# Sun-Sir/BSARec

Hardware: AMD Instinct MI355X
Metric: train sequences/sec, ML-1M L=50 d=64 2-layer (higher is better)
Workload: dtype f32

## Files before the change

### bsarec_amd/_lib.py

```python
import ctypes as C
import os

HERE = os.path.dirname(os.path.abspath(__file__))
LIB_PATH = os.environ.get("BSAREC_LIB") or os.path.join(HERE, "libbsarec_hip.so")
MAX_LAYERS = 16
ABI_VERSION = 10
TOPK_MAX = 1024
NEG_MAX = 1024
NEG_MAX_DRAWS = 1 << 20
TRAIN_NEG_MAX = 8192
TRAIN_NEG_SITE = 0x4E454753

(BUF_LAYER_OUT, BUF_LOGITS, BUF_LOSS, BUF_DSP, BUF_HMIX, BUF_PROBS, BUF_DLAYER_IN, BUF_LOSS_ROWS, BUF_CTX,
 BUF_DLOGITS, BUF_TRAIN_CAND, BUF_TRAIN_CORR, BUF_TRAIN_LOGITS, BUF_TRAIN_DLOGITS) = range(14)
K_NONE, K_FFN1, K_FFN2, K_QKV, K_LOGITS, K_DU, K_DW1, K_FUSED_FWD, K_FUSED_BWD = range(9)

LAYER_FIELDS = ["sqrt_beta", "filter_ln_w", "filter_ln_b", "query_w", "query_b", "key_w", "key_b", "value_w", "value_b",
                "dense_w", "dense_b", "attn_ln_w", "attn_ln_b", "ffn1_w", "ffn1_b", "ffn2_w", "ffn2_b", "ffn_ln_w",
                "ffn_ln_b"]
LAYER_KEYS = {
    "sqrt_beta": "layer.filter_layer.sqrt_beta",
    "filter_ln_w": "layer.filter_layer.LayerNorm.weight", "filter_ln_b": "layer.filter_layer.LayerNorm.bias",
    "query_w": "layer.attention_layer.query.weight", "query_b": "layer.attention_layer.query.bias",
    "key_w": "layer.attention_layer.key.weight", "key_b": "layer.attention_layer.key.bias",
    "value_w": "layer.attention_layer.value.weight", "value_b": "layer.attention_layer.value.bias",
    "dense_w": "layer.attention_layer.dense.weight", "dense_b": "layer.attention_layer.dense.bias",
    "attn_ln_w": "layer.attention_layer.LayerNorm.weight", "attn_ln_b": "layer.attention_layer.LayerNorm.bias",
    "ffn1_w": "feed_forward.dense_1.weight", "ffn1_b": "feed_forward.dense_1.bias",
    "ffn2_w": "feed_forward.dense_2.weight", "ffn2_b": "feed_forward.dense_2.bias",
    "ffn_ln_w": "feed_forward.LayerNorm.weight", "ffn_ln_b": "feed_forward.LayerNorm.bias",
}
OPTIONAL_LAYER_KEYS = {"filter_cw": "layer.filter_layer.complex_weight"}
TOP_KEYS = {"item_emb": "item_embeddings.weight", "pos_emb": "position_embeddings.weight",
            "ln_w": "LayerNorm.weight", "ln_b": "LayerNorm.bias"}


class Config(C.Structure):
    _fields_ = [("batch", C.c_int), ("seq_len", C.c_int), ("hidden", C.c_int), ("heads", C.c_int), ("layers", C.c_int),
                ("item_size", C.c_int), ("cutoff_bins", C.c_int), ("alpha", C.c_float), ("ln_eps", C.c_float),
                ("p_hidden", C.c_float), ("p_attn", C.c_float), ("filter_kind", C.c_int),
                ("hidden_act", C.c_int), ("storage", C.c_int), ("no_fused", C.c_int), ("no_prune_top", C.c_int),
                ("dw_tiled", C.c_int), ("splits", C.c_int), ("top_slabs", C.c_int), ("separate_embed", C.c_int),
                ("separate_top", C.c_int), ("chain_kernels", C.c_int), ("x3_products", C.c_int),
                ("train_negatives", C.c_int), ("train_sampler", C.c_int), ("train_no_logq", C.c_int),
                ("train_lazy_adam", C.c_int),
                ("weight_image", C.c_int)]


TRAIN_FIELDS = ("train_negatives", "train_sampler", "train_no_logq")
TRAIN_SAMPLERS = {"uniform": 0, "popularity": 1}


OPTION_FIELDS = ("storage", "no_fused", "no_prune_top", "dw_tiled", "splits", "top_slabs", "separate_embed", "separate_top", "chain_kernels", "x3_products",
                 "weight_image")
HIDDEN_ACTS = {"gelu": 0, "relu": 1, "swish": 2, "tanh": 3, "sigmoid": 4}

_defaults = {k: 0 for k in OPTION_FIELDS}
_defaults["weight_image"] = 1


def _env_defaults():
    e = os.environ
    d = {}
    if e.get("BSAREC_DW") == "tiled":
        d["dw_tiled"] = 1
    if e.get("BSAREC_PRUNE_TOP") == "0":
        d["no_prune_top"] = 1
    if e.get("BSAREC_EMBED_IN_BLOCK") == "0":
        d["separate_embed"] = 1
    if e.get("BSAREC_TOP_TAIL") == "0":
        d["separate_top"] = 1
    if e.get("BSAREC_FUSED") == "0":
        d["no_fused"] = 1
    if e.get("BSAREC_BLOCK_KERNELS") == "chain":
        d["chain_kernels"] = 1
    if e.get("BSAREC_PRODUCTS") == "bf16x3":
        d["x3_products"] = 1
    for env, key, hi in (("BSAREC_TOP_SLABS", "top_slabs", 16), ("BSAREC_SPLITS", "splits", 1024)):
        if e.get(env, "").isdigit() and 1 <= int(e[env]) <= hi:
            d[key] = int(e[env])
    if e.get("BSAREC_STORAGE") == "bf16":
        d["storage"] = 1
    if e.get("BSAREC_WEIGHT_IMAGE") == "0":
        d["weight_image"] = 0
    return d


def set_default_options(**kw):
    old = {}
    for k, v in kw.items():
        if k not in _defaults:
            raise KeyError(k)
        old[k] = _defaults[k]
        _defaults[k] = int(v)
    return old


def default_options():
    d = dict(_defaults)
    d.update(_env_defaults())
    return d


class Layer(C.Structure):
    _fields_ = [(f, C.c_void_p) for f in LAYER_FIELDS] + [("filter_cw", C.c_void_p)]


class Tensors(C.Structure):
    _fields_ = [("item_emb", C.c_void_p), ("pos_emb", C.c_void_p), ("ln_w", C.c_void_p), ("ln_b", C.c_void_p),
                ("layer", Layer * MAX_LAYERS)]


class Adam(C.Structure):
    _fields_ = [("params", C.c_void_p), ("grads", C.c_void_p), ("exp_avg", C.c_void_p), ("exp_avg_sq", C.c_void_p),
                ("n", C.c_long), ("lr", C.c_float), ("beta1", C.c_float), ("beta2", C.c_float), ("eps", C.c_float),
                ("weight_decay", C.c_float), ("grad_scale", C.c_float), ("shadow_bf16", C.c_void_p), ("shadow_from", C.c_long),
                ("grads2", C.c_void_p), ("grads2_n", C.c_long), ("n_grad_srcs", C.c_int), ("grad_srcs", C.c_void_p * 8),
# ... 10 lines not shown
                ("num_layers", C.c_int), ("out_size", C.c_int)]


class Gru4RecConfig(C.Structure):
    _fields_ = [("gru", GruConfig), ("item_size", C.c_int), ("dropout", C.c_float)]


class Gru4RecHead(C.Structure):
    _fields_ = [("loss", C.c_int), ("candidates", C.c_int), ("bpreg", C.c_float)]


class CaserConfig(C.Structure):
    _fields_ = [("batch", C.c_int), ("seq_len", C.c_int), ("width", C.c_int), ("n_h", C.c_int), ("n_v", C.c_int)]


GRU4REC_CAND_MAX = 8192
GRU4REC_LOSSES = {"ce": 1, "top1": 2, "bpr_max": 3}
GRU4REC_CANDIDATES = {"in_batch": 1, "in_batch+sampled": 2}

HOOK = C.CFUNCTYPE(None, C.c_void_p, C.c_void_p)


EXPORTS = {
    "bsarec_abi_version": (C.c_int, []),
    "bsarec_workspace_bytes": (C.c_size_t, [C.POINTER(Config)]),
    "bsarec_plan_create": (C.c_int, [C.POINTER(C.c_void_p), C.POINTER(Config), C.POINTER(Tensors), C.POINTER(Tensors),
                                     C.POINTER(Tensors), C.c_void_p, C.c_size_t, C.c_void_p, C.c_void_p, C.c_void_p]),
    "bsarec_shadow_refresh": (C.c_int, [C.c_void_p, C.c_void_p]),
    "bsarec_wimage_refresh": (C.c_int, [C.c_void_p, C.c_void_p]),
    "bsarec_wimage_floats": (C.c_long, [C.POINTER(Config)]),
    "bsarec_wimage_offset": (C.c_long, [C.c_int] * 5),
    "bsarec_plan_set_dense_grad_hook": (C.c_int, [C.c_void_p, HOOK, C.c_void_p, C.c_void_p]),
    "bsarec_plan_set_train_sampler": (C.c_int, [C.c_void_p, C.c_void_p]),
    "bsarec_buffer_is_bf16": (C.c_int, [C.c_void_p, C.c_int, C.c_int]),
    "bsarec_plan_is_fused": (C.c_int, [C.c_void_p]),
    "bsarec_config_is_fused": (C.c_int, [C.c_void_p]),
    "bsarec_plan_destroy": (None, [C.c_void_p]),
    "bsarec_buffer_offset": (C.c_long, [C.c_void_p, C.c_int, C.c_int]),
    "bsarec_step_begin": (C.c_int, [C.c_void_p, C.c_void_p]),
    "bsarec_forward": (C.c_int, [C.c_void_p, C.c_void_p, C.c_int, C.c_void_p]),
    "bsarec_forward_last": (C.c_int, [C.c_void_p, C.c_void_p, C.c_int, C.c_void_p]),
    "bsarec_loss": (C.c_int, [C.c_void_p, C.c_void_p, C.c_void_p]),
    "bsarec_loss_bce": (C.c_int, [C.c_void_p, C.c_void_p, C.c_void_p, C.c_void_p]),
    "bsarec_loss_logsig": (C.c_int, [C.c_void_p, C.c_void_p, C.c_void_p, C.c_void_p]),
    "bsarec_logits": (C.c_int, [C.c_void_p, C.c_void_p]),
    "bsarec_backward": (C.c_int, [C.c_void_p, C.c_void_p]),
    "bsarec_backward_seq": (C.c_int, [C.c_void_p, C.c_void_p, C.c_void_p]),
    "bsarec_backward_seq_multi": (C.c_int, [C.c_void_p, C.c_void_p, C.c_void_p]),
    "bsarec_adam_step": (C.c_int, [C.POINTER(Adam), C.c_void_p, C.c_void_p]),
    "bsarec_train_step": (C.c_int, [C.c_void_p, C.c_void_p, C.c_void_p, C.POINTER(Adam), C.c_void_p]),
    "bsarec_gather_batch": (C.c_int, [C.c_void_p, C.c_void_p, C.c_void_p, C.c_long, C.c_void_p, C.c_int, C.c_int,
                                      C.c_void_p, C.c_void_p, C.c_void_p]),
    "bsarec_train_step_indexed": (C.c_int, [C.c_void_p] * 4 + [C.c_long] + [C.c_void_p] * 3 + [C.POINTER(Adam), C.c_void_p]),
    "bsarec_grad_step_indexed": (C.c_int, [C.c_void_p] * 4 + [C.c_long] + [C.c_void_p] * 3 + [C.c_float] * 3 + [C.c_void_p]),
    "bsarec_adam_apply": (C.c_int, [C.POINTER(Adam), C.c_void_p, C.c_void_p]),
    "bsarec_mask_seen": (C.c_int, [C.c_void_p, C.c_long, C.c_int, C.c_void_p, C.c_void_p, C.c_void_p, C.c_void_p]),
    "bsarec_topk_seen": (C.c_int, [C.c_void_p, C.c_long, C.c_int, C.c_int, C.c_void_p, C.c_void_p, C.c_void_p, C.c_int, C.c_void_p,
                                   C.c_void_p, C.c_void_p]),
    "bsarec_sampled_rank": (C.c_int, [C.c_void_p, C.c_long, C.c_void_p, C.c_int, C.c_int, C.c_int] + [C.c_void_p] * 5 +
                            [C.c_int, C.c_uint64, C.c_uint32] + [C.c_void_p] * 4),
    "bsarec_topk_full_workspace_bytes": (C.c_long, [C.c_int] * 5),
    "bsarec_topk_full": (C.c_int, [C.c_void_p, C.c_long, C.c_void_p, C.c_int, C.c_int, C.c_int] + [C.c_void_p] * 3 +
                         [C.c_int, C.c_int, C.c_void_p, C.c_long, C.c_void_p, C.c_void_p, C.c_void_p]),
    "bsarec_topk_full_range": (C.c_int, [C.c_void_p, C.c_long, C.c_void_p, C.c_int, C.c_int, C.c_long, C.c_int] + [C.c_void_p] * 3 +
                               [C.c_int, C.c_int, C.c_void_p, C.c_long, C.c_void_p, C.c_void_p, C.c_void_p]),
    "bsarec_answer_rank": (C.c_int, [C.c_void_p, C.c_long, C.c_void_p, C.c_int, C.c_int, C.c_int] + [C.c_void_p] * 7),
# ... 138 lines not shown
```

### bsarec_amd/csrc/bsarec_hip.hip

```cpp
#include <cmath>
#include "../../include/bsarec_hip.h"
#include "../../include/bsarec_shard.h"
#include "epilogues.h"
#include "kernels.h"
#include "fused_layer.h"
#include "dw_direct.h"
#include "fused_top.h"
#include "fused_chain.h"
#include "comm.h"
#include "catalogue_shard.h"
#include "rank.h"
#include "sampled_rank.h"
#include "full_rank.h"
#include "answer_rank.h"
#include "info_nce.h"
#include "ce_head.h"
#include "sampled_softmax.h"
#include "lazy_adam.h"
#include "gru.h"
#include "gru4rec_step.h"
#include "gru4rec_cand.h"
#include "caser.h"

#include <hip/hip_runtime.h>
// ... 45 lines not shown
    LayerBufs lb[BSAREC_MAX_LAYERS];
    float *logits, *dlogits, *loss_rows, *loss;
    float *dXa, *dXb, *dz, *dT, *dU, *dH, *dXacc, *dO, *dF, *dC, *dS, *dq, *dk, *dv, *dXtmp, *dlast_slab;
    float *slab_wL[BSAREC_MAX_LAYERS], *slab_bL[BSAREC_MAX_LAYERS], *part_lnL[BSAREC_MAX_LAYERS], *part_betaL[BSAREC_MAX_LAYERS];
    float *part_ln0, *part_pos, *trash;
    int pos_slices;
    ReduceJob* jobs; int jobs_per_layer;
    ReduceJob* jobs_pruned;
    bool prune_ok;
    bool pruned;
    int loss_kind;
    const float* ext_dy = nullptr;
    const float* ext_mid[BSAREC_MAX_LAYERS] = {};
    const int64_t *bce_pos, *bce_neg;
    float *part_kvb, *slab_dummy;
    float* part_cwL[BSAREC_MAX_LAYERS];
    float *top_dq, *top_dO, *top_dT, *top_dU, *top_ak, *top_rk, *top_av, *top_rv;
    int* blockmap; int red_blocks;
    long red_elems; const float *red_lo, *red_hi;
    int top_slabs; bool embed_in_block, direct_dw;
    bool scatter_in_block;
    ProfState prof;
    long long* stamps = nullptr;
    bsarec_hook_t dense_hook = nullptr; void* dense_hook_user = nullptr;
    float* lookup_grad = nullptr;
    unsigned long long* lookup_acc = nullptr;
    int* ssm_cand = nullptr; float *ssm_corr = nullptr, *ssm_logits = nullptr, *ssm_dlogits = nullptr;
    const int64_t* pop_cum = nullptr;
    const int64_t* ssm_answers = nullptr;
    int ssm_nslab = 0;
    LazyRows lazy = {};
    bool lazy_now = false;
    float* wimg = nullptr;
};
struct PlanScope {
    bsarec_plan* prev;
    explicit PlanScope(bsarec_plan* p) : prev(t_plan) { t_plan = p; }
    ~PlanScope() { t_plan = prev; }
};

struct ProfScope {
    hipStream_t s; bool on; hipEvent_t stop;
    ProfScope(int kclass, hipStream_t st) : s(st), on(false) {
        ProfState* ps = t_plan ? &t_plan->prof : nullptr;
        on = ps && kclass != BSAREC_K_NONE && kclass == ps->kclass;
        if (!on) return;
        if (ps->used == ps->events.size()) {
            hipEvent_t a, b;
            (void)hipEventCreate(&a); (void)hipEventCreate(&b);
            ps->events.push_back({a, b});
        }
        (void)hipEventRecord(ps->events[ps->used].first, s);
        stop = ps->events[ps->used].second;
        ++ps->used;
    }
    ~ProfScope() { if (on) (void)hipEventRecord(stop, s); }
};

template <auto Kernel, class... A>
static int launch_lds(dim3 grid, dim3 block, size_t smem, hipStream_t s, const A&... a) {
    static size_t raised = 0;
    if (smem > 48 * 1024 && smem > raised) {
        HIPCHK(hipFuncSetAttribute(reinterpret_cast<const void*>(Kernel), hipFuncAttributeMaxDynamicSharedMemorySize, (int)smem));
        raised = smem;
    }
    if (g_dry) return 0;
// ... 48 lines not shown
    explicit Carver(char* b) : base(b), off(0) {}
    template <class T> T* take(size_t n) {
        T* p = base ? reinterpret_cast<T*>(base + off) : nullptr;
        off += rup((long)(n * sizeof(T)), 256);
        return p;
    }
};

static int check_cfg(const bsarec_config_t& c) {
    if (c.batch < 1 || c.seq_len < 1 || c.seq_len > 256) return -1;
    if (c.hidden < 4 || c.hidden > 256 || c.hidden % 4) return -2;
    if (c.heads < 1 || c.hidden % c.heads || (c.hidden / c.heads) % 4) return -3;
    if (c.layers < 1 || c.layers > BSAREC_MAX_LAYERS) return -4;
    if (c.item_size < 2) return -5;
    if (c.cutoff_bins < 1 || c.cutoff_bins > c.seq_len / 2 + 1) return -6;
    if ((long)c.cutoff_bins * c.hidden > 8192) return -7;
    if (c.p_hidden < 0.f || c.p_hidden >= 1.f || c.p_attn < 0.f || c.p_attn >= 1.f) return -8;
    if (c.filter_kind != 0 && c.filter_kind != 1) return -9;
    if (c.filter_kind == 1 && c.cutoff_bins != c.seq_len / 2 + 1) return -9;
    if (c.hidden_act < 0 || c.hidden_act > 4) return -14;
    if (c.storage < 0 || c.storage > 1) return -15;
    if (c.splits < 0 || c.splits > 1024 || c.top_slabs < 0 || c.top_slabs > 16) return -16;
    if (c.train_negatives < 0 || c.train_negatives > BSAREC_TRAIN_NEG_MAX) return -17;
    if (c.train_sampler < 0 || c.train_sampler > 1 || c.train_no_logq < 0 || c.train_no_logq > 1) return -17;
    if (c.train_negatives > 0 && c.storage != 0) return -18;
    if (c.train_lazy_adam < 0 || c.train_lazy_adam > 1 || (c.train_lazy_adam && c.train_negatives == 0)) return -19;
    if (c.weight_image < 0 || c.weight_image > 1) return -20;
    return 0;
}

static bool fused_shape_ok(const bsarec_config_t& c);
static bool wimage_wanted(const bsarec_config_t& c) {
    return c.weight_image && fused_shape_ok(c) && c.storage == 0 && !c.x3_products && !c.chain_kernels && c.filter_kind == 0;
}

static bool fused_shape_ok(const bsarec_config_t& c) {
    const int dh = c.hidden / c.heads;
    if (c.no_fused || c.hidden_act != 0 || c.hidden != 64 || c.seq_len > 64 || !(dh == 16 || dh == 32 || dh == 64)) return false;
    if (c.filter_kind == 1) return c.storage == 0 && c.alpha == 1.0f && c.cutoff_bins <= 36;
    return c.cutoff_bins <= FUSED_MAX_CB;
}

#define SSM_SLAB_MAX 32
static void ssm_split(int N, int cap, int* nslab, int* chunk) {
    const int want = std::max(1, std::min(cap, N / 256));
    *chunk = (int)rup(cdiv(N, want), SSM_KS);
    *nslab = cdiv(N, *chunk);
}

static void derive(bsarec_plan& p) {
    const bsarec_config_t& c = p.cfg;
    p.fused = fused_shape_ok(c);
    p.bf = c.storage == 1 && p.fused;
    p.bf_products = c.storage == 1 && !p.fused;
    p.T = c.batch * c.seq_len;
    p.Lp = (int)rup(c.seq_len, 4);
    p.Vp = (int)rup(c.item_size, 4);
    p.dh = c.hidden / c.heads;
    p.nblk = p.fused ? c.batch : cdiv(p.T, 64);
    p.rows_pb = p.fused ? c.seq_len : 64;
    const int want_splits = c.splits > 0 ? c.splits : (p.fused ? 32 : 40);
    p.top_slabs = c.top_slabs > 0 ? c.top_slabs : 2;
    p.embed_in_block = !c.separate_embed || p.bf;
    p.direct_dw = !c.dw_tiled && (long)p.T * 4 * c.hidden * 4 < (1L << 31);
    p.scatter_in_block = p.fused && p.direct_dw && !c.separate_embed;
    long ch = rup(cdiv(p.T, want_splits), p.bf ? 2 * GEMM_BK : GEMM_BK);
// ... 35 lines not shown
    p.dXa = cv.take<float>(Td); p.dXb = cv.take<float>(Td); p.dz = cv.take<float>(Td); p.dT = cv.take<float>(Td);
    p.dU = cv.take<float>(4 * Td); p.dH = cv.take<float>(Td); p.dXacc = cv.take<float>(Td); p.dO = cv.take<float>(Td);
    p.dF = cv.take<float>(Td); p.dC = cv.take<float>(Td); p.dS = cv.take<float>(B * h * L * p.Lp);
    p.dq = cv.take<float>(Td); p.dk = cv.take<float>(Td); p.dv = cv.take<float>(Td); p.dXtmp = cv.take<float>(Td);
    p.dlast_slab = cv.take<float>((long)p.vsplit * B * d);
    for (int l = 0; l < N; ++l) {
        p.slab_wL[l] = cv.take<float>((long)p.nsplit * 12 * d * d);
        p.slab_bL[l] = cv.take<float>((long)p.nsplit * 9 * d);
        p.part_lnL[l] = cv.take<float>((long)p.nblk * 6 * d);
        p.part_betaL[l] = cv.take<float>(B * d);
    }
    p.part_ln0 = cv.take<float>((long)p.nblk * 2 * d);
    p.pos_slices = cdiv(B, 64);
    p.part_pos = cv.take<float>((long)p.pos_slices * L * d);
    p.trash = cv.take<float>(1024);
    p.lookup_acc = cv.take<unsigned long long>((long)c.item_size * d);
    p.part_kvb = cv.take<float>(2 * B * d);
    for (int l = 0; l < N; ++l) p.part_cwL[l] = c.filter_kind == 1 ? cv.take<float>(B * c.cutoff_bins * d * 2) : nullptr;
    p.top_dq = cv.take<float>(B * d); p.top_dO = cv.take<float>(B * d); p.top_dT = cv.take<float>(B * d);
    p.top_dU = cv.take<float>(4 * B * d);
    p.top_ak = cv.take<float>(B * h * d); p.top_rk = cv.take<float>(B * h * d);
    p.top_av = cv.take<float>(B * h * d); p.top_rv = cv.take<float>(B * h * d);
    p.slab_dummy = cv.take<float>((long)p.nsplit * 4 * d);
    if (c.train_negatives > 0) {
        const long Nn = c.train_negatives;
        p.ssm_cand = cv.take<int>(Nn); p.ssm_corr = cv.take<float>(Nn);
        p.ssm_logits = cv.take<float>(B * (Nn + 1)); p.ssm_dlogits = cv.take<float>(B * (Nn + 1));
    }
    if (c.train_lazy_adam) {
        p.lazy.cap = (int)std::min<long>(c.item_size, T + B + c.train_negatives);
        p.lazy.d4 = (int)(d / 4);
        p.lazy.mark = cv.take<int>(c.item_size); p.lazy.rows = cv.take<int>(p.lazy.cap); p.lazy.count = cv.take<int>(1);
    }
    *total = cv.off;
}

extern "C" int bsarec_abi_version(void) { return BSAREC_ABI_VERSION; }

extern "C" size_t bsarec_workspace_bytes(const bsarec_config_t* cfg) {
    if (!cfg || check_cfg(*cfg) != 0) return 0;
    bsarec_plan p;
    p.cfg = *cfg;
    derive(p);
    size_t total = 0;
    carve(p, nullptr, &total);
    return total;
}

struct SlabMap { long wq, wk, wv, wo, w1, w2, wtot, bq, bk, bv, bo, b1, b2, btot; };
static SlabMap slab_map(long d) {
    SlabMap m;
    m.wq = 0; m.wk = d * d; m.wv = 2 * d * d; m.wo = 3 * d * d; m.w1 = 4 * d * d; m.w2 = 8 * d * d; m.wtot = 12 * d * d;
    m.bq = 0; m.bk = d; m.bv = 2 * d; m.bo = 3 * d; m.b1 = 4 * d; m.b2 = 8 * d; m.btot = 9 * d;
    return m;
}

static float* slab_w_ptr(const bsarec_plan& p, int l, long tensor_off) { return p.slab_wL[l] + tensor_off * p.nsplit; }
static float* slab_b_ptr(const bsarec_plan& p, int l, long tensor_off) { return p.slab_bL[l] + tensor_off * p.nsplit; }

enum LnPart { LN_FF_G, LN_FF_B, LN_A_G, LN_A_B, LN_F_G, LN_F_B };
enum Ln0Part { LN_E_G, LN_E_B };
static float* ln_part(const bsarec_plan& p, int l, LnPart k) { return p.part_lnL[l] + (long)k * p.nblk * p.cfg.hidden; }
static float* ln0_part(const bsarec_plan& p, Ln0Part k) { return p.part_ln0 + (long)k * p.nblk * p.cfg.hidden; }

static const float* h_last(const bsarec_plan& p) { return p.X[p.cfg.layers] + (long)(p.cfg.seq_len - 1) * p.cfg.hidden; }
static long h_last_stride(const bsarec_plan& p) { return (long)p.cfg.seq_len * p.cfg.hidden; }
// ... 102 lines not shown
        if (!p->red_lo || j.dst < p->red_lo) p->red_lo = j.dst;
        if (!p->red_hi || j.dst + j.len > p->red_hi) p->red_hi = j.dst + j.len;
    }
    hipError_t e = hipMemcpyAsync(p->jobs, jobs.data(), jobs.size() * sizeof(ReduceJob), hipMemcpyHostToDevice,
                                  (hipStream_t)stream);
    if (e == hipSuccess) e = hipMemcpyAsync(p->blockmap, bmap.data(), bmap.size() * sizeof(int), hipMemcpyHostToDevice,
                                            (hipStream_t)stream);
    if (e == hipSuccess) e = hipMemcpyAsync(p->jobs_pruned, jobs_pr.data(), jobs_pr.size() * sizeof(ReduceJob),
                                            hipMemcpyHostToDevice, (hipStream_t)stream);
    if (e == hipSuccess) e = hipStreamSynchronize((hipStream_t)stream);
    if (e != hipSuccess) { delete p; return (int)e; }
    g_dry = true;
    int rc = 0;
    for (int last = 0; last < 2 && rc == 0; ++last) {
        rc = last ? bsarec_forward_last(p, reinterpret_cast<const int64_t*>(p->ws), 1, stream)
                  : bsarec_forward(p, reinterpret_cast<const int64_t*>(p->ws), 1, stream);
        if (rc == 0) rc = bsarec_loss(p, reinterpret_cast<const int64_t*>(p->ws), stream);
        if (rc == 0 && p->G.item_emb) rc = bsarec_backward(p, stream);
    }
    g_dry = false;
    p->pruned = false;
    p->train = false;
    if (rc != 0) { delete p; return rc; }
    *out = p;
    return 0;
}

extern "C" void bsarec_plan_destroy(bsarec_plan_t* plan) { delete plan; }

extern "C" long bsarec_buffer_offset(const bsarec_plan_t* p, int buffer, int layer) {
    if (!p) return -1;
    const int N = p->cfg.layers;
    const void* ptr = nullptr;
    if (buffer >= BSAREC_BUF_TRAIN_CAND && p->cfg.train_negatives == 0) return -1;
    switch (buffer) {
        case BSAREC_BUF_LAYER_OUT: if (layer < 0 || layer > N) return -1; ptr = p->X[layer]; break;
        case BSAREC_BUF_LOGITS: ptr = p->logits; break;
        case BSAREC_BUF_DLOGITS: ptr = p->dlogits; break;
        case BSAREC_BUF_LOSS: ptr = p->loss; break;
        case BSAREC_BUF_LOSS_ROWS: ptr = p->loss_rows; break;
        case BSAREC_BUF_DSP: if (layer < 0 || layer >= N) return -1; ptr = p->lb[layer].dsp; break;
        case BSAREC_BUF_HMIX: if (layer < 0 || layer >= N) return -1; ptr = p->lb[layer].hmix; break;
        case BSAREC_BUF_PROBS: if (layer < 0 || layer >= N) return -1; ptr = p->lb[layer].probs; break;
        case BSAREC_BUF_CTX: if (layer < 0 || layer >= N) return -1; ptr = p->lb[layer].ctx; break;
        case BSAREC_BUF_DLAYER_IN: if (layer < 0 || layer > N) return -1; ptr = (layer & 1) ? p->dXb : p->dXa; break;
        case BSAREC_BUF_TRAIN_CAND: ptr = p->ssm_cand; break;
        case BSAREC_BUF_TRAIN_CORR: ptr = p->ssm_corr; break;
        case BSAREC_BUF_TRAIN_LOGITS: ptr = p->ssm_logits; break;
        case BSAREC_BUF_TRAIN_DLOGITS: ptr = p->ssm_dlogits; break;
        default: return -1;
    }
    return (long)((const char*)ptr - p->ws);
}

extern "C" int bsarec_plan_set_dense_grad_hook(bsarec_plan_t* p, bsarec_hook_t hook, void* user, float* lookup_grad) {
    if (!p) return -10;
    if (p->cfg.train_negatives > 0 && (hook || lookup_grad)) return -22;
    p->dense_hook = hook; p->dense_hook_user = user; p->lookup_grad = lookup_grad;
    return 0;
}

extern "C" int bsarec_plan_set_train_sampler(bsarec_plan_t* p, const int64_t* pop_cum) {
    if (!p) return -10;
    if (p->cfg.train_negatives == 0 || p->cfg.train_sampler != 1) return -22;
    p->pop_cum = pop_cum;
    return 0;
}

static int sampled_refusal(const bsarec_plan& p) {
    if (p.cfg.train_negatives == 0) return 0;
    if (p.dense_hook || p.lookup_grad) return -22;
    if (p.cfg.train_sampler == 1 && !p.pop_cum && !g_dry) return -23;
    return 0;
}

static int head_nsplit(const bsarec_plan& p) { return p.loss_kind == 1 ? 1 : (p.loss_kind == 2 ? p.ssm_nslab : p.vsplit); }

extern "C" int bsarec_plan_is_fused(const bsarec_plan_t* p) { return p && p->fused ? 1 : 0; }
extern "C" int bsarec_config_is_fused(const bsarec_config_t* cfg) {
    if (!cfg) return -10;
    RET(check_cfg(*cfg));
    return fused_shape_ok(*cfg) ? 1 : 0;
}

extern "C" int bsarec_buffer_is_bf16(const bsarec_plan_t* p, int buffer, int layer) {
    if (!p || !p->bf) return 0;
    switch (buffer) {
        case BSAREC_BUF_LAYER_OUT: return layer < p->cfg.layers ? 1 : 0;
        case BSAREC_BUF_HMIX: case BSAREC_BUF_PROBS: case BSAREC_BUF_CTX: return 1;
        case BSAREC_BUF_DLAYER_IN: return 1;
        default: return 0;
    }
// ... 101 lines not shown
}
static bool dh_problem_ok(const DhP& h) {
    if (!h.A || !h.E || !h.slab) return false;
    if (h.B < 1 || h.V < 1 || h.kchunk < 8 || (h.kchunk & 7) || h.nsplit < 1 || h.lda < h.V) return false;
    if ((long)h.B * h.lda * 4 >= (1L << 31) || (long)h.V * 256 >= (1L << 31)) return false;
    return true;
}

#define DISPATCH_DH(dh, ...) \
    do { switch (dh) { case 16: { constexpr int DH = 16; __VA_ARGS__; } break; \
                       case 32: { constexpr int DH = 32; __VA_ARGS__; } break; \
                       default: { constexpr int DH = 64; __VA_ARGS__; } break; } } while (0)
#define DISPATCH_BLOCK(p, ...) \
    do { if ((p).bf) { constexpr bool BF = true, X3 = false; DISPATCH_DH((p).dh, __VA_ARGS__); } \
         else if ((p).cfg.x3_products) { constexpr bool BF = false, X3 = true; DISPATCH_DH((p).dh, __VA_ARGS__); } \
         else { constexpr bool BF = false, X3 = false; DISPATCH_DH((p).dh, __VA_ARGS__); } } while (0)

template <bool FWD, class BlockP>
static void fill_block(const bsarec_plan& p, int l, bool tr, const bsarec_layer_t& wm, BlockP& F) {
    const bsarec_config_t& c = p.cfg;
    const bsarec_layer_t& w = p.P.layer[l];
    const LayerBufs& b = p.lb[l];
    memset(&F, 0, sizeof(F));
    F.X = p.X[l];
    F.sqrt_beta = w.sqrt_beta; F.f_g = w.filter_ln_w; F.wq = wm.query_w; F.wk = wm.key_w; F.wv = wm.value_w; F.wo = wm.dense_w;
    F.a_g = w.attn_ln_w; F.w1 = wm.ffn1_w; F.w2 = wm.ffn2_w; F.ff_g = w.ffn_ln_w; F.tw = p.twiddle;
    F.xhat_f = b.xhat_f; F.rstd_f = b.rstd_f; F.q = b.q; F.k = b.k; F.v = b.v; F.probs = b.probs;
    F.xhat_a = b.xhat_a; F.rstd_a = b.rstd_a; F.xhat_ff = b.xhat_ff; F.rstd_ff = b.rstd_ff;
    F.L = c.seq_len; F.Lp = p.Lp; F.cb = c.cutoff_bins; F.heads = c.heads;
    F.alpha = c.alpha; F.oma = (float)(1.0 - (double)c.alpha);
    F.drop_f = make_drop(p, c.p_hidden, 1 + 4 * l, tr); F.drop_p = make_drop(p, c.p_attn, 2 + 4 * l, tr);
    F.drop_o = make_drop(p, c.p_hidden, 3 + 4 * l, tr); F.drop_ff = make_drop(p, c.p_hidden, 4 + 4 * l, tr);
    F.stamps = p.stamps ? p.stamps + 32 * (2 * l + (FWD ? 0 : 1)) : nullptr;
    if constexpr (FWD) {
        F.Xout = p.X[l + 1];
        F.f_b = w.filter_ln_b; F.bq = w.query_b; F.bk = w.key_b; F.bv = w.value_b; F.bo = w.dense_b; F.a_b = w.attn_ln_b;
        F.b1 = w.ffn1_b; F.b2 = w.ffn2_b; F.ff_b = w.ffn_ln_b;
        F.ids32 = p.ids32; F.ctx = b.ctx; F.hmix = b.hmix; F.u = b.u;
        F.eps = c.ln_eps;
    }
}

template <class BlockP>
static void fill_block_partials(const bsarec_plan& p, int l, BlockP& F) {
    F.pg_ff = ln_part(p, l, LN_FF_G); F.pb_ff = ln_part(p, l, LN_FF_B); F.pg_a = ln_part(p, l, LN_A_G);
    F.pb_a = ln_part(p, l, LN_A_B); F.pg_f = ln_part(p, l, LN_F_G); F.pb_f = ln_part(p, l, LN_F_B);
    F.pbeta = p.part_betaL[l];
}

static void fill_top_fwd(bsarec_plan& p, int l, bool tr, TopFwdP& F) {
    fill_block<true>(p, l, tr, p.P.layer[l], F);
    F.low = p.lb[l].dsp;
    F.wk_sh = p.S.layer[l].key_w; F.wv_sh = p.S.layer[l].value_w;
}

static int launch_fused_fwd(bsarec_plan& p, int l, bool tr, hipStream_t s, const int64_t* ids = nullptr, const GatherP* gp = nullptr,
                            bool top_tail = false ) {
    const bsarec_config_t& c = p.cfg;
    FusedFwdP F;
    fill_block<true>(p, l, tr, p.bf ? p.S.layer[l] : p.wimg ? wimage_layer(p, l, false) : p.P.layer[l], F);
    F.xout_f32 = (l == c.layers - 1);
    F.gp = p.lb[l].gp;
    F.dsp = nullptr;
    if (l == 0 && gp) {
        F.e_E = p.P.item_emb; F.e_pos = p.P.pos_emb; F.e_g = p.P.ln_w; F.e_b = p.P.ln_b; F.e_ids = ids; F.e_gp = *gp;
        F.e_drop = make_drop(p, c.p_hidden, 0, tr); F.e_V = c.item_size;
// ... 23 lines not shown
        DISPATCH_DH(p.dh, rc = top_tail ? launch_lds<fused_layer_fwd_kernel<DH, false, TopFwdP, false, false, true>>(grid, block, smem, s, F, TF)
                                        : launch_lds<fused_layer_fwd_kernel<DH, false, NoTail, false, false, true>>(grid, block, smem, s, F, NoTail()));
        return rc;
    }
    DISPATCH_BLOCK(p, rc = top_tail ? launch_lds<fused_layer_fwd_kernel<DH, BF, TopFwdP, X3>>(grid, block, smem, s, F, TF)
                                    : launch_lds<fused_layer_fwd_kernel<DH, BF, NoTail, X3>>(grid, block, smem, s, F, NoTail()));
    return rc;
}

static int launch_fused_bwd(bsarec_plan& p, int l, bool tr, const float* dY, float* dXout, hipStream_t s, bool top,
                            const TopBwdP* head = nullptr ) {
    const bsarec_config_t& c = p.cfg;
    FusedBwdP F;
    fill_block<false>(p, l, tr, p.bf ? p.S.layer[l] : p.wimg ? wimage_layer(p, l, true) : p.P.layer[l], F);
    fill_block_partials(p, l, F);
    F.dY = dY; F.dX = dXout;
    F.u = p.lb[l].gp;
    if (top) { F.dh_slabs = p.dlast_slab; F.dh_nsplit = head_nsplit(p); F.dh_stride = (long)c.batch * c.hidden; }
    if (l == 0) {
        F.e_dz = p.dz; F.e_xhat = p.xhat0; F.e_rstd = p.rstd0; F.e_g = p.P.ln_w;
        F.e_pg = ln0_part(p, LN_E_G); F.e_pb = ln0_part(p, LN_E_B); F.e_drop = make_drop(p, c.p_hidden, 0, tr);
        F.e_dx_extra = p.ext_dy ? p.ext_mid[0] : nullptr;
    }
    F.dT = p.dT; F.dU = p.dU; F.dO = p.dO; F.dq = p.dq; F.dk = p.dk; F.dv = p.dv;
    F.trash = p.trash;
    const dim3 grid(c.batch), block(512);
    const size_t smem = fused_bwd_smem_bytes();
    ProfScope prof(BSAREC_K_FUSED_BWD, s);
    if (c.filter_kind == 1) {
        F.filter_cw = p.P.layer[l].filter_cw; F.pcw = p.part_cwL[l];
        return launch_lds<fused_layer_bwd_kernel<32, false, NoTail, false, true>>(grid, block, smem, s, F, NoTail());
    }
    int rc = 0;
    if (p.wimg) {
        DISPATCH_DH(p.dh, rc = head ? launch_lds<fused_layer_bwd_kernel<DH, false, TopBwdP, false, false, true>>(grid, block, smem, s, F, *head)
                                    : launch_lds<fused_layer_bwd_kernel<DH, false, NoTail, false, false, true>>(grid, block, smem, s, F, NoTail()));
        return rc;
    }
    DISPATCH_BLOCK(p, rc = head ? launch_lds<fused_layer_bwd_kernel<DH, BF, TopBwdP, X3>>(grid, block, smem, s, F, *head)
                                : launch_lds<fused_layer_bwd_kernel<DH, BF, NoTail, X3>>(grid, block, smem, s, F, NoTail()));
    return rc;
}

static int launch_top_fwd(bsarec_plan& p, int l, bool tr, hipStream_t s) {
    TopFwdP F;
    fill_top_fwd(p, l, tr, F);
    int rc = 0;
    DISPATCH_BLOCK(p, rc = launch_lds<top_fwd_kernel<DH, BF>>(dim3(p.cfg.batch), dim3(256), top_fwd_smem_bytes(), s, F));
    return rc;
}

static void fill_top_bwd(bsarec_plan& p, int l, bool tr, float* dXout, TopBwdP& F) {
    const bsarec_config_t& c = p.cfg;
    fill_block<false>(p, l, tr, p.P.layer[l], F);
    fill_block_partials(p, l, F);
    F.dX = dXout;
    F.u = p.lb[l].u; F.low = p.lb[l].dsp;
    F.dh_slabs = p.dlast_slab; F.dh_nsplit = head_nsplit(p); F.dh_stride = (long)c.batch * c.hidden;
    F.dT = p.top_dT; F.dU = p.top_dU; F.dO = p.top_dO; F.dq = p.top_dq;
    F.ak = p.top_ak; F.rk = p.top_rk; F.av = p.top_av; F.rv = p.top_rv;
    F.pbk = p.part_kvb; F.pbv = p.part_kvb + (long)c.batch * c.hidden;
}

static int launch_top_bwd(bsarec_plan& p, int l, bool tr, float* dXout, hipStream_t s) {
    TopBwdP F;
    fill_top_bwd(p, l, tr, dXout, F);
    int rc = 0;
    DISPATCH_BLOCK(p, rc = launch_lds<top_bwd_kernel<DH, BF>>(dim3(p.cfg.batch), dim3(256), top_bwd_smem_bytes(), s, F));
    return rc;
}

extern "C" int bsarec_debug_stamps(bsarec_plan_t* p, void* dev_buf) { if (!p) return -10; p->stamps = (long long*)dev_buf; return 0; }

#ifdef BSAREC_DW_STAMPS
extern "C" int bsarec_debug_dw_stamps(long long* host_out, int n) {
    if (!host_out || n < 1 || n > DW_STAMP_MAX) return -10;
    HIPCHK(hipDeviceSynchronize());
    HIPCHK(hipMemcpyFromSymbol(host_out, HIP_SYMBOL(g_dw_stamps), (size_t)n * 8 * sizeof(long long)));
    return 0;
}
#endif

extern "C" int bsarec_step_begin(bsarec_plan_t* p, void* stream) {
    if (!p) return -10;
    LAUNCH(step_begin_kernel, dim3(1), dim3(1), 0, (hipStream_t)stream, p->state, (long long*)nullptr, 0);
    return (int)hipGetLastError();
}

static int forward_impl(bsarec_plan_t* p, const int64_t* ids, int train, void* stream, const GatherP& gp, bool last_only);

extern "C" int bsarec_forward(bsarec_plan_t* p, const int64_t* ids, int train, void* stream) {
    GatherP none;
    memset(&none, 0, sizeof(none));
    return forward_impl(p, ids, train, stream, none, false);
}

extern "C" int bsarec_forward_last(bsarec_plan_t* p, const int64_t* ids, int train, void* stream) {
    GatherP none;
    memset(&none, 0, sizeof(none));
    return forward_impl(p, ids, train, stream, none, true);
// ... 1961 lines not shown
```

### bsarec_amd/csrc/fused_layer.h

```cpp
#pragma once
#include "common.h"
#include "kernels.h"
#include "wimage.h"
#include <type_traits>

#define FS 68
#define FU 260
#define FUSED_MAX_CB 8

struct FusedFwdP {
    const float* X; float* Xout;
    const float *sqrt_beta, *f_g, *f_b, *wq, *bq, *wk, *bk, *wv, *bv, *wo, *bo, *a_g, *a_b, *w1, *b1, *w2, *b2, *ff_g, *ff_b;
    const float* tw; const int* ids32;
    float *xhat_f, *rstd_f, *q, *k, *v, *probs, *ctx, *xhat_a, *rstd_a, *hmix, *u, *xhat_ff, *rstd_ff, *dsp;
    float* gp;
    int L, Lp, cb, heads;
    float alpha, oma, eps;
    DropP drop_f, drop_p, drop_o, drop_ff;
    float* trash;
    long long* stamps;
    const float *e_E, *e_pos, *e_g, *e_b; const int64_t* e_ids; GatherP e_gp; DropP e_drop; int e_V;
    float *e_X0, *e_xhat, *e_rstd; int* e_ids32;
    int xout_f32;
    const float* filter_cw;
};


template <class T> struct GlobalPtr { static __device__ __forceinline__ T fix(T v) { return v; } };
template <class U> struct GlobalPtr<U*> {
    static __device__ __forceinline__ U* fix(U* v) {
        return (U*)(__attribute__((address_space(1))) U*)v;
    }
};
template <class T>
__device__ __forceinline__ T kernarg_field(unsigned byte_off) {
    typedef __attribute__((address_space(4))) const char* kptr_t;
    typedef __attribute__((address_space(4))) const unsigned* kwords_t;
    kptr_t base = (kptr_t)__builtin_amdgcn_kernarg_segment_ptr();
    asm volatile("" : "+s"(base));
    kwords_t w = (kwords_t)(base + byte_off);
    union { T v; unsigned u[(sizeof(T) + 3) / 4]; } x;
#pragma unroll
    for (unsigned i = 0; i < (sizeof(T) + 3) / 4; ++i) x.u[i] = w[i];
    return GlobalPtr<T>::fix(x.v);
}
#define KARG(S, f) kernarg_field<decltype(S::f)>((unsigned)offsetof(S, f))
struct KernargTouch { unsigned v[3]; };
template <unsigned BYTES>
__device__ __forceinline__ KernargTouch kernarg_touch() {
    static_assert(BYTES <= 24 * 64, "three lines per wave");
    typedef __attribute__((address_space(4))) const unsigned* kwords_t;
    kwords_t base = (kwords_t)__builtin_amdgcn_kernarg_segment_ptr();
    const unsigned wave = __builtin_amdgcn_readfirstlane(threadIdx.x >> 6);
    constexpr unsigned LAST = (BYTES - 4) / 64;
    KernargTouch t;
#pragma unroll
    for (unsigned j = 0; j < 3; ++j) t.v[j] = base[16 * min(8 * j + wave, LAST)];
// ... 202 lines not shown
#pragma unroll
        for (int s = 0; s < K / 16; ++s)
            acc = mfma_bf16(pk8(ld4(sa + 16 * s), ld4(sa + 16 * s + 4)), pk8(ld4(sb + 16 * s), ld4(sb + 16 * s + 4)), acc);
    } else if constexpr (MM == 2) {
#pragma unroll
        for (int s = 0; s < K / 16; ++s)
            acc = mfma_x3(split3(ld4(sa + 16 * s), ld4(sa + 16 * s + 4)), split3(ld4(sb + 16 * s), ld4(sb + 16 * s + 4)), acc);
    } else {
#pragma unroll
        for (int kb = 0; kb < K / 8; ++kb) {
            const f32x4 a = ld4(sa + 8 * kb), b = ld4(sb + 8 * kb);
#pragma unroll
            for (int s = 0; s < 4; ++s) acc = __builtin_amdgcn_mfma_f32_32x32x2f32(a[s], b[s], acc, 0, 0, 0);
        }
    }
}

struct LnPre { f32x4 bi, g, be, dm[2]; };
__device__ __forceinline__ LnPre ln_pre(const float* __restrict__ bias, const float* __restrict__ gamma, const float* __restrict__ beta,
                                        const DropP& drop, const DropSeed& dseed, long tok0) {
    const int lr = threadIdx.x >> 4, lc = (threadIdx.x & 15) << 2;
    LnPre P;
    P.bi = gld4(bias + lc); P.g = gld4(gamma + lc); P.be = gld4(beta + lc);
#pragma unroll
    for (int i = 0; i < 2; ++i) P.dm[i] = drop_mult4(drop, dseed, (uint64_t)((tok0 + lr + 32 * i) * 64 + lc) >> 2);
    return P;
}
template <bool MIX, bool BF>
__device__ __forceinline__ void ln_rows_64(const LnPre& P, const float* __restrict__ tileA, const float* __restrict__ tileB,
                                           const float* __restrict__ resid, float eps, const float* __restrict__ dsp,
                                           float alpha, float oma, long tok0, int L, float* __restrict__ outL,
                                           float* __restrict__ outG, float* __restrict__ xhatG, float* __restrict__ rstdG,
                                           bool out_f32 = false ,
                                           bool round_outL = false ) {
    const int lr = threadIdx.x >> 4, lc = (threadIdx.x & 15) << 2;
#pragma unroll
    for (int i = 0; i < 2; ++i) {
        const int r = lr + 32 * i;
        const bool ok = r < L;
        const long e = (tok0 + r) * 64 + lc;
        f32x4 v = {0, 0, 0, 0};
        if (ok) v = (ld4(tileA + r * FS + lc) + ld4(tileB + r * FS + lc) + P.bi) * P.dm[i] + ld4(resid + r * FS + lc);
        const float mean = group_sum<16>(v.x + v.y + v.z + v.w) * (1.0f / 64.0f);
        f32x4 dl = {0, 0, 0, 0};
        if (ok) dl = v - mean;
        const float var = group_sum<16>(dl.x * dl.x + dl.y * dl.y + dl.z * dl.z + dl.w * dl.w) * (1.0f / 64.0f);
        const float rs = 1.0f / sqrtf(var + eps);
        f32x4 y = {0, 0, 0, 0};
        if (ok) {
            const f32x4 xh = dl * rs;
            y = P.g * xh + P.be;
            if (MIX) y = alpha * ld4(dsp + r * FS + lc) + oma * y;
            ast4<BF>(xhatG, e, xh);
            if (BF && out_f32) gst4(outG + e, y); else ast4<BF>(outG, e, y);
            if (lc == 0) gst(rstdG + tok0 + r, rs);
        }
        if (BF && round_outL) {
            const unsigned a = pk_bf16(y.x, y.y), c = pk_bf16(y.z, y.w);
            y = f32x4{bf_lo(a), bf_hi(a), bf_lo(c), bf_hi(c)};
        }
        if (outL) st4(outL + r * FS + lc, y);
    }
}

struct NoTail {};
template <bool BF> struct TopFwdRegs;
template <bool BF, unsigned KOFF, bool KV> __device__ __forceinline__ void top_fwd_prefetch(TopFwdRegs<BF>& R);
template <int DH, bool BF, unsigned KOFF, bool HELPED>
__device__ __forceinline__ void top_fwd_rest(const TopFwdRegs<BF>& R, const DropSeed& dseed, float* sX, float* sK, float* sV,
                                             float* sPart, float* sTab, float* sSpec, float* sVec, const int* sIds);
template <bool BF> struct TopFwdHelpRegs;
template <bool BF, unsigned KOFF, bool IMG> __device__ __forceinline__ void top_fwd_help_prefetch(TopFwdHelpRegs<BF>& H);
template <int DH, bool BF, unsigned KOFF>
__device__ __forceinline__ void top_fwd_help(const TopFwdHelpRegs<BF>& H, const float* sX, float* sK, float* sV, float* sVec);
template <class T> struct IsTail { static constexpr bool value = true; };
template <> struct IsTail<NoTail> { static constexpr bool value = false; };
constexpr int TOP_BWD_BARRIERS = 11;
struct TopBwdRegs {
    float sl[32];
    float xh_ff, g_ff, rs_ff, xa, xf, g_a, g_f, rs_a, rs_f, bt, low_l, x_l, q_l;
    f32x4 tq[16];
    float p_pre;
};
struct TopBwdHelpRegs { f32x4 w2c[16], w1c[16], u4; };
template <bool BF, unsigned KOFF> __device__ __forceinline__ void top_bwd_prefetch(TopBwdRegs& R);
template <bool BF, unsigned KOFF> __device__ __forceinline__ void top_bwd_prefetch_tile(TopBwdRegs& R);
template <bool BF, unsigned KOFF> __device__ __forceinline__ void top_bwd_help_prefetch(TopBwdHelpRegs& H);
template <int DH, bool BF, unsigned KOFF, bool HELPED>
__device__ __forceinline__ void top_bwd_body(const TopBwdRegs& R, const DropSeed& dseed, float* sX, float* sK, float* sV, const float* sTab,
                                             float* sVec, float* sDX);
template <bool BF, unsigned KOFF> __device__ __forceinline__ void top_bwd_help_a(const TopBwdHelpRegs& H, float* sVec);
template <int DH, bool BF, unsigned KOFF> __device__ __forceinline__ void top_bwd_help_b(const float* sX, float* sVec, const float* gu, f32x4 (&uw)[16]);


template <int DH, bool BF, class TAILP, bool X3 = false, bool FM = false, bool IMG = false>
__global__ void __launch_bounds__(512) __attribute__((amdgpu_waves_per_eu(2, 2)))
fused_layer_fwd_kernel(const FusedFwdP P_unused, const TAILP T_unused) {
#define PTYPE FusedFwdP
    static_assert(!(BF && X3), "x3 products work on fp32 tensors");
    static_assert(!IMG || (!BF && !X3 && !FM), "the fragment image feeds the fp32 products of the BSARec block");
    constexpr int MM = X3 ? 2 : (BF ? 1 : 0);
    static_assert(!FM || (!BF && !X3 && !IsTail<TAILP>::value), "the FMLPRec block runs in fp32, without a top-block tail");
    constexpr int MAXCB = FM ? 36 : FUSED_MAX_CB;
    constexpr bool TAIL = IsTail<TAILP>::value;
    constexpr unsigned KOFF = (unsigned)((sizeof(FusedFwdP) + 7) & ~(size_t)7);
    const auto R0_L = KARG(FusedFwdP, L);
    const auto R0_Lp = KARG(FusedFwdP, Lp);
    const auto R0_cb = KARG(FusedFwdP, cb);
    const auto R0_heads = KARG(FusedFwdP, heads);
    extern __shared__ __attribute__((aligned(16))) float sm[];
    constexpr int TS = 64 * FS;
    float* sX = sm;
    float* sD = sm + TS;
    float* sH = sm + 2 * TS;
    float* sE = sm + 3 * TS;
    float* sR = sm + 4 * TS;
    float* sQ = sR;
    float* sK = sR + TS;
    float* sVt = sR + 2 * TS;
    float* sC = sR + 3 * TS;
    float* sU = sR;
    float* sTab = sR + 4 * TS;
    float* sSpec = sTab + FUSED_MAX_CB * 128;
    float* sRed = sSpec + FUSED_MAX_CB * 128;
    int* sIds = reinterpret_cast<int*>(sRed + 512);
    if constexpr (FM) { sTab = sR; sSpec = sR + 2 * TS; }

    const int tid = threadIdx.x, lane = tid & 63, wave = tid >> 6;
    const int l31 = lane & 31, half = lane >> 5;
    const int grp = wave >> 2, wm = (wave >> 1) & 1, wn = wave & 1;
    const int L = R0_L, Lp = R0_Lp, heads = R0_heads, cb = R0_cb;
    const int b = blockIdx.x;
    const long tok0 = (long)b * L;
    const int col = wn * 32 + l31;
    constexpr int KHM = MM ? 8 : 4;
    const int KH = KHM * half;
    const long wrow = (long)col * 64 + KH;
    const int arow = (wm * 32 + l31) * FS + KH;
    float* const trash = KARG(FusedFwdP, trash) + 4 * lane;

    STAMP(0);
    const KernargTouch ktouch = kernarg_touch<IsTail<TAILP>::value ? KOFF + (unsigned)sizeof(TAILP) : (unsigned)sizeof(FusedFwdP)>();
    const DropSeed dseed = drop_seed(KARG(FusedFwdP, drop_f));
    kernarg_touch_done(ktouch);
    const auto R1_X = KARG(FusedFwdP, X);
    const auto R1_ids32 = KARG(FusedFwdP, ids32);
    const auto R1_tw = KARG(FusedFwdP, tw);
    const auto R1_wq = KARG(FusedFwdP, wq);
    WFrag<MM, 64> wA, wB;
    float qkv_bias[3] = {0.f, 0.f, 0.f};
    if (!FM && grp == 1) {
        load_w<MM, 64, 64, IMG>(R1_wq, wrow, wA);
        qkv_bias[0] = gld(KARG(FusedFwdP, bq) + col); qkv_bias[1] = gld(KARG(FusedFwdP, bk) + col);
        qkv_bias[2] = gld(KARG(FusedFwdP, bv) + col);
    }
    const float* const eE = KARG(FusedFwdP, e_E);
    if (eE) {
        const GatherP gp = KARG(FusedFwdP, e_gp);
        const int64_t* const eids = KARG(FusedFwdP, e_ids);
        const float* const epos = KARG(FusedFwdP, e_pos);
        const int V = KARG(FusedFwdP, e_V);
        const float eeps = KARG(FusedFwdP, eps);
        const float* const e_g = KARG(FusedFwdP, e_g); const float* const e_b = KARG(FusedFwdP, e_b);
        int* const e_ids32 = KARG(FusedFwdP, e_ids32); const DropP e_drop = KARG(FusedFwdP, e_drop);
        float* const e_xhat = KARG(FusedFwdP, e_xhat); float* const e_X0 = KARG(FusedFwdP, e_X0); float* const e_rstd = KARG(FusedFwdP, e_rstd);
        long src = 0;
        if (gp.table) {
            src = *(const AS_GLOBAL long long*)gp.cursor + b;
            src = src < gp.n ? (long)*(const AS_GLOBAL int64_t*)(gp.perm + src) : 0;
            if (tid == 0) *(AS_GLOBAL int64_t*)(gp.ans_out + b) = *(const AS_GLOBAL int64_t*)(gp.ans_table + src);
        }
        const f32x4 eg = gld4(e_g + ((tid & 15) << 2)), eb = gld4(e_b + ((tid & 15) << 2));
#pragma unroll
        for (int p = 0; p < 2; ++p) {
            const int idx = tid + p * 512, r = idx >> 4, c4 = (idx & 15) << 2;
            const bool ok = r < L;
            const long e = (tok0 + r) * 64 + c4;
            f32x4 v = {0, 0, 0, 0};
            int id = 0;
            if (ok) {
                int64_t id64;
                if (gp.table) {
                    id64 = *(const AS_GLOBAL int64_t*)(gp.table + src * L + r);
                    if (c4 == 0) *(AS_GLOBAL int64_t*)(gp.ids_out + tok0 + r) = id64;
                } else id64 = *(const AS_GLOBAL int64_t*)(eids + tok0 + r);
                id = (int)id64;
                id = id < 0 ? 0 : (id >= V ? V - 1 : id);
                v = gld4(eE + (long)id * 64 + c4) + gld4(epos + (long)r * 64 + c4);
            }
            if (c4 == 0) { sIds[r] = id; if (ok) *(AS_GLOBAL int*)(e_ids32 + tok0 + r) = id; }
            const float mean = group_sum<16>(v.x + v.y + v.z + v.w) * (1.0f / 64.0f);
            f32x4 dl = {0, 0, 0, 0};
            if (ok) dl = v - mean;
            const float var = group_sum<16>(dl.x * dl.x + dl.y * dl.y + dl.z * dl.z + dl.w * dl.w) * (1.0f / 64.0f);
            const float rs = 1.0f / sqrtf(var + eeps);
            f32x4 y = {0, 0, 0, 0};
            if (ok) {
                const f32x4 xh = dl * rs;
                y = (eg * xh + eb) * drop_mult4(e_drop, dseed, (uint64_t)e >> 2);
                ast4<BF>(e_xhat, e, xh);
                ast4<BF>(e_X0, e, y);
                if (c4 == 0) gst(e_rstd + tok0 + r, rs);
            }
            st4(sX + r * FS + c4, y);
        }
    } else {
#pragma unroll
    for (int p = 0; p < 2; ++p) {
        const int idx = tid + p * 512, r = idx >> 4, c4 = (idx & 15) << 2;
        f32x4 v = ald4<BF>(R1_X, (tok0 + min(r, L - 1)) * 64 + c4);
        if (r >= L) v = f32x4{0, 0, 0, 0};
        st4(sX + r * FS + c4, v);
    }
    if (tid < 64) sIds[tid] = tid < L ? gldi(R1_ids32 + (tok0 + tid)) : 0;
    }
    build_twiddle_table(R1_tw, L, cb, sTab);
    lds_barrier();

    STAMP(1);
    const auto R2_bk = KARG(FusedFwdP, bk);
    const auto R2_bq = KARG(FusedFwdP, bq);
    const auto R2_bv = KARG(FusedFwdP, bv);
    const auto R2_drop_f = KARG(FusedFwdP, drop_f);
    const auto R2_dsp = KARG(FusedFwdP, dsp);
    const auto R2_eps = KARG(FusedFwdP, eps);
    const auto R2_f_b = KARG(FusedFwdP, f_b);
    const auto R2_f_g = KARG(FusedFwdP, f_g);
    const auto R2_k = KARG(FusedFwdP, k);
    const auto R2_q = KARG(FusedFwdP, q);
    const auto R2_rstd_f = KARG(FusedFwdP, rstd_f);
    const auto R2_sqrt_beta = KARG(FusedFwdP, sqrt_beta);
    const auto R2_v = KARG(FusedFwdP, v);
    const auto R2_wk = KARG(FusedFwdP, wk);
    const auto R2_wo = KARG(FusedFwdP, wo);
    const auto R2_wv = KARG(FusedFwdP, wv);
    const auto R2_xhat_f = KARG(FusedFwdP, xhat_f);
    {
        float* part = sH;
        const int lr = (tid & 255) >> 4, lc = (tid & 15) << 2;
        auto qkv = [&](auto whichc) {
            constexpr int which = decltype(whichc)::value;
            f32x16 acc;
#pragma unroll
            for (int r = 0; r < 16; ++r) acc[r] = 0.f;
            if (which == 0) { load_w<MM, 64, 64, IMG>(R2_wk, wrow, wB); mma_w<MM, 64>(sX + arow, wA, acc); }
            else if (which == 1) { load_w<MM, 64, 64, IMG>(R2_wv, wrow, wA); mma_w<MM, 64>(sX + arow, wB, acc); }
            else mma_w<MM, 64>(sX + arow, wA, acc);
            const float bias = qkv_bias[which];
#pragma unroll
            for (int r = 0; r < 16; ++r) {
                const int row = wm * 32 + rho(r) + 4 * half;
                const float val = acc[r] + bias;
                if (which == 0) sQ[row * FS + col] = val;
                else if (which == 1) sK[row * FS + col] = val;
                else sVt[col * FS + row] = val;
            }
        };
#pragma unroll
        for (int ch = 0; ch < MAXCB / 4; ++ch) {
            const int k0 = 4 * ch;
            if (k0 >= cb) break;
            if (grp == 0) {
                f32x4 re[4], im[4];
#pragma unroll
                for (int j = 0; j < 4; ++j) { re[j] = f32x4{0, 0, 0, 0}; im[j] = f32x4{0, 0, 0, 0}; }
#pragma unroll
                for (int r0 = 0; r0 < 64; r0 += 16) {
                    const int t = r0 + lr;
                    if (t < L) {
// ... 20 lines not shown
                        float acc = 0.f;
#pragma unroll
                        for (int g = 0; g < 16; ++g) acc += part[g * 512 + i];
                        sSpec[(k0 + j) * 128 + rc] = acc;
                    }
                }
            } else if (!FM && ch == 0) qkv(std::integral_constant<int, 1>{});
            lds_barrier();
        }
        if (!FM && grp == 1) qkv(std::integral_constant<int, 2>{});
        if constexpr (FM) {
            const float* const cwp = KARG(FusedFwdP, filter_cw);
            for (int i = tid; i < cb * 64; i += 512) {
                const int k = i >> 6, c = i & 63;
                const float xr = sSpec[k * 128 + c], xi = sSpec[k * 128 + 64 + c];
                const float wr = gld(cwp + 2 * i), wi = gld(cwp + 2 * i + 1);
                sSpec[k * 128 + c] = xr * wr - xi * wi;
                sSpec[k * 128 + 64 + c] = xr * wi + xi * wr;
            }
            lds_barrier();
        }
        {
            f32x4 b2 = gld4(R2_sqrt_beta + lc);
            b2 = b2 * b2;
            if constexpr (FM) b2 = f32x4{0, 0, 0, 0};
            float* const R2_hmix = KARG(FusedFwdP, hmix);
            const f32x4 g = gld4(R2_f_g + lc), be = gld4(R2_f_b + lc);
            const int rbeg = grp == 0 ? 0 : 48, rend = grp == 0 ? 48 : 64;
            for (int r0 = rbeg; r0 < rend; r0 += 16) {
                const int t = r0 + lr;
                const bool ok = t < L;
                const long e = (tok0 + t) * 64 + lc;
                f32x4 v = {0, 0, 0, 0};
                if (ok) {
                    const f32x4 xv = ld4(sX + t * FS + lc);
                    const f32x4 low = lowpass_tab(sSpec, t, lc, L, cb, sTab);
                    v = (low + b2 * (xv - low)) * drop_mult4(R2_drop_f, dseed, (uint64_t)e >> 2) + xv;
                }
                const float mean = group_sum<16>(v.x + v.y + v.z + v.w) * (1.0f / 64.0f);
                f32x4 dl = {0, 0, 0, 0};
                if (ok) dl = v - mean;
                const float var = group_sum<16>(dl.x * dl.x + dl.y * dl.y + dl.z * dl.z + dl.w * dl.w) * (1.0f / 64.0f);
                const float rs = 1.0f / sqrtf(var + R2_eps);
                f32x4 y = {0, 0, 0, 0};
                if (ok) {
                    const f32x4 xh = dl * rs;
                    y = g * xh + be;
                    ast4<BF>(R2_xhat_f, e, xh);
                    if (R2_dsp) gst4(R2_dsp + e, y);
                    if constexpr (FM) gst4(R2_hmix + e, y);
                    if (lc == 0) gst(R2_rstd_f + (tok0 + t), rs);
                }
                st4((FM ? sH : sD) + t * FS + lc, y);
            }
        }
    }
    WFrag<MM, 32> wO;
    if constexpr (!FM) load_w<MM, 32, 64, IMG>(R2_wo, wrow + 32 * grp, wO);
    lds_barrier();
    if constexpr (!FM) {
    {
        const int lr = tid >> 4, lc = (tid & 15) << 2;
#pragma unroll
        for (int r0 = 0; r0 < 64; r0 += 32) {
            const int r = r0 + lr;
            if (r < L) {
                const long e = (tok0 + r) * 64 + lc;
                ast4<BF>(R2_q, e, ld4(sQ + r * FS + lc));
                ast4<BF>(R2_k, e, ld4(sK + r * FS + lc));
                ast4<BF>(R2_v, e, f32x4{sVt[lc * FS + r], sVt[(lc + 1) * FS + r], sVt[(lc + 2) * FS + r], sVt[(lc + 3) * FS + r]});
            }
        }
    }

    STAMP(3);
    const auto R3_ctx = KARG(FusedFwdP, ctx);
    const auto R3_drop_p = KARG(FusedFwdP, drop_p);
    const auto R3_probs = KARG(FusedFwdP, probs);
    {
        const int nt = (L + 31) >> 5;
        const float sqrt_dh = sqrtf((float)DH);
        constexpr int NCT = (DH + 31) / 32;
        const int ncombo = heads * nt;
        const int pair = wave >> 1, kt = wave & 1;
        for (int c0 = 0; c0 < ncombo; c0 += 4) {
            const int combo = c0 + pair;
            const bool act = combo < ncombo && kt < nt;
            const int head = act ? combo / nt : 0, qt = act ? combo % nt : 0;
            const int query = 32 * qt + l31;
            f32x16 st;
#pragma unroll
            for (int r = 0; r < 16; ++r) st[r] = 0.f;
            float mx = -INFINITY;
            if (act) {
                mma_ll<MM, DH>(sK + (32 * kt + l31) * FS + head * DH + KH, sQ + query * FS + head * DH + KH, st);
#pragma unroll
                for (int r = 0; r < 16; ++r) {
                    const int key = 32 * kt + rho(r) + 4 * half;
                    float s = -INFINITY;
                    if (key < L) s = st[r] / sqrt_dh + ((key <= query && sIds[key] > 0) ? 0.0f : -10000.0f);
                    st[r] = s;
                    mx = fmaxf(mx, s);
                }
                mx = xor32_max(mx);
                sRed[(pair * 2 + kt) * 64 + lane] = mx;
            }
            lds_barrier();
            float sum = 0.f;
            if (act) {
                if (nt == 2) mx = fmaxf(mx, sRed[(pair * 2 + (kt ^ 1)) * 64 + lane]);
#pragma unroll
                for (int r = 0; r < 16; ++r) {
                    const int key = 32 * kt + rho(r) + 4 * half;
                    const float e = key < L ? __expf(st[r] - mx) : 0.f;
                    st[r] = e;
                    sum += e;
                }
                sum = xor32_sum(sum);
            }
            lds_barrier();
            if (act) sRed[(pair * 2 + kt) * 64 + lane] = sum;
            lds_barrier();
            if (act) {
                if (nt == 2) sum += sRed[(pair * 2 + (kt ^ 1)) * 64 + lane];
                const float inv = 1.0f / sum;
#pragma unroll
                for (int g = 0; g < 4; ++g) {
                    const int key0 = 32 * kt + 8 * g + 4 * half;
                    f32x4 p = {st[4 * g] * inv, st[4 * g + 1] * inv, st[4 * g + 2] * inv, st[4 * g + 3] * inv};
                    f32x4 m = {1.f, 1.f, 1.f, 1.f};
                    if (query < L && key0 < Lp) {
                        const long e = (((long)b * heads + head) * L + query) * Lp + key0;
                        ast4<BF>(R3_probs, e, p);
                        m = drop_mult4(R3_drop_p, dseed, (uint64_t)e >> 2);
                    }
                    p = p * m;
                    st[4 * g] = p.x; st[4 * g + 1] = p.y; st[4 * g + 2] = p.z; st[4 * g + 3] = p.w;
                }
                float* dstT = kt == 0 ? sC : sE;
#pragma unroll
                for (int ct = 0; ct < NCT; ++ct) {
                    f32x16 cacc;
#pragma unroll
                    for (int r = 0; r < 16; ++r) cacc[r] = 0.f;
                    const bool crow_ok = 32 * ct + l31 < DH;
                    const float* va = sVt + (head * DH + 32 * ct + (crow_ok ? l31 : 0)) * FS + 32 * kt + 4 * half;
                    if constexpr (MM != 0) {
#pragma unroll
                        for (int s2 = 0; s2 < 2; ++s2) {
                            f32x4 a0 = ld4(va + 16 * s2), a1 = ld4(va + 16 * s2 + 8);
                            if (!crow_ok) { a0 = f32x4{0, 0, 0, 0}; a1 = a0; }
                            if constexpr (MM == 1) {
                                const u32x4 pb = {pk_bf16(st[8 * s2], st[8 * s2 + 1]), pk_bf16(st[8 * s2 + 2], st[8 * s2 + 3]),
                                                  pk_bf16(st[8 * s2 + 4], st[8 * s2 + 5]), pk_bf16(st[8 * s2 + 6], st[8 * s2 + 7])};
                                cacc = mfma_bf16(pk8(a0, a1), pb, cacc);
                            } else {
                                cacc = mfma_x3(split3(a0, a1), split3(f32x4{st[8 * s2], st[8 * s2 + 1], st[8 * s2 + 2], st[8 * s2 + 3]},
                                                                      f32x4{st[8 * s2 + 4], st[8 * s2 + 5], st[8 * s2 + 6], st[8 * s2 + 7]}), cacc);
                            }
                        }
                    } else {
#pragma unroll
                    for (int g = 0; g < 4; ++g) {
                        f32x4 a = ld4(va + 8 * g);
                        if (!crow_ok) a = f32x4{0, 0, 0, 0};
#pragma unroll
                        for (int j = 0; j < 4; ++j)
                            cacc = __builtin_amdgcn_mfma_f32_32x32x2f32(a[j], st[4 * g + j], cacc, 0, 0, 0);
                    }
                    }
#pragma unroll
// ... 21 lines not shown
    lds_barrier();
    }

    STAMP(4);
    const auto R4_a_b = KARG(FusedFwdP, a_b);
    const auto R4_a_g = KARG(FusedFwdP, a_g);
    const auto R4_alpha = KARG(FusedFwdP, alpha);
    const auto R4_bo = KARG(FusedFwdP, bo);
    const auto R4_drop_o = KARG(FusedFwdP, drop_o);
    const auto R4_eps = KARG(FusedFwdP, eps);
    const auto R4_hmix = KARG(FusedFwdP, hmix);
    const auto R4_oma = KARG(FusedFwdP, oma);
    const auto R4_rstd_a = KARG(FusedFwdP, rstd_a);
    const auto R4_w1 = KARG(FusedFwdP, w1);
    const auto R4_xhat_a = KARG(FusedFwdP, xhat_a);
    float ffn_bias[2];
    LnPre lnA;
    if constexpr (!FM) lnA = ln_pre(R4_bo, R4_a_g, R4_a_b, R4_drop_o, dseed, tok0);
    {
        load_w<MM, 64, 64, IMG>(R4_w1, (long)(128 * grp + col) * 64 + KH, wA);
        ffn_bias[0] = gld(KARG(FusedFwdP, b1) + 128 * grp + col); ffn_bias[1] = gld(KARG(FusedFwdP, b1) + 128 * grp + 64 + col);
        if constexpr (!FM) {
        f32x16 acc;
#pragma unroll
        for (int r = 0; r < 16; ++r) acc[r] = 0.f;
        mma_w<MM, 32>(sC + arow + 32 * grp, wO, acc);
        float* part = grp == 0 ? sQ : sK;
#pragma unroll
        for (int r = 0; r < 16; ++r) part[(wm * 32 + rho(r) + 4 * half) * FS + col] = acc[r];
        }
    }
    if constexpr (!FM) {
    lds_barrier();
    ln_rows_64<true, BF>(lnA, sQ, sK, sX, R4_eps, sD, R4_alpha, R4_oma, tok0, L, sH, R4_hmix, R4_xhat_a, R4_rstd_a);
    lds_barrier();
    }

    STAMP(5);
    const auto R5_b1 = KARG(FusedFwdP, b1);
    const auto R5_u = KARG(FusedFwdP, u);
    const auto R5_w1 = KARG(FusedFwdP, w1);
    const auto R5_w2 = KARG(FusedFwdP, w2);
    {
        const float* sa = sH + arow;
#pragma unroll
        for (int i = 0; i < 2; ++i) {
            const int c256 = (2 * grp + i) * 64 + col;
            WFrag<MM, 64>& wcur = i ? wB : wA;
            WFrag<MM, 64>& wnxt = i ? wA : wB;
            if (i == 0) load_w<MM, 64, 64, IMG>(R5_w1, (long)(c256 + 64) * 64 + KH, wnxt);
            else load_w<MM, 64, 256, IMG>(R5_w2, (long)col * 256 + 128 * grp + KH, wnxt);
            f32x16 acc;
#pragma unroll
            for (int r = 0; r < 16; ++r) acc[r] = 0.f;
            mma_w<MM, 64>(sa, wcur, acc);
            const float bias = ffn_bias[i];
#pragma unroll
            for (int r = 0; r < 16; ++r) {
                const int row = wm * 32 + rho(r) + 4 * half;
                sU[row * FU + c256] = acc[r] + bias;
            }
        }
    }
    lds_barrier();

    STAMP(6);
    const auto R6_w2 = KARG(FusedFwdP, w2);
// ... 7 lines not shown
    {
        for (int idx = tid; idx < 64 * 64; idx += 512) {
            const int r = idx >> 6, c4 = (idx & 63) << 2;
            const f32x4 v = ld4(sU + r * FU + c4);
            float g0, g1, g2, g3, p0, p1, p2, p3;
            gelu_both(v.x, g0, p0); gelu_both(v.y, g1, p1); gelu_both(v.z, g2, p2); gelu_both(v.w, g3, p3);
            const f32x4 g = {g0, g1, g2, g3}, gp = {p0, p1, p2, p3};
            if (r < L) { ast4<BF>(R6_u, (tok0 + r) * 256 + c4, g); ast4<BF>(R6_gp, (tok0 + r) * 256 + c4, gp); }
            st4(sU + r * FU + c4, g);
        }
        lds_barrier();
        lnF = ln_pre(R7_b2, R7_ff_g, R7_ff_b, R7_drop_ff, dseed, tok0);
        f32x16 acc;
#pragma unroll
        for (int r = 0; r < 16; ++r) acc[r] = 0.f;
        const float* sa = sU + (wm * 32 + l31) * FU + 128 * grp + KH;
        load_w<MM, 64, 256, IMG>(R6_w2, (long)col * 256 + 128 * grp + 64 + KH, wB);
        mma_w<MM, 64>(sa, wA, acc);
        mma_w<MM, 64>(sa + 64, wB, acc);
        float* part = grp == 0 ? sX : sE;
#pragma unroll
        for (int r = 0; r < 16; ++r) part[(wm * 32 + rho(r) + 4 * half) * FS + col] = acc[r];
    }
    lds_barrier();
    STAMP(7);
    TopFwdRegs<BF> TR;
    TopFwdHelpRegs<BF> TH;
    if constexpr (TAIL) { if (wave < 4) top_fwd_prefetch<BF, KOFF, false>(TR); else top_fwd_help_prefetch<BF, KOFF, IMG>(TH); }
    const auto R7_Xout = KARG(FusedFwdP, Xout);
    const auto R7_eps = KARG(FusedFwdP, eps);
    const auto R7_rstd_ff = KARG(FusedFwdP, rstd_ff);
    const auto R7_xhat_ff = KARG(FusedFwdP, xhat_ff);
    ln_rows_64<false, BF>(lnF, sX, sE, sH, R7_eps, nullptr, 0.f, 1.f, tok0, L,
                          TAIL ? sD : nullptr, R7_Xout, R7_xhat_ff, R7_rstd_ff, KARG(FusedFwdP, xout_f32) != 0, TAIL);
    STAMP(8);
    if constexpr (TAIL) {
        lds_barrier();
        if (wave < 4) top_fwd_rest<DH, BF, KOFF, true>(TR, dseed, sD, sR, sR + TS, sR + 2 * TS, sTab, sSpec, sX, sIds);
        else top_fwd_help<DH, BF, KOFF>(TH, sD, sR, sR + TS, sX);
    }
}
#undef PTYPE

static inline size_t fused_fwd_smem_bytes() {
    return (size_t)(8 * 64 * FS + 2 * FUSED_MAX_CB * 128 + 512 + 64) * 4;
}

struct FusedBwdP {
    const float* dY; float* dX; const float* X;
    const float *sqrt_beta, *f_g, *wq, *wk, *wv, *wo, *a_g, *w1, *w2, *ff_g;
    const float* tw;
    const float *xhat_f, *rstd_f, *q, *k, *v, *probs, *xhat_a, *rstd_a, *u, *xhat_ff, *rstd_ff;
    const float* dh_slabs; int dh_nsplit; long dh_stride;
    float *dT, *dU, *dO, *dq, *dk, *dv;
    float *pg_ff, *pb_ff, *pg_a, *pb_a, *pg_f, *pb_f, *pbeta;
    int L, Lp, cb, heads;
    float alpha, oma;
    DropP drop_f, drop_p, drop_o, drop_ff;
    float* trash;
    long long* stamps;
    float* e_dz; const float *e_xhat, *e_rstd, *e_g; float *e_pg, *e_pb; DropP e_drop;
    const float* filter_cw; float* pcw;
    const float* e_dx_extra;
};


__device__ __forceinline__ void seq_partial_64(const f32x4& v, float* __restrict__ red, float* __restrict__ dst, float scale_by = 1.f,
                                               const float* __restrict__ mul = nullptr) {
    const int lr = threadIdx.x >> 4, lc = (threadIdx.x & 15) << 2;
    const int ng = blockDim.x >> 4;
    lds_barrier();
    st4(red + lr * 64 + lc, v);
    lds_barrier();
    if (threadIdx.x < 64) {
        float s = 0.f;
        for (int g = 0; g < ng; ++g) s += red[g * 64 + threadIdx.x];
        if (mul) s *= gld(mul + threadIdx.x);
        gst(dst + threadIdx.x, s * scale_by);
    }
}


template <int N>
__device__ __forceinline__ void seq_partials_64(const f32x4 (&v)[N], float* const (&red)[N], float* const (&dst)[N],
                                                float scale0 = 1.f, const float* __restrict__ mul0 = nullptr) {
    const int lr = threadIdx.x >> 4, lc = (threadIdx.x & 15) << 2;
    const int ng = blockDim.x >> 4;
    lds_barrier();
#pragma unroll
    for (int i = 0; i < N; ++i) st4(red[i] + lr * 64 + lc, v[i]);
    lds_barrier();
    const int i = threadIdx.x >> 6, c = threadIdx.x & 63;
    if (i < N) {
        const float* r = red[0];
        float* d = dst[0];
#pragma unroll
        for (int k = 1; k < N; ++k) if (i == k) { r = red[k]; d = dst[k]; }
        float s0 = 0.f, s1 = 0.f, s2 = 0.f, s3 = 0.f;
        for (int g = 0; g < ng; g += 4) {
            s0 += r[g * 64 + c]; s1 += r[(g + 1) * 64 + c]; s2 += r[(g + 2) * 64 + c]; s3 += r[(g + 3) * 64 + c];
        }
        float sum = (s0 + s1) + (s2 + s3);
        if (i == 0) { if (mul0) sum *= gld(mul0 + c); sum *= scale0; }
        gst(d + c, sum);
    }
}

template <int DH, bool BF, class HEADP, bool X3 = false, bool FM = false, bool IMG = false>
__global__ void __launch_bounds__(512) __attribute__((amdgpu_waves_per_eu(2, 2)))
fused_layer_bwd_kernel(const FusedBwdP P_unused, const HEADP H_unused) {
#define PTYPE FusedBwdP
    static_assert(!(BF && X3), "x3 products work on fp32 tensors");
    static_assert(!IMG || (!BF && !X3 && !FM), "the fragment image feeds the fp32 products of the BSARec block");
    constexpr int MM = X3 ? 2 : (BF ? 1 : 0);
    static_assert(!FM || (!BF && !X3 && !IsTail<HEADP>::value), "the FMLPRec block runs in fp32, without a top-block head");
    constexpr bool HEAD = IsTail<HEADP>::value;
    constexpr unsigned KOFF = (unsigned)((sizeof(FusedBwdP) + 7) & ~(size_t)7);
    const auto R0_L = KARG(FusedBwdP, L);
    const auto R0_Lp = KARG(FusedBwdP, Lp);
    const auto R0_cb = KARG(FusedBwdP, cb);
    const auto R0_heads = KARG(FusedBwdP, heads);
    extern __shared__ __attribute__((aligned(16))) float sm[];
    constexpr int TS = 64 * FS;
    float* sAcc = sm;
    float* sT = sm + TS;
    float* sQ = sm + 2 * TS;
    float* sK = sm + 3 * TS;
    float* sV = sm + 4 * TS;
    float* sS = sm + 5 * TS;
    float* sdU = sQ;
    float* sG = sm + 6 * TS;
    float* sdF = sm + 7 * TS;
    float* sPm = sm + 8 * TS;
    float* sTab = sm + 9 * TS;
    float* sRed = sTab + FUSED_MAX_CB * 128;
    const int tid = threadIdx.x, lane = tid & 63, wave = tid >> 6;
    const int l31 = lane & 31, half = lane >> 5;
    const int grp = wave >> 2, wm = (wave >> 1) & 1, wn = wave & 1;
    const int lr = tid >> 4, lc = (tid & 15) << 2;
    const int L = R0_L, Lp = R0_Lp, heads = R0_heads, cb = R0_cb;
    const int b = blockIdx.x;
    const long tok0 = (long)b * L;
    const int col = wn * 32 + l31;
    constexpr int KHM = MM ? 8 : 4;
    const int KH = KHM * half;
    const int arow = (wm * 32 + l31) * FS + KH;
    float* const trash = KARG(FusedBwdP, trash) + 4 * lane;

    STAMP(0);
    const KernargTouch ktouch = kernarg_touch<KOFF + (unsigned)sizeof(HEADP)>();
    TopBwdRegs HR;
    TopBwdHelpRegs HH;
    if constexpr (HEAD) {
        if (wave == 0) top_bwd_prefetch<BF, KOFF>(HR);
        else if (wave < 4) {
            if (wave == 3) build_twiddle_table(KARG(FusedBwdP, tw), L, cb, sTab, 192, 64);
            top_bwd_prefetch_tile<BF, KOFF>(HR);
        } else top_bwd_help_prefetch<BF, KOFF>(HH);
    }
    const DropSeed dseed = drop_seed(KARG(FusedBwdP, drop_f));
    kernarg_touch_done(ktouch);
    const auto R1_dT = KARG(FusedBwdP, dT);
    const auto R1_dY = KARG(FusedBwdP, dY);
    const auto R1_dh_nsplit = KARG(FusedBwdP, dh_nsplit);
    const auto R1_dh_slabs = KARG(FusedBwdP, dh_slabs);
    const auto R1_dh_stride = KARG(FusedBwdP, dh_stride);
    const auto R1_drop_ff = KARG(FusedBwdP, drop_ff);
    const auto R1_ff_g = KARG(FusedBwdP, ff_g);
    const auto R1_pb_ff = KARG(FusedBwdP, pb_ff);
    const auto R1_pg_ff = KARG(FusedBwdP, pg_ff);
    const auto R1_rstd_ff = KARG(FusedBwdP, rstd_ff);
    const auto R1_tw = KARG(FusedBwdP, tw);
    const auto R1_w2 = KARG(FusedBwdP, w2);
    const auto R1_xhat_ff = KARG(FusedBwdP, xhat_ff);
    if constexpr (!FM && !HEAD) build_twiddle_table(R1_tw, L, cb, sTab);
    if constexpr (HEAD) {
        if (wave < 4) {
            top_bwd_body<DH, BF, KOFF, true>(HR, dseed, sG, sdF, sPm, sTab, sAcc, sT);
        } else {
            top_bwd_help_a<BF, KOFF>(HH, sAcc);
            f32x4 uw[16];
            top_bwd_help_b<DH, BF, KOFF>(sG, sAcc, KARG(FusedBwdP, u), uw);
#pragma unroll
            for (int i = 0; i < 16; ++i) {
                const int idx = (tid - 256) + i * 256, r = idx >> 6, c4 = (idx & 63) << 2;
                st4(sdU + r * FU + c4, r < L ? uw[i] : f32x4{0, 0, 0, 0});
            }
        }
    }
    WFrag<MM, 64> wA, wB;
    WFrag<MM, 32> wk4;
    f32x4 e_bt, e_x[2];
    load_wT<MM, 64, 256, 64, IMG>(R1_w2, (long)KH * 256 + 128 * grp + col, wA);
    const f32x4 g = gld4(R1_ff_g + lc);
    f32x4 dy[2], xh[2];
    float rs[2];
#pragma unroll
    for (int i = 0; i < 2; ++i) {
        const int r = 32 * i + lr;
        const long e = (tok0 + r) * 64 + lc;
        dy[i] = f32x4{0, 0, 0, 0}; xh[i] = dy[i]; rs[i] = 0.f;
        if (R1_dh_slabs) {
            if (r < L) {
                if (r == L - 1)
                    for (int sp = 0; sp < R1_dh_nsplit; ++sp) dy[i] += gld4(R1_dh_slabs + sp * R1_dh_stride + (long)b * 64 + lc);
                xh[i] = ald4<BF>(R1_xhat_ff, e); rs[i] = gld(R1_rstd_ff + tok0 + r);
            }
        } else {
            const bool ok = r < L;
            const long ec = (tok0 + min(r, L - 1)) * 64 + lc;
            f32x4 d4 = {0, 0, 0, 0};
            if constexpr (!HEAD) d4 = ald4<BF>(R1_dY, ec);
            const f32x4 x4 = ald4<BF>(R1_xhat_ff, ec);
            const float r1 = gld(R1_rstd_ff + tok0 + min(r, L - 1));
            if constexpr (HEAD) d4 = ld4(sT + r * FS + lc);
            dy[i] = ok ? d4 : f32x4{0, 0, 0, 0}; xh[i] = ok ? x4 : f32x4{0, 0, 0, 0}; rs[i] = ok ? r1 : 0.f;
        }
    }
    f32x4 uv[8];
    if constexpr (!HEAD)
    {
        const float* gu = KARG(FusedBwdP, u);
#pragma unroll
        for (int i = 0; i < 8; ++i) {
            const int idx = tid + i * 512, r = idx >> 6, c4 = (idx & 63) << 2;
            uv[i] = ald4<BF>(gu, (tok0 + min(r, L - 1)) * 256 + c4);
        }
    }

    {
        f32x4 sg = {0, 0, 0, 0}, sb = sg;
#pragma unroll
        for (int i = 0; i < 2; ++i) {
            const int r = 32 * i + lr;
            const bool ok = r < L;
            const long e = (tok0 + r) * 64 + lc;
            const f32x4 gg = dy[i] * g;
            const float m1 = group_sum<16>(gg.x + gg.y + gg.z + gg.w) * (1.0f / 64.0f);
            const float m2 = group_sum<16>(gg.x * xh[i].x + gg.y * xh[i].y + gg.z * xh[i].z + gg.w * xh[i].w) * (1.0f / 64.0f);
            const f32x4 dz = rs[i] * (gg - m1 - xh[i] * m2);
            sg += dy[i] * xh[i]; sb += dy[i];
            f32x4 dt = {0, 0, 0, 0};
            if (ok) { dt = dz * drop_mult4(R1_drop_ff, dseed, (uint64_t)e >> 2); ast4<BF>(R1_dT, e, dt); }
            st4(sAcc + r * FS + lc, dz);
            st4(sT + r * FS + lc, dt);
        }
        {
            const f32x4 pv[2] = {sg, sb};
            float* const pr[2] = {sPm, sPm + 2048};
            float* const pd[2] = {R1_pg_ff + (long)b * 64, R1_pb_ff + (long)b * 64};
            seq_partials_64<2>(pv, pr, pd);
        }
    }
    if constexpr (!HEAD) {
#pragma unroll
    for (int i = 0; i < 8; ++i) {
        const int idx = tid + i * 512, r = idx >> 6, c4 = (idx & 63) << 2;
        st4(sdU + r * FU + c4, r < L ? uv[i] : f32x4{0, 0, 0, 0});
    }
    }
    lds_barrier();

    STAMP(1);
    const auto R2_dU = KARG(FusedBwdP, dU);
    const auto R2_u = KARG(FusedBwdP, u);
    const auto R2_w1 = KARG(FusedBwdP, w1);
    const auto R2_w2 = KARG(FusedBwdP, w2);
    if constexpr (MM == 0) {
        const float* sa = sT + arow;
        const int c0 = (2 * grp) * 64 + col, c1 = c0 + 64;
        load_wT<MM, 64, 256, 64, IMG>(R2_w2, (long)KH * 256 + c1, wB);
        f32x16 acc0, acc1;
#pragma unroll
        for (int r = 0; r < 16; ++r) { acc0[r] = 0.f; acc1[r] = 0.f; }
        mma_w<MM, 64>(sa, wA, acc0);
        load_wT<MM, 64, 64, 256, IMG>(R2_w1, (long)(128 * grp + KH) * 64 + col, wA);
// ... 13 lines not shown
            float* pu = sdU + row * FU + c1;
            *pu = row < L ? acc1[r] * *pu : 0.f;
        }
    } else {
        const float* sa = sT + arow;
#pragma unroll
        for (int i = 0; i < 2; ++i) {
            const int blk = 2 * grp + i, c256 = blk * 64 + col;
            WFrag<MM, 64>& wcur = i ? wB : wA;
            WFrag<MM, 64>& wnxt = i ? wA : wB;
            if (i == 0) load_wT<MM, 64, 256, 64, IMG>(R2_w2, (long)KH * 256 + c256 + 64, wnxt);
            else load_wT<MM, 64, 64, 256, IMG>(R2_w1, (long)(128 * grp + KH) * 64 + col, wnxt);
            f32x16 acc;
#pragma unroll
            for (int r = 0; r < 16; ++r) acc[r] = 0.f;
            mma_w<MM, 64>(sa, wcur, acc);
#pragma unroll
            for (int r = 0; r < 16; ++r) {
                const int row = wm * 32 + rho(r) + 4 * half;
                float* pu = sdU + row * FU + c256;
                *pu = row < L ? acc[r] * *pu : 0.f;
            }
        }
    }
    lds_barrier();
    for (int idx = tid; idx < 64 * 64; idx += 512) {
        const int r = idx >> 6, c4 = (idx & 63) << 2;
        if (r < L) ast4<BF>(R2_dU, (tok0 + r) * 256 + c4, ld4(sdU + r * FU + c4));
    }

    STAMP(2);
    const auto R3_w1 = KARG(FusedBwdP, w1);
    const auto R3_wo = KARG(FusedBwdP, wo);
    WFrag<MM, 32> wO;
    f32x4 pq[2], pk[2], pv[2], xa[2], xf[2];
    float ra[2], rf[2];
    {
        f32x16 acc;
#pragma unroll
        for (int r = 0; r < 16; ++r) acc[r] = 0.f;
        const float* sa = sdU + (wm * 32 + l31) * FU + 128 * grp + KH;
        load_wT<MM, 64, 64, 256, IMG>(R3_w1, (long)(128 * grp + 64 + KH) * 64 + col, wB);
        if constexpr (!FM) load_wT<MM, 32, 64, 64, IMG>(R3_wo, (long)(32 * grp + KH) * 64 + col, wO);
#pragma unroll
        for (int i = 0; i < 2; ++i) {
            const int r = 32 * i + lr;
            const long ec = (tok0 + min(r, L - 1)) * 64 + lc;
            if constexpr (!FM) {
            pq[i] = ald4<BF>(KARG(FusedBwdP, q), ec); pk[i] = ald4<BF>(KARG(FusedBwdP, k), ec); pv[i] = ald4<BF>(KARG(FusedBwdP, v), ec);
            xa[i] = ald4<BF>(KARG(FusedBwdP, xhat_a), ec); ra[i] = gld(KARG(FusedBwdP, rstd_a) + tok0 + min(r, L - 1));
            }
            xf[i] = ald4<BF>(KARG(FusedBwdP, xhat_f), ec);
            rf[i] = gld(KARG(FusedBwdP, rstd_f) + tok0 + min(r, L - 1));
        }
        mma_w<MM, 64>(sa, wA, acc);
        mma_w<MM, 64>(sa + 64, wB, acc);
        float* part = grp == 0 ? sG : sdF;
#pragma unroll
        for (int r = 0; r < 16; ++r) part[(wm * 32 + rho(r) + 4 * half) * FS + col] = acc[r];
    }
    lds_barrier();

    STAMP(3);
    if constexpr (FM) {
        float* const sXin = sT;  float* const sdFm = sPm;  float* const tab = sV;  float* const spec = sG;
        const DropP drop_f = KARG(FusedBwdP, drop_f);
        const f32x4 gf = gld4(KARG(FusedBwdP, f_g) + lc);
        const float* const Xg = KARG(FusedBwdP, X);
        f32x4 sgf = {0, 0, 0, 0}, sbf = sgf;
        const f32x4 z4 = {0, 0, 0, 0};
        f32x4 dzf2[2], dF2[2], x2[2];
#pragma unroll
        for (int i = 0; i < 2; ++i) {
            const int r = 32 * i + lr;
            const bool ok = r < L;
            const long e = (tok0 + r) * 64 + lc;
            if (!ok) { xf[i] = z4; rf[i] = 0.f; }
            f32x4 dh = z4;
            if (ok) dh = ld4(sG + r * FS + lc) + ld4(sdF + r * FS + lc) + ld4(sAcc + r * FS + lc);
            const f32x4 g2 = dh * gf;
            const float n1 = group_sum<16>(g2.x + g2.y + g2.z + g2.w) * (1.0f / 64.0f);
            const float n2 = group_sum<16>(g2.x * xf[i].x + g2.y * xf[i].y + g2.z * xf[i].z + g2.w * xf[i].w) * (1.0f / 64.0f);
            dzf2[i] = rf[i] * (g2 - n1 - xf[i] * n2);
            sgf += dh * xf[i]; sbf += dh;
            dF2[i] = z4; x2[i] = z4;
            if (ok) {
// ... 134 lines not shown
    const auto R4_rstd_a = KARG(FusedBwdP, rstd_a);
    const auto R4_rstd_f = KARG(FusedBwdP, rstd_f);
    const auto R4_v = KARG(FusedBwdP, v);
    const auto R4_xhat_a = KARG(FusedBwdP, xhat_a);
    const auto R4_xhat_f = KARG(FusedBwdP, xhat_f);
    {
        const f32x4 ga = gld4(R4_a_g + lc), gf = gld4(R4_f_g + lc);
        f32x4 sga = {0, 0, 0, 0}, sba = sga, sgf = sga, sbf = sga;
#pragma unroll
        for (int i = 0; i < 2; ++i) {
            const int r = 32 * i + lr;
            const f32x4 z4 = {0, 0, 0, 0};
            f32x4 q4 = pq[i], k4 = pk[i], v4 = pv[i];
            if (r >= L) { q4 = z4; k4 = z4; v4 = z4; xa[i] = z4; xf[i] = z4; ra[i] = 0.f; rf[i] = 0.f; }
            st4(sQ + r * FS + lc, q4); st4(sK + r * FS + lc, k4); st4(sV + r * FS + lc, v4);
        }
#pragma unroll
        for (int i = 0; i < 2; ++i) {
            const int r = 32 * i + lr;
            const bool ok = r < L;
            const long e = (tok0 + r) * 64 + lc;
            f32x4 dh = {0, 0, 0, 0};
            if (ok) dh = ld4(sG + r * FS + lc) + ld4(sdF + r * FS + lc) + ld4(sAcc + r * FS + lc);
            const f32x4 dya = dh * R4_oma, dyf = dh * R4_alpha;
            const f32x4 g1 = dya * ga, g2 = dyf * gf;
            const float m1 = group_sum<16>(g1.x + g1.y + g1.z + g1.w) * (1.0f / 64.0f);
            const float m2 = group_sum<16>(g1.x * xa[i].x + g1.y * xa[i].y + g1.z * xa[i].z + g1.w * xa[i].w) * (1.0f / 64.0f);
            const float n1 = group_sum<16>(g2.x + g2.y + g2.z + g2.w) * (1.0f / 64.0f);
            const float n2 = group_sum<16>(g2.x * xf[i].x + g2.y * xf[i].y + g2.z * xf[i].z + g2.w * xf[i].w) * (1.0f / 64.0f);
            const f32x4 dza = ra[i] * (g1 - m1 - xa[i] * m2), dzf = rf[i] * (g2 - n1 - xf[i] * n2);
            sga += dya * xa[i]; sba += dya; sgf += dyf * xf[i]; sbf += dyf;
            f32x4 dO = {0, 0, 0, 0}, dF = dO;
            if (ok) {
                dO = dza * drop_mult4(R4_drop_o, dseed, (uint64_t)e >> 2);
                dF = dzf * drop_mult4(R4_drop_f, dseed, (uint64_t)e >> 2);
                ast4<BF>(R4_dO, e, dO);
            }
            st4(sAcc + r * FS + lc, dza + dzf);
            st4(sT + r * FS + lc, dO);
            st4(sdF + r * FS + lc, dF);
        }
        {
            const f32x4 pv[4] = {sga, sba, sgf, sbf};
            float* const pr[4] = {sPm, sPm + 2048, sG, sG + 2048};
            float* const pd[4] = {R4_pg_a + (long)b * 64, R4_pb_a + (long)b * 64, R4_pg_f + (long)b * 64, R4_pb_f + (long)b * 64};
            seq_partials_64<4>(pv, pr, pd);
        }
    }
    lds_barrier();

    STAMP(4);
    {
        f32x16 acc;
#pragma unroll
        for (int r = 0; r < 16; ++r) acc[r] = 0.f;
        mma_w<MM, 32>(sT + arow + 32 * grp, wO, acc);
        float* part = grp == 0 ? sG : sPm;
#pragma unroll
        for (int r = 0; r < 16; ++r) part[(wm * 32 + rho(r) + 4 * half) * FS + col] = acc[r];
    }
    lds_barrier();
#pragma unroll
    for (int i = 0; i < 2; ++i) {
        const int r = 32 * i + lr;
        st4(sG + r * FS + lc, ld4(sG + r * FS + lc) + ld4(sPm + r * FS + lc));
    }
    lds_barrier();

    STAMP(5);
    const auto R6_dk = KARG(FusedBwdP, dk);
    const auto R6_dq = KARG(FusedBwdP, dq);
    const auto R6_drop_p = KARG(FusedBwdP, drop_p);
    const auto R6_dv = KARG(FusedBwdP, dv);
    const auto R6_probs = KARG(FusedBwdP, probs);
    {
        const int nt = (L + 31) >> 5;
        const float inv_sqrt_dh = 1.0f / sqrtf((float)DH);
        constexpr int NCT = (DH + 31) / 32;
        constexpr int NRES = (6 * NCT + 7) / 8;
        for (int head = 0; head < heads; ++head) {
            const int hc = head * DH;
            const int qt = (wave >> 1) & 1, kt = wave & 1;
            const int query = 32 * qt + l31;
            const bool c1 = wave < 4;
            f32x4 pp[4], mm[4];
            f32x16 da;
            float delta = 0.f;
            if (c1) {
#pragma unroll
                for (int g = 0; g < 4; ++g) {
                    const int key0 = 32 * kt + 8 * g + 4 * half;
                    pp[g] = f32x4{0, 0, 0, 0}; mm[g] = pp[g];
                    if (query < L && key0 < Lp) {
                        const long e = (((long)b * heads + head) * L + query) * Lp + key0;
                        pp[g] = ald4<BF>(R6_probs, e);
                        mm[g] = drop_mult4(R6_drop_p, dseed, (uint64_t)e >> 2);
                    }
                }
#pragma unroll
                for (int r = 0; r < 16; ++r) da[r] = 0.f;
                if (kt < nt && qt < nt)
                    mma_ll<MM, DH>(sV + (32 * kt + l31) * FS + hc + KH, sG + query * FS + hc + KH, da);
#pragma unroll
                for (int g = 0; g < 4; ++g)
#pragma unroll
                    for (int j = 0; j < 4; ++j) {
                        const float dA = da[4 * g + j] * mm[g][j];
                        delta += dA * pp[g][j];
                        da[4 * g + j] = dA;
                        sPm[(32 * kt + 8 * g + 4 * half + j) * FS + query] = pp[g][j] * mm[g][j];
                    }
                delta = xor32_sum(delta);
                sRed[(qt * 2 + kt) * 64 + lane] = delta;
            }
            lds_barrier();
            if (c1) {
                delta += sRed[(qt * 2 + (kt ^ 1)) * 64 + lane];
#pragma unroll
                for (int g = 0; g < 4; ++g)
#pragma unroll
                    for (int j = 0; j < 4; ++j)
                        sS[(32 * kt + 8 * g + 4 * half + j) * FS + query] = pp[g][j] * (da[4 * g + j] - delta) * inv_sqrt_dh;
            }
            lds_barrier();
            f32x16 res[NRES];
#pragma unroll
            for (int ti = 0; ti < NRES; ++ti) {
                const int t = wave + 8 * ti;
                f32x16 acc;
#pragma unroll
                for (int r = 0; r < 16; ++r) acc[r] = 0.f;
                if (t < 6 * NCT) {
                    const int kind = t / (2 * NCT), rt = (t / NCT) & 1, ct = t % NCT;
                    const int c = 32 * ct + l31;
                    const bool cok = c < DH;
                    const int cc = hc + (cok ? c : 0);
                    if (rt < nt) {
                        const float* bsrc = kind == 0 ? sK : kind == 1 ? sQ : sG;
                        const float* asrc = kind == 2 ? sPm : sS;
                        if constexpr (MM != 0) {
#pragma unroll 2
                            for (int s2 = 0; s2 < 2 * nt; ++s2) {
                                f32x4 a0, a1;
// ... 71 lines not shown
                ast4<BF>(R6_dq, e, ld4(sQ + r * FS + lc));
                ast4<BF>(R6_dk, e, ld4(sK + r * FS + lc));
                ast4<BF>(R6_dv, e, ld4(sV + r * FS + lc));
            }
        }
    }

    STAMP(6);
    {
        f32x16 acc;
#pragma unroll
        for (int r = 0; r < 16; ++r) acc[r] = 0.f;
        mma_w<MM, 64>((grp == 0 ? sQ : sV) + arow, wA, acc);
        mma_w<MM, 32>(sK + arow + 32 * grp, wk4, acc);
        float* part = grp == 0 ? sG : sPm;
#pragma unroll
        for (int r = 0; r < 16; ++r) part[(wm * 32 + rho(r) + 4 * half) * FS + col] = acc[r];
    }
    lds_barrier();

    STAMP(7);
    const auto R8_dX = KARG(FusedBwdP, dX);
    const auto R8_pbeta = KARG(FusedBwdP, pbeta);
    const auto R8_sqrt_beta = KARG(FusedBwdP, sqrt_beta);
    {
        float* sXin = sT;
        float* spec = sAcc;
        float* part = (grp == 0 ? sQ : sV);
        const f32x4 bt = e_bt;
        const f32x4 b2 = bt * bt, omb2 = 1.0f - b2;
        float* const e_dz = KARG(FusedBwdP, e_dz);
        const float* const e_dx_extra = KARG(FusedBwdP, e_dx_extra);
        f32x4 g0 = {0, 0, 0, 0}, e_xh[2], e_ex[2], e_dm[2];
        float e_rs[2];
#pragma unroll
        for (int i = 0; i < 2; ++i) { e_xh[i] = f32x4{0, 0, 0, 0}; e_ex[i] = e_xh[i]; e_dm[i] = e_xh[i]; e_rs[i] = 0.f; }
        if (e_dz || e_dx_extra) {
            const float* const e_xhat = KARG(FusedBwdP, e_xhat);
            const float* const e_rstd = KARG(FusedBwdP, e_rstd);
            const DropP e_drop = KARG(FusedBwdP, e_drop);
            if (e_dz) g0 = gld4(KARG(FusedBwdP, e_g) + lc);
#pragma unroll
            for (int i = 0; i < 2; ++i) {
                const int t = 32 * i + lr;
                const long e = (tok0 + min(t, L - 1)) * 64 + lc;
                if (e_dx_extra) e_ex[i] = gld4(e_dx_extra + e);
                if (e_dz) { e_xh[i] = ald4<BF>(e_xhat, e); e_rs[i] = gld(e_rstd + tok0 + min(t, L - 1)); e_dm[i] = drop_mult4(e_drop, dseed, (uint64_t)e >> 2); }
            }
        }
#pragma unroll
        for (int i = 0; i < 2; ++i) {
            const int r = 32 * i + lr;
            f32x4 x = e_x[i];
            if (r >= L) x = f32x4{0, 0, 0, 0};
            st4(sG + r * FS + lc, ld4(sG + r * FS + lc) + ld4(sPm + r * FS + lc) + ld4(sAcc + r * FS + lc));
            st4(sXin + r * FS + lc, x);
        }
        lds_barrier();
        const int lr16 = (tid & 255) >> 4;
        const float* srcT = grp == 0 ? sXin : sdF;
        float* specg = spec + grp * cb * 128;
#pragma unroll
        for (int ch = 0; ch < FUSED_MAX_CB / 4; ++ch) {
            const int k0 = 4 * ch;
            if (k0 >= cb) break;
            f32x4 re[4], im[4];
#pragma unroll
            for (int j = 0; j < 4; ++j) { re[j] = f32x4{0, 0, 0, 0}; im[j] = f32x4{0, 0, 0, 0}; }
#pragma unroll
            for (int r0 = 0; r0 < 64; r0 += 16) {
                const int t = r0 + lr16;
                if (t < L) {
                    f32x4 x = ld4(srcT + t * FS + lc);
                    if (grp == 1) x = x * omb2;
#pragma unroll
                    for (int j = 0; j < 4; ++j)
                        if (k0 + j < cb) {
                            const float c = sTab[2 * ((k0 + j) * 64 + t)], sn = sTab[2 * ((k0 + j) * 64 + t) + 1];
                            re[j] += x * c; im[j] -= x * sn;
                        }
// ... 1 lines not shown
            }
#pragma unroll
            for (int j = 0; j < 4; ++j) {
                st4(part + ((lr16 * 4 + j) * 2 + 0) * 64 + lc, re[j]);
                st4(part + ((lr16 * 4 + j) * 2 + 1) * 64 + lc, im[j]);
            }
            lds_barrier();
            for (int i = tid & 255; i < 512; i += 256) {
                const int j = i >> 7, rc = i & 127;
                if (k0 + j < cb) {
                    float acc = 0.f;
#pragma unroll
                    for (int g = 0; g < 16; ++g) acc += part[g * 512 + i];
                    specg[(k0 + j) * 128 + rc] = acc;
                }
            }
            lds_barrier();
        }
        f32x4 sb = {0, 0, 0, 0}, sg0 = sb, sb0 = sb;
#pragma unroll
        for (int i = 0; i < 2; ++i) {
            const int t = 32 * i + lr;
            const bool ok = t < L;
            const long e = (tok0 + t) * 64 + lc;
            f32x4 dx = {0, 0, 0, 0}, xh = dx;
            float rs = 0.f;
            if (ok) {
                const f32x4 xv = ld4(sXin + t * FS + lc), df = ld4(sdF + t * FS + lc);
                const f32x4 lowx = lowpass_tab(spec, t, lc, L, cb, sTab);
                const f32x4 lowg = lowpass_tab(spec + cb * 128, t, lc, L, cb, sTab);
                dx = ld4(sG + t * FS + lc) + b2 * df + lowg;
                if (e_dx_extra) dx += e_ex[i];
                sb += df * (xv - lowx);
                if (e_dz) { xh = e_xh[i]; rs = e_rs[i]; dx = dx * e_dm[i]; }
                else ast4<BF>(R8_dX, e, dx);
            }
            if (e_dz) {
                const f32x4 gg = dx * g0;
                const float m1 = group_sum<16>(gg.x + gg.y + gg.z + gg.w) * (1.0f / 64.0f);
                const float m2 = group_sum<16>(gg.x * xh.x + gg.y * xh.y + gg.z * xh.z + gg.w * xh.w) * (1.0f / 64.0f);
                if (ok) gst4(e_dz + e, rs * (gg - m1 - xh * m2));
                sg0 += dx * xh; sb0 += dx;
            }
        }
        if (e_dz) {
            const f32x4 pv[3] = {sb, sg0, sb0};
            float* const pr[3] = {sQ, sQ + 2048, sQ + 4096};
            float* const pd[3] = {R8_pbeta + (long)b * 64, KARG(FusedBwdP, e_pg) + (long)b * 64, KARG(FusedBwdP, e_pb) + (long)b * 64};
            seq_partials_64<3>(pv, pr, pd, 2.0f, R8_sqrt_beta);
        } else {
            const f32x4 pv[1] = {sb};
            float* const pr[1] = {sQ};
            float* const pd[1] = {R8_pbeta + (long)b * 64};
            seq_partials_64<1>(pv, pr, pd, 2.0f, R8_sqrt_beta);
        }
    }
    STAMP(8);
}
#undef PTYPE

static inline size_t fused_bwd_smem_bytes() { return (size_t)(9 * 64 * FS + FUSED_MAX_CB * 128 + 512) * 4; }
```

### bsarec_amd/csrc/fused_top.h

```cpp
#pragma once
#include "fused_layer.h"

struct TopFwdP {
    const float* X; float* Xout;
    const float *sqrt_beta, *f_g, *f_b, *wq, *bq, *wk, *bk, *wv, *bv, *wo, *bo, *a_g, *a_b, *w1, *b1, *w2, *b2, *ff_g, *ff_b;
    const float* tw; const int* ids32;
    float *xhat_f, *rstd_f, *q, *k, *v, *probs, *ctx, *xhat_a, *rstd_a, *hmix, *u, *xhat_ff, *rstd_ff;
    float* low;
    int L, Lp, cb, heads;
    float alpha, oma, eps;
    DropP drop_f, drop_p, drop_o, drop_ff;
    long long* stamps;
    const float *wk_sh, *wv_sh;
};

__device__ __forceinline__ float drop_mult1(const DropP& d, const DropSeed& sd, uint64_t e) {
    if (d.thresh == 0) return d.scale;
    const uint64_t grp = e >> 2;
    const uint4 w = philox4x32_10((uint32_t)grp, (uint32_t)(grp >> 32), d.site, sd.step, sd.k0, sd.k1);
    const int j = (int)(e & 3);
    const uint32_t r = j == 0 ? w.x : j == 1 ? w.y : j == 2 ? w.z : w.w;
    return r >= d.thresh ? d.scale : 0.f;
}

template <int K, int KS>
__device__ __forceinline__ void gemv_rows_load(const float* __restrict__ W, int ldw, int n, int slice, f32x4 (&wv)[K / KS / 4]) {
    const float* w = W + (long)n * ldw + slice * (K / KS);
#pragma unroll
    for (int i = 0; i < K / KS / 4; ++i) wv[i] = gld4(w + 4 * i);
}
template <int K, int KS>
__device__ __forceinline__ float gemv_rows_dot(const f32x4 (&wv)[K / KS / 4], const float* __restrict__ sx, int slice) {
    const float* x = sx + slice * (K / KS);
    float acc = 0.f;
#pragma unroll
    for (int i = 0; i < K / KS / 4; ++i) {
        const f32x4 xv = ld4(x + 4 * i);
        acc += wv[i].x * xv.x + wv[i].y * xv.y + wv[i].z * xv.z + wv[i].w * xv.w;
    }
    if (KS >= 2) acc += dpp_mov<0xB1>(acc);
    if (KS >= 4) acc += dpp_mov<0x4E>(acc);
    if (KS >= 8) acc += dpp_mov<0x141>(acc);
    if (KS >= 16) acc += dpp_mov<0x140>(acc);
    return acc;
}

template <int KC>
__device__ __forceinline__ void gemv_cols_load(const float* __restrict__ W, int ldw, int k0, int i, float (&wv)[KC]) {
    const float* w = W + (long)k0 * ldw + i;
#pragma unroll
    for (int k = 0; k < KC; ++k) wv[k] = gld(w + (long)k * ldw);
}
template <int KC>
__device__ __forceinline__ float gemv_cols_dot(const float (&wv)[KC], const float* __restrict__ sx, int k0) {
    float acc = 0.f;
// ... 49 lines not shown
    const int KH = (BF ? 8 : 4) * half;
    const long wrow = (long)col * 64 + KH;
    if constexpr (KV) {
        load_w<BF, 64>(BF ? TP(wk_sh) : TP(wk), wrow, R.wA);
        load_w<BF, 64>(BF ? TP(wv_sh) : TP(wv), wrow, R.wB);
        R.bias_k = gld(TP(bk) + col); R.bias_v = gld(TP(bv) + col);
    }
    const int on = tid >> 2, osl = tid & 3;
    gemv_rows_load<64, 4>(TP(wq), 64, on, osl, R.wq4);
    gemv_rows_load<64, 4>(TP(wo), 64, on, osl, R.wo4);
    R.bq_n = gld(TP(bq) + on); R.bo_n = gld(TP(bo) + on); R.b1_n = gld(TP(b1) + tid); R.b2_n = gld(TP(b2) + on);
}

template <int DH, bool BF, unsigned KOFF, bool HELPED>
__device__ __forceinline__ void top_fwd_rest(const TopFwdRegs<BF>& R, const DropSeed& dseed, float* sX, float* sK, float* sV,
                                             float* sPart, float* sTab, float* sSpec, float* sVec, const int* sIds) {
    float* sQ = sVec; float* sPd = sVec + 64; float* sCtx = sVec + 320; float* sHm = sVec + 384; float* sG = sVec + 448;
    float* sDsp = sVec + 704;
    float* sMul = sVec + 768;
    float* sMp = sVec + 960;
    const int tid = threadIdx.x, lane = tid & 63, wave = tid >> 6;
    const int l31 = lane & 31, half = lane >> 5;
    const int L = TP(L), Lp = TP(Lp), heads = TP(heads), cb = TP(cb);
    const int b = blockIdx.x, tl = L - 1;
    const long tok0 = (long)b * L, el = (tok0 + tl) * 64;
    const int wm = wave >> 1, wn = wave & 1, col = wn * 32 + l31;
    const int KH = (BF ? 8 : 4) * half;
    const int on = tid >> 2, osl = tid & 3;
    TSTAMP(1);
    float* const Pq = TP(q); float* const Pk = TP(k); float* const Pv = TP(v);
    float* const k_low = TP(low); const DropP d_f = TP(drop_f); const float k_eps = TP(eps);
    float* const k_xhat_f = TP(xhat_f); float* const k_rstd_f = TP(rstd_f);
    const float* const pW1 = TP(w1); const float* const pW2 = TP(w2);

    if constexpr (!HELPED) {
        const int arow = (wm * 32 + l31) * FS + KH;
        f32x16 acc;
#pragma unroll
        for (int r = 0; r < 16; ++r) acc[r] = 0.f;
        mma_w<BF, 64>(sX + arow, R.wA, acc);
#pragma unroll
        for (int r = 0; r < 16; ++r) sK[(wm * 32 + rho(r) + 4 * half) * FS + col] = acc[r] + R.bias_k;
#pragma unroll
        for (int r = 0; r < 16; ++r) acc[r] = 0.f;
        mma_w<BF, 64>(sX + arow, R.wB, acc);
#pragma unroll
        for (int r = 0; r < 16; ++r) sV[(wm * 32 + rho(r) + 4 * half) * FS + col] = acc[r] + R.bias_v;
    }
#ifdef BSAREC_FINE_STAMPS
    TSTAMP(9);
#endif
    if constexpr (!HELPED) {
        auto xsrc = [&](int, int t, int lc) { return ld4(sX + t * FS + lc); };
        dft_spectrum_tab<1>(xsrc, L, cb, sTab, sSpec, sPart);
    } else {
        if (wave == 1) sMul[lane] = drop_mult1(d_f, dseed, (uint64_t)(el + lane));
        const int t = 16 * wave + (lane & 15);
        float pl = 0.f;
        if (t < L)
            for (int k = 0; k < cb; ++k) {
                const float w = (k == 0 || 2 * k == L) ? 1.0f : 2.0f;
                pl += w * (sTab[2 * (k * 64 + t)] * sTab[2 * (k * 64 + tl)] + sTab[2 * (k * 64 + t) + 1] * sTab[2 * (k * 64 + tl) + 1]);
            }
        pl *= 1.0f / (float)L;
        float a2[2] = {0.f, 0.f};
#pragma unroll
        for (int j = 0; j < 16; ++j)
            a2[j & 1] += __builtin_bit_cast(float, __builtin_amdgcn_readlane(__builtin_bit_cast(int, pl), j)) * sX[(16 * wave + j) * FS + lane];
        sPart[wave * 64 + lane] = a2[0] + a2[1];
    }
#ifdef BSAREC_FINE_STAMPS
    TSTAMP(10);
#endif

    {
        const float qv = gemv_rows_dot<64, 4>(R.wq4, sX + tl * FS, osl) + R.bq_n;
        if (osl == 0) { sQ[on] = qv; ast<BF>(Pq, el + on, qv); }
        if constexpr (!HELPED) {
            const int lr = tid >> 4, lc = (tid & 15) << 2;
            for (int r = lr; r < L; r += 16) {
                ast4<BF>(Pk, (tok0 + r) * 64 + lc, ld4(sK + r * FS + lc));
                ast4<BF>(Pv, (tok0 + r) * 64 + lc, ld4(sV + r * FS + lc));
            }
        }
    }
    if constexpr (HELPED) lds_barrier();
#ifdef BSAREC_FINE_STAMPS
    TSTAMP(11);
#endif
    if (wave == 0) {
        const int c = lane, c4 = c & ~3;
        float low;
        if constexpr (HELPED) low = (sPart[c] + sPart[64 + c]) + (sPart[128 + c] + sPart[192 + c]);
        else {
            const f32x4 low4 = lowpass_tab(sSpec, tl, c4, L, cb, sTab);
            low = (c & 3) == 0 ? low4.x : (c & 3) == 1 ? low4.y : (c & 3) == 2 ? low4.z : low4.w;
        }
        const float xv = sX[tl * FS + c];
        gst(k_low + el + c, low);
        const float bt = R.c_beta;
        const float f = low + bt * bt * (xv - low);
        const float v = f * (HELPED ? sMul[c] : drop_mult1(d_f, dseed, (uint64_t)(el + c))) + xv;
        float xh, rs;
        ln_row(v, k_eps, xh, rs);
        ast<BF>(k_xhat_f, el + c, xh);
        if (c == 0) gst(k_rstd_f + tok0 + tl, rs);
        sDsp[c] = R.c_fg * xh + R.c_fb;
    }
    if constexpr (HELPED) {
        if (wave >= 2) {
            const DropP dd = wave == 2 ? TP(drop_o) : TP(drop_ff);
            sMul[(wave - 1) * 64 + lane] = drop_mult1(dd, dseed, (uint64_t)(el + lane));
            const DropP dp = TP(drop_p);
            for (int h = wave - 2; h < heads; h += 2) {
                const long pe = (((long)b * heads + h) * L + tl) * Lp;
                sMp[h * 64 + lane] = drop_mult1(dp, dseed, (uint64_t)(pe + lane));
            }
        }
    }
    float* const k_probs = TP(probs); const DropP d_p = TP(drop_p); float* const k_ctx = TP(ctx);
    lds_barrier();
    TSTAMP(2);
    f32x4 w1r[HELPED ? 1 : 16], w2r[HELPED ? 1 : 16];
    if constexpr (!HELPED) gemv_rows_load<64, 1>(pW1, 64, tid, 0, w1r);

    if (wave < heads) {
        const int head = wave, key = lane;
        float s = -INFINITY;
        if (key < L) {
            float acc = 0.f;
            const float* kr = sK + key * FS + head * DH;
            const float* qr = sQ + head * DH;
#pragma unroll
            for (int c = 0; c < DH; c += 4) {
                const f32x4 kv = ld4(kr + c), qv = ld4(qr + c);
                acc += kv.x * qv.x + kv.y * qv.y + kv.z * qv.z + kv.w * qv.w;
            }
            s = acc / sqrtf((float)DH) + (sIds[key] > 0 ? 0.0f : -10000.0f);
        }
        const float mx = group_max<64>(s);
        const float e = key < L ? __expf(s - mx) : 0.f;
        const float p = e / group_sum<64>(e);
        const long pe = (((long)b * heads + head) * L + tl) * Lp;
        if (key < Lp) ast<BF>(k_probs, pe + key, p);
        sPd[head * 64 + key] = key < L ? p * (HELPED ? sMp[head * 64 + key] : drop_mult1(d_p, dseed, (uint64_t)(pe + key))) : 0.f;
    }
    const DropP d_o = TP(drop_o); float* const k_xhat_a = TP(xhat_a); float* const k_rstd_a = TP(rstd_a);
    const float k_alpha = TP(alpha), k_oma = TP(oma); float* const k_hmix = TP(hmix); float* const k_u = TP(u);
    lds_barrier();
    TSTAMP(3);
    if (tid < 64) {
        const int c = tid, head = c / DH;
        float acc = 0.f;
        float a4[4] = {0.f, 0.f, 0.f, 0.f};
#pragma unroll 16
        for (int j = 0; j < 64; ++j) a4[j & 3] += sPd[head * 64 + j] * sV[j * FS + c];
        acc = (a4[0] + a4[1]) + (a4[2] + a4[3]);
        sCtx[c] = acc;
        ast<BF>(k_ctx, el + c, acc);
    }
    lds_barrier();
    TSTAMP(4);

    {
        const float o = gemv_rows_dot<64, 4>(R.wo4, sCtx, osl) + R.bo_n;
        if (osl == 0) sG[on] = o;
    }
    lds_barrier();
    TSTAMP(5);
    if constexpr (!HELPED) { if (wave != 0) gemv_rows_load<256, 4>(pW2, 256, on, osl, w2r); }
    if (wave == 0) {
        const int c = lane;
        const float v = sG[c] * (HELPED ? sMul[64 + c] : drop_mult1(d_o, dseed, (uint64_t)(el + c))) + sX[tl * FS + c];
        float xh, rs;
        ln_row(v, k_eps, xh, rs);
        ast<BF>(k_xhat_a, el + c, xh);
        if (c == 0) gst(k_rstd_a + tok0 + tl, rs);
        const float a = R.c_ag * xh + R.c_ab;
        const float hm = k_alpha * sDsp[c] + k_oma * a;
        sHm[c] = hm;
        ast<BF>(k_hmix, el + c, hm);
        if constexpr (!HELPED) gemv_rows_load<256, 4>(pW2, 256, on, osl, w2r);
    }
    const DropP d_ff = TP(drop_ff); float* const k_xhat_ff = TP(xhat_ff); float* const k_rstd_ff = TP(rstd_ff); float* const k_Xout = TP(Xout);
    lds_barrier();
    TSTAMP(6);

    if constexpr (!HELPED) {
        const float u = gemv_rows_dot<64, 1>(w1r, sHm, 0) + R.b1_n;
        ast<BF>(k_u, (tok0 + tl) * 256 + tid, u);
        sG[tid] = gelu_f(u);
    }
    lds_barrier();
    TSTAMP(7);
    if constexpr (!HELPED) {
        const float y = gemv_rows_dot<256, 4>(w2r, sG, osl) + R.b2_n;
        if (osl == 0) sQ[on] = y;
    }
    lds_barrier();
    TSTAMP(8);
    if (wave == 0) {
        const int c = lane;
        const float v = sQ[c] * (HELPED ? sMul[128 + c] : drop_mult1(d_ff, dseed, (uint64_t)(el + c))) + sHm[c];
        float xh, rs;
        ln_row(v, k_eps, xh, rs);
        ast<BF>(k_xhat_ff, el + c, xh);
        if (c == 0) gst(k_rstd_ff + tok0 + tl, rs);
        gst(k_Xout + el + c, R.c_ffg * xh + R.c_ffb);
    }
    TSTAMP(15);
}

template <bool BF>
struct TopFwdHelpRegs {
    WFrag<BF, 64> wA, wB;
    float bias_k, bias_v;
};
template <bool BF, unsigned KOFF, bool IMG>
__device__ __forceinline__ void top_fwd_help_prefetch(TopFwdHelpRegs<BF>& H) {
    const int lane = threadIdx.x & 63, hw = ((int)threadIdx.x >> 6) - 4;
    const int l31 = lane & 31, half = lane >> 5;
    const int wn = hw & 1, col = wn * 32 + l31;
    const int KH = (BF ? 8 : 4) * half;
    load_w<BF, 64, 64, IMG>(BF || IMG ? TP(wv_sh) : TP(wv), (long)col * 64 + KH, H.wB);
    load_w<BF, 64, 64, IMG>(BF || IMG ? TP(wk_sh) : TP(wk), (long)col * 64 + KH, H.wA);
    H.bias_v = gld(TP(bv) + col); H.bias_k = gld(TP(bk) + col);
}
template <int DH, bool BF, unsigned KOFF>
__device__ __forceinline__ void top_fwd_help(const TopFwdHelpRegs<BF>& H, const float* sX, float* sK, float* sV, float* sVec) {
    float* sQ = sVec; const float* sHm = sVec + 384; float* sG = sVec + 448;
    const int t = (int)threadIdx.x - 256, lane = t & 63, hw = t >> 6;
    const int l31 = lane & 31, half = lane >> 5;
    const int L = TP(L);
    const int b = blockIdx.x, tl = L - 1;
    const long tok0 = (long)b * L;
    const int wm = hw >> 1, wn = hw & 1, col = wn * 32 + l31;
// ... 99 lines not shown
    {
        const float* const X = TP(X);
#pragma unroll
        for (int p = 0; p < 4; ++p) {
            const int idx = tid + p * 256, r = idx >> 4, c4 = (idx & 15) << 2;
            f32x4 v = ald4<BF>(X, (tok0 + min(r, L - 1)) * 64 + c4);
            if (r >= L) v = f32x4{0, 0, 0, 0};
            st4(sX + r * FS + c4, v);
        }
    }
    if (tid < 64) sIds[tid] = tid < L ? gldi(TP(ids32) + (tok0 + tid)) : 0;
    build_twiddle_table(TP(tw), L, cb, sTab);
    lds_barrier();
    top_fwd_rest<DH, BF, KOFF, false>(R, dseed, sX, sK, sV, sPart, sTab, sSpec, sVec, sIds);
}

static inline size_t top_fwd_smem_bytes() { return (size_t)(3 * 64 * FS + 8192 + 2 * FUSED_MAX_CB * 128 + 768 + 64) * 4; }


struct TopBwdP {
    float* dX; const float* X;
    const float *sqrt_beta, *f_g, *wq, *wk, *wv, *wo, *a_g, *w1, *w2, *ff_g;
    const float* tw;
    const float *xhat_f, *rstd_f, *q, *k, *v, *probs, *xhat_a, *rstd_a, *u, *xhat_ff, *rstd_ff, *low;
    const float* dh_slabs; int dh_nsplit; long dh_stride;
    float *dT, *dU, *dO, *dq;
    float *ak, *rk, *av, *rv;
    float *pbk, *pbv;
    float *pg_ff, *pb_ff, *pg_a, *pb_a, *pg_f, *pb_f, *pbeta;
    int L, Lp, cb, heads;
    float alpha, oma;
    DropP drop_f, drop_p, drop_o, drop_ff;
    long long* stamps;
};

__device__ __forceinline__ float ln_row_bwd(float dy, float gamma, float xhat, float rstd) {
    const float g = dy * gamma;
    const float m1 = group_sum<64>(g) * (1.0f / 64.0f);
    const float m2 = group_sum<64>(g * xhat) * (1.0f / 64.0f);
    return rstd * (g - m1 - xhat * m2);
}

#define TB(f) kernarg_field<decltype(TopBwdP::f)>(KOFF + (unsigned)offsetof(TopBwdP, f))
#define BSTAMP(i) do { long long* st_ = TB(stamps); if (st_ && blockIdx.x == 0 && threadIdx.x == 0) st_[i] = clock64(); } while (0)
static_assert(TOP_BWD_BARRIERS == 11, "barriers of top_bwd_body (fused_layer.h holds the constant)");

template <bool BF, unsigned KOFF>
__device__ __forceinline__ void top_bwd_prefetch(TopBwdRegs& R) {
    const int c = threadIdx.x & 63;
    const int L = TB(L), b = blockIdx.x, tl = L - 1;
    const long tok0 = (long)b * L, el = (tok0 + tl) * 64;
    const int ns = TB(dh_nsplit);
    const float* const slabs = TB(dh_slabs);
    const long stride = TB(dh_stride);
    const float* const k_xhat_ff = TB(xhat_ff); const float* const k_ff_g = TB(ff_g); const float* const k_rstd_ff = TB(rstd_ff);
    const float* const k_xhat_a = TB(xhat_a); const float* const k_xhat_f = TB(xhat_f); const float* const k_a_g = TB(a_g);
    const float* const k_f_g = TB(f_g); const float* const k_rstd_a = TB(rstd_a); const float* const k_rstd_f = TB(rstd_f);
    const float* const k_beta = TB(sqrt_beta); const float* const k_low = TB(low); const float* const k_q = TB(q);
    const float* const pX = TB(X);
    const long slab_bytes = (long)min(ns, 32) * stride * 4;
    const __amdgpu_buffer_rsrc_t rs = __builtin_amdgcn_make_buffer_rsrc((void*)slabs, 0, (int)min(slab_bytes, 0x7fffffffL), 0x00020000);
    const int voff = (b * 64 + c) * 4, sstep = (int)(stride * 4);
#pragma unroll
    for (int sp = 0; sp < 32; ++sp) R.sl[sp] = __builtin_bit_cast(float, __builtin_amdgcn_raw_buffer_load_b32(rs, voff, sp * sstep, 0));
    R.xh_ff = ald<BF>(k_xhat_ff, el + c); R.g_ff = gld(k_ff_g + c); R.rs_ff = gld(k_rstd_ff + tok0 + tl);
    R.xa = ald<BF>(k_xhat_a, el + c); R.xf = ald<BF>(k_xhat_f, el + c); R.g_a = gld(k_a_g + c); R.g_f = gld(k_f_g + c);
    R.rs_a = gld(k_rstd_a + tok0 + tl); R.rs_f = gld(k_rstd_f + tok0 + tl);
    R.bt = gld(k_beta + c); R.low_l = gld(k_low + el + c); R.x_l = ald<BF>(pX, el + c);
    R.q_l = ald<BF>(k_q, el + c);
    const int heads = TB(heads), Lp = TB(Lp);
    R.p_pre = c < L ? ald<BF>(TB(probs), (((long)b * heads + 0) * L + tl) * Lp + c) : 0.f;
}
template <bool BF, unsigned KOFF>
__device__ __forceinline__ void top_bwd_prefetch_tile(TopBwdRegs& R) {
    const int lane = threadIdx.x & 63, wave = threadIdx.x >> 6;
    const int L = TB(L), Lp = TB(Lp), heads = TB(heads), b = blockIdx.x, tl = L - 1;
    const long tok0 = (long)b * L;
    const float* const src = wave == 1 ? TB(X) : wave == 2 ? TB(k) : TB(v);
    R.p_pre = (wave < heads && lane < L) ? ald<BF>(TB(probs), (((long)b * heads + wave) * L + tl) * Lp + lane) : 0.f;
#pragma unroll
    for (int p = 0; p < 16; ++p) {
        const int idx = lane + p * 64, r = idx >> 4, c4 = (idx & 15) << 2;
        R.tq[p] = ald4<BF>(src, (tok0 + min(r, L - 1)) * 64 + c4);
    }
}

template <int DH, bool BF, unsigned KOFF>
__device__ __forceinline__ void top_bwd_head_vectors(int head, int i, int b, int heads, const float (&wkc)[DH], const float (&wvc)[DH],
                                                     const float* sX, float* sVec) {
    const float* sDC = sVec + 832; const float* sQ = sVec + 896; const float* sDs = sVec + 1024; const float* sPd = sVec + 1280;
    float* sQK = sVec + 1536; float* sCV = sVec + 1792;
    const int o = head * 64 + i;
    float* const k_rk = TB(rk); float* const k_rv = TB(rv); float* const k_ak = TB(ak); float* const k_av = TB(av);
    float rk = 0.f, rv = 0.f;
    float rk2 = 0.f, rv2 = 0.f;
#pragma unroll 16
    for (int j = 0; j < 64; j += 2) {
        const float x0 = sX[j * FS + i], x1 = sX[(j + 1) * FS + i];
        rk += sDs[head * 64 + j] * x0; rv += sPd[head * 64 + j] * x0;
        rk2 += sDs[head * 64 + j + 1] * x1; rv2 += sPd[head * 64 + j + 1] * x1;
    }
    rk += rk2; rv += rv2;
    const long e = ((long)b * heads + head) * 64 + i;
    const bool mine = i / DH == head;
    ast<BF>(k_rk, e, rk); ast<BF>(k_rv, e, rv);
    ast<BF>(k_ak, e, mine ? sQ[i] : 0.f); ast<BF>(k_av, e, mine ? sDC[i] : 0.f);
    sQK[o] = gemv_cols_dot<DH>(wkc, sQ, head * DH);
    sCV[o] = gemv_cols_dot<DH>(wvc, sDC, head * DH);
}

template <bool BF, unsigned KOFF>
__device__ __forceinline__ void top_bwd_help_prefetch(TopBwdHelpRegs& H) {
// ... 25 lines not shown
}
template <int DH, bool BF, unsigned KOFF>
__device__ __forceinline__ void top_bwd_help_b(const float* sX, float* sVec, const float* gu, f32x4 (&uw)[16]) {
    const int t = (int)threadIdx.x - 256, lane = t & 63, hw = t >> 6;
    const int heads = TB(heads), L = TB(L), b = blockIdx.x;
    const long tok0 = (long)b * L;
    const bool hv = hw < heads;
    float wkc[DH], wvc[DH];
    const float* const pWk = TB(wk); const float* const pWv = TB(wv);
    auto u_quarter = [&](int q) {
#pragma unroll
        for (int i = 4 * q; i < 4 * q + 4; ++i) {
            const int idx = t + i * 256, r = idx >> 6, c4 = (idx & 63) << 2;
            uw[i] = ald4<BF>(gu, (tok0 + min(r, L - 1)) * 256 + c4);
        }
    };
    gemv_cols_load<DH>(pWk, 64, (hv ? hw : 0) * DH, lane, wkc);
    gemv_cols_load<DH>(pWv, 64, (hv ? hw : 0) * DH, lane, wvc);
    lds_barrier();
    u_quarter(0);
    lds_barrier();
    u_quarter(1);
    lds_barrier();
    lds_barrier();
    if (hv) top_bwd_head_vectors<DH, BF, KOFF>(hw, lane, b, heads, wkc, wvc, sX, sVec);
    lds_barrier();
    u_quarter(2);
    lds_barrier();
    u_quarter(3);
    lds_barrier();
    lds_barrier();
}

template <int DH, bool BF, unsigned KOFF, bool HELPED>
__device__ __forceinline__ void top_bwd_body(const TopBwdRegs& R, const DropSeed& dseed, float* sX, float* sK, float* sV, const float* sTab,
                                             float* sVec, float* sDX) {
    float* sDT = sVec;
    float* sDU = sVec + 64;
    float* sRed = sVec + 320;
    float* sDH = sVec + 576;
    float* sDO = sVec + 640;
    float* sDF = sVec + 704;
    float* sLast = sVec + 768;
    float* sDC = sVec + 832;
    float* sQ = sVec + 896;
    float* sDQ = sVec + 960;
    float* sDs = sVec + 1024;
    float* sPd = sVec + 1280;
    float* sQK = sVec + 1536;
    float* sCV = sVec + 1792;
    float* sPl = sVec + 2048;
    float* sSum = sVec + 2112;

    const int tid = threadIdx.x, lane = tid & 63, wave = tid >> 6;
    BSTAMP(0);
    const int L = TB(L), Lp = TB(Lp), heads = TB(heads), cb = TB(cb);
    const int b = blockIdx.x, tl = L - 1;
    const long tok0 = (long)b * L, el = (tok0 + tl) * 64;

    const int c = lane;
    float dy = 0.f, dz_ff = 0.f;
    float xa = 0.f, xf = 0.f, g_a = 0.f, g_f = 0.f, rs_a = 0.f, rs_f = 0.f, bt = 0.f, low_l = 0.f, x_l = 0.f;
    float u_mine = 0.f;
    float w2c[HELPED ? 1 : 64], w1c[HELPED ? 1 : 64];
    f32x4 tx[4], tk[4], tv[4];
    const float* const pX = TB(X); const float* const pK = TB(k); const float* const pV = TB(v);
    const float* const pW1 = TB(w1); const float* const pW2 = TB(w2); const float* const pU = TB(u);
    const float* const pWo = TB(wo); const float* const pWq = TB(wq); const float* const pWk = TB(wk); const float* const pWv = TB(wv);
    auto weight_loads = [&]() {
        if constexpr (!HELPED) {
            u_mine = ald<BF>(pU, (tok0 + tl) * 256 + tid);
            gemv_cols_load<64>(pW2, 256, 0, tid, w2c);
            gemv_cols_load<64>(pW1, 64, 64 * wave, lane, w1c);
        }
    };
    auto tile_loads = [&]() {
#pragma unroll
        for (int p = 0; p < 4; ++p) {
            const int idx = tid + p * 256, r = idx >> 4, c4 = (idx & 15) << 2;
            const long et = (tok0 + min(r, L - 1)) * 64 + c4;
            tx[p] = ald4<BF>(pX, et); tk[p] = ald4<BF>(pK, et); tv[p] = ald4<BF>(pV, et);
            if (r >= L) { tx[p] = f32x4{0, 0, 0, 0}; tk[p] = tx[p]; tv[p] = tx[p]; }
        }
    };
    if (wave != 0) {
        if constexpr (!HELPED) { weight_loads(); tile_loads(); }
        if (wave == 1) { const DropP d_o = TB(drop_o); sDH[c] = drop_mult1(d_o, dseed, (uint64_t)(el + c)); }
        if (wave == 2) { const DropP d_f = TB(drop_f); sDQ[c] = drop_mult1(d_f, dseed, (uint64_t)(el + c)); }
    }
    if (wave == 0) {
        const int ns = TB(dh_nsplit);
        const DropP d_ff = TB(drop_ff);
        float* const k_pg_ff = TB(pg_ff); float* const k_pb_ff = TB(pb_ff); float* const k_dT = TB(dT);
        xa = R.xa; xf = R.xf; g_a = R.g_a; g_f = R.g_f; rs_a = R.rs_a; rs_f = R.rs_f; bt = R.bt; low_l = R.low_l; x_l = R.x_l;
        const float m_ff = drop_mult1(d_ff, dseed, (uint64_t)(el + c));
        asm volatile("" :: "v"(m_ff));
        __builtin_amdgcn_sched_barrier(0);
        float part[4] = {0.f, 0.f, 0.f, 0.f};
#pragma unroll
        for (int sp = 0; sp < 32; ++sp) part[sp & 3] += R.sl[sp];
        if (ns > 32) {
            const float* const slabs = TB(dh_slabs);
            const long stride = TB(dh_stride);
            for (int sp = 32; sp < ns; ++sp) part[0] += gld(slabs + (long)sp * stride + (long)b * 64 + c);
        }
        dy = (part[0] + part[1]) + (part[2] + part[3]);
        dz_ff = ln_row_bwd(dy, R.g_ff, R.xh_ff, R.rs_ff);
        const float dt = dz_ff * m_ff;
        sDT[c] = dt;
        sQ[c] = R.q_l;
        gst(k_pg_ff + (long)b * 64 + c, dy * R.xh_ff);
        gst(k_pb_ff + (long)b * 64 + c, dy);
        ast<BF>(k_dT, (long)b * 64 + c, dt);
        if constexpr (!HELPED) { __builtin_amdgcn_sched_barrier(0); weight_loads(); tile_loads(); }
    }
    const float k_oma = TB(oma), k_alpha = TB(alpha);
    float* const k_pg_a = TB(pg_a); float* const k_pb_a = TB(pb_a); float* const k_pg_f = TB(pg_f); float* const k_pb_f = TB(pb_f);
    float* const k_dO = TB(dO); float* const k_pbeta = TB(pbeta); float* const k_dU = TB(dU);
    lds_barrier();
    BSTAMP(1);
    if constexpr (HELPED) {
        if (wave != 0) {
            float* const dst = wave == 1 ? sX : wave == 2 ? sK : sV;
#pragma unroll
            for (int p = 0; p < 16; ++p) {
                const int idx = lane + p * 64, r = idx >> 4, c4 = (idx & 15) << 2;
                st4(dst + r * FS + c4, r < L ? R.tq[p] : f32x4{0, 0, 0, 0});
            }
// ... 45 lines not shown
        float pl = 0.f;
        if (c < L)
            for (int k = 0; k < cb; ++k) {
                const float w = (k == 0 || 2 * k == L) ? 1.0f : 2.0f;
                pl += w * (sTab[2 * (k * 64 + c)] * sTab[2 * (k * 64 + tl)] + sTab[2 * (k * 64 + c) + 1] * sTab[2 * (k * 64 + tl) + 1]);
            }
        sPl[c] = pl / (float)L;
#ifdef BSAREC_FINE_STAMPS
        BSTAMP(12);
#endif
    }
    lds_barrier();
    BSTAMP(4);
    sRed[wave * 64 + lane] = gemv_cols_dot<16>(woc, sDO, 16 * wave);
    lds_barrier();
    BSTAMP(5);
    if (tid < 64) sDC[tid] = (sRed[tid] + sRed[64 + tid]) + (sRed[128 + tid] + sRed[192 + tid]);
    lds_barrier();
    BSTAMP(6);

    if (wave < heads) {
        const int head = wave, key = lane;
        float dpd = 0.f, p = 0.f, mp = 0.f;
        if (key < L) {
            const float* vr = sV + key * FS + head * DH;
            const float* dc = sDC + head * DH;
#pragma unroll
            for (int c = 0; c < DH; c += 4) {
                const f32x4 vv = ld4(vr + c), dv = ld4(dc + c);
                dpd += vv.x * dv.x + vv.y * dv.y + vv.z * dv.z + vv.w * dv.w;
            }
            const long pe = (((long)b * heads + head) * L + tl) * Lp + key;
            p = HELPED ? R.p_pre : ald<BF>(k_probs, pe);
            mp = drop_mult1(d_p, dseed, (uint64_t)pe);
        }
        const float dp = dpd * mp;
        const float delta = group_sum<64>(p * dp);
        const float ds = p * (dp - delta) / sqrtf((float)DH);
        const float pd = p * mp;
        sDs[head * 64 + key] = ds;
        sPd[head * 64 + key] = pd;
        const float s1 = group_sum<64>(ds), s2 = group_sum<64>(pd);
        if (key == 0) { sSum[head] = s1; sSum[4 + head] = s2; }
    }
    lds_barrier();
    BSTAMP(7);
    if (tid < 64) {
        const int c = tid, head = c / DH;
        float acc = 0.f;
        float a4[4] = {0.f, 0.f, 0.f, 0.f};
#pragma unroll 16
        for (int j = 0; j < 64; ++j) a4[j & 3] += sDs[head * 64 + j] * sK[j * FS + c];
        acc = (a4[0] + a4[1]) + (a4[2] + a4[3]);
        sDQ[c] = acc;
        ast<BF>(k_dq, (long)b * 64 + c, acc);
        gst(k_pbk + (long)b * 64 + c, sQ[c] * sSum[head]);
        gst(k_pbv + (long)b * 64 + c, sDC[c] * sSum[4 + head]);
    }
    if constexpr (!HELPED) {
        if (hv) top_bwd_head_vectors<DH, BF, KOFF>(wave, lane, b, heads, wkc, wvc, sX, sVec);
    }
    lds_barrier();
    BSTAMP(8);
    sRed[wave * 64 + lane] = gemv_cols_dot<16>(wqc, sDQ, 16 * wave);
    lds_barrier();
    BSTAMP(9);
    if (tid < 64) sLast[tid] += (sRed[tid] + sRed[64 + tid]) + (sRed[128 + tid] + sRed[192 + tid]);
    lds_barrier();
    BSTAMP(10);
    {
        const int lr = tid >> 4, lc = (tid & 15) << 2;
        const f32x4 df = ld4(sDF + lc);
        float* const pdX = sDX ? nullptr : TB(dX);
        for (int j = lr; j < L; j += 16) {
            f32x4 dx = df * sPl[j];
            for (int h = 0; h < heads; ++h)
                dx += ld4(sQK + h * 64 + lc) * sDs[h * 64 + j] + ld4(sCV + h * 64 + lc) * sPd[h * 64 + j];
            if (j == tl) dx += ld4(sLast + lc);
            if (sDX) {
                if constexpr (BF) {
                    const unsigned a = pk_bf16(dx.x, dx.y), c2 = pk_bf16(dx.z, dx.w);
                    dx = f32x4{bf_lo(a), bf_hi(a), bf_lo(c2), bf_hi(c2)};
                }
                st4(sDX + j * FS + lc, dx);
            } else ast4<BF>(pdX, (tok0 + j) * 64 + lc, dx);
        }
    }
    lds_barrier();
    BSTAMP(15);
}

template <int DH, bool BF>
__global__ void __launch_bounds__(256)
top_bwd_kernel(const TopBwdP P_unused) {
    constexpr unsigned KOFF = 0;
    constexpr int TS = 64 * FS;
    extern __shared__ __attribute__((aligned(16))) float sm[];
    float* sX = sm;
    float* sK = sm + TS;
    float* sV = sm + 2 * TS;
    float* sTab = sm + 3 * TS;
    float* sVec = sTab + FUSED_MAX_CB * 128;
    BSTAMP(0);
    TopBwdRegs R;
    if (threadIdx.x < 64) top_bwd_prefetch<BF, KOFF>(R);
    const DropSeed dseed = drop_seed(TB(drop_f));
    build_twiddle_table(TB(tw), TB(L), TB(cb), sTab);
    lds_barrier();
    top_bwd_body<DH, BF, KOFF, false>(R, dseed, sX, sK, sV, sTab, sVec, nullptr);
}


static inline size_t top_bwd_smem_bytes() { return (size_t)(3 * 64 * FS + FUSED_MAX_CB * 128 + 2176) * 4; }
```

### bsarec_amd/model.py

```python
from __future__ import annotations

import ctypes as C
import math
from collections import OrderedDict
from typing import Dict, List, Optional, Tuple

import numpy as np
import torch
import torch.nn as nn

from . import _lib as L


def param_shapes(args) -> "OrderedDict[str, Tuple[int, ...]]":
    d, Lq, V = args.hidden_size, args.max_seq_length, args.item_size
    s: "OrderedDict[str, Tuple[int, ...]]" = OrderedDict()
    s["item_embeddings.weight"] = (V, d)
    s["position_embeddings.weight"] = (Lq, d)
    s["LayerNorm.weight"] = (d,)
    s["LayerNorm.bias"] = (d,)
    for l in range(args.num_hidden_layers):
        p = f"item_encoder.blocks.{l}."
        s[p + "layer.filter_layer.sqrt_beta"] = (1, 1, d)
        s[p + "layer.filter_layer.LayerNorm.weight"] = (d,)
# ... 9 lines not shown
        s[p + "feed_forward.dense_2.bias"] = (d,)
        s[p + "feed_forward.LayerNorm.weight"] = (d,)
        s[p + "feed_forward.LayerNorm.bias"] = (d,)
    if getattr(args, "filter_kind", 0) == 1:
        for l in range(args.num_hidden_layers):
            s[f"item_encoder.blocks.{l}.layer.filter_layer.complex_weight"] = (1, Lq // 2 + 1, d, 2)
    return s


class _Bag(nn.Module):
    """Attribute container so that parameter paths match the reference's module tree."""


def _twiddle(Lq: int) -> torch.Tensor:
    j = np.arange(Lq, dtype=np.float64)
    tw = np.stack([np.cos(2.0 * np.pi * j / Lq), np.sin(2.0 * np.pi * j / Lq)], axis=1)
    return torch.from_numpy(tw.astype(np.float32).reshape(-1).copy())


class _Plan:

    def __init__(self, model: "BSARecModel", batch: int, garena=None, own_state: bool = False):
        lib = L.load()
        a = model.args
        self.cfg = L.Config(batch, a.max_seq_length, a.hidden_size, a.num_attention_heads, a.num_hidden_layers,
                            a.item_size, model.cutoff_bins, float(a.alpha), 1e-12, float(a.hidden_dropout_prob),
                            float(a.attention_probs_dropout_prob), int(getattr(a, "filter_kind", 0)))
        self.cfg.hidden_act = L.HIDDEN_ACTS[getattr(a, "hidden_act", "gelu")]
        opts = L.default_options()
        opts.update(model.options)
        for k in L.OPTION_FIELDS:
            setattr(self.cfg, k, int(opts.get(k, 0)))
        self.options = {k: int(getattr(self.cfg, k)) for k in L.OPTION_FIELDS}
        for k in L.TRAIN_FIELDS:
            setattr(self.cfg, k, model.train_head[k])
        self.cfg.train_lazy_adam = int(model.lazy_adam)
        nbytes = lib.bsarec_workspace_bytes(C.byref(self.cfg))
        if nbytes == 0:
            raise ValueError("configuration not supported by libbsarec_hip (see include/bsarec_hip.h limits: "
                             "L <= 256, hidden <= 256 and % 4 == 0, head size % 4 == 0, cutoff_bins*hidden <= 8192)")
        dev = model._arena.device
        self.ws = torch.empty(nbytes + 256, dtype=torch.uint8, device=dev)
        off = (-self.ws.data_ptr()) % 256
        self.ws = self.ws[off:off + nbytes]
        self.ws.zero_()
        self.batch = batch
        self.handle = C.c_void_p()
        self.bf16 = bool(self.cfg.storage) and lib.bsarec_config_is_fused(C.byref(self.cfg)) == 1
        self.garena = model._garena if garena is None else garena
        pt, gt = model._tensor_struct(model._arena), model._tensor_struct(self.garena)
        st = model._tensor_struct(model._shadow_arena()) if self.bf16 else None
        self.wimage = lib.bsarec_wimage_floats(C.byref(self.cfg)) > 0
        if self.wimage:
            st = L.Tensors()
            st.layer[0].query_w = model._wimage_arena(lib.bsarec_wimage_floats(C.byref(self.cfg))).data_ptr()
        stream = torch.cuda.current_stream(dev).cuda_stream
        self.state = torch.zeros_like(model._state) if own_state else model._state
        L.check(lib.bsarec_plan_create(C.byref(self.handle), C.byref(self.cfg), C.byref(pt), C.byref(gt),
                                       C.byref(st) if st is not None else None,
                                       self.ws.data_ptr(), nbytes, self.state.data_ptr(),
                                       model._twiddle.data_ptr(), stream), "bsarec_plan_create")
        self.lib = lib
        if self.cfg.train_negatives > 0 and self.cfg.train_sampler == 1 and model._train_cum is not None:
            model._install_train_sampler(self)

    def view(self, buf: int, layer: int, shape) -> torch.Tensor:
        off = self.lib.bsarec_buffer_offset(self.handle, buf, layer)
        if off < 0:
            raise IndexError("no such buffer")
        if self.lib.bsarec_buffer_is_bf16(self.handle, buf, layer):
            n = int(np.prod(shape)) * 2
            return self.ws[off:off + n].view(torch.bfloat16).view(*shape)
        n = int(np.prod(shape)) * 4
        return self.ws[off:off + n].view(torch.float32).view(*shape)

    def __del__(self):
        try:
            if self.handle:
                self.lib.bsarec_plan_destroy(self.handle)
        except Exception:
            pass


class _SlotToken:

    def __init__(self, model, key):
        self.model, self.key = model, key

    def release(self):
        if self.key is not None:
            self.model._slots_busy.discard(self.key)
            self.key = None

    def __del__(self):
        self.release()
# ... 836 lines not shown
```

### include/bsarec_hip.h

```cpp
#ifndef BSAREC_HIP_H
#define BSAREC_HIP_H

#include <stddef.h>
#include <stdint.h>

#ifdef __cplusplus
extern "C" {
#endif

#define BSAREC_MAX_LAYERS 16
#define BSAREC_ABI_VERSION 10

typedef struct {
    int batch;
    int seq_len;
    int hidden;
    int heads;
    int layers;
    int item_size;
    int cutoff_bins;
    float alpha;
    float ln_eps;
    float p_hidden;
    float p_attn;
// ... 15 lines not shown
    int train_lazy_adam;
    int weight_image;
} bsarec_config_t;

typedef struct {
    float *sqrt_beta, *filter_ln_w, *filter_ln_b;
    float *query_w, *query_b, *key_w, *key_b, *value_w, *value_b, *dense_w, *dense_b;
    float *attn_ln_w, *attn_ln_b;
    float *ffn1_w, *ffn1_b, *ffn2_w, *ffn2_b, *ffn_ln_w, *ffn_ln_b;
    float *filter_cw;
} bsarec_layer_t;

typedef struct {
    float *item_emb;
    float *pos_emb;
    float *ln_w, *ln_b;
    bsarec_layer_t layer[BSAREC_MAX_LAYERS];
} bsarec_tensors_t;

enum {
    BSAREC_BUF_LAYER_OUT = 0,
    BSAREC_BUF_LOGITS = 1,
    BSAREC_BUF_LOSS = 2,
    BSAREC_BUF_DSP = 3,
    BSAREC_BUF_HMIX = 4,
    BSAREC_BUF_PROBS = 5,
    BSAREC_BUF_DLAYER_IN = 6,
    BSAREC_BUF_LOSS_ROWS = 7,
    BSAREC_BUF_CTX = 8,
    BSAREC_BUF_DLOGITS = 9,
    BSAREC_BUF_TRAIN_CAND = 10,
    BSAREC_BUF_TRAIN_CORR = 11,
    BSAREC_BUF_TRAIN_LOGITS = 12,
    BSAREC_BUF_TRAIN_DLOGITS = 13
};

typedef struct bsarec_plan bsarec_plan_t;

int bsarec_abi_version(void);

size_t bsarec_workspace_bytes(const bsarec_config_t *cfg);

#define BSAREC_STATE_BYTES 64

int bsarec_plan_create(bsarec_plan_t **out, const bsarec_config_t *cfg, const bsarec_tensors_t *params,
                       const bsarec_tensors_t *grads, const bsarec_tensors_t *shadow, void *workspace,
                       size_t workspace_bytes, void *state, const float *twiddle, void *stream);
int bsarec_shadow_refresh(bsarec_plan_t *plan, void *stream);
int bsarec_wimage_refresh(bsarec_plan_t *plan, void *stream);
long bsarec_wimage_floats(const bsarec_config_t *cfg);
long bsarec_wimage_offset(int which, int transposed, int d, int n, int k);
int bsarec_buffer_is_bf16(const bsarec_plan_t *plan, int buffer, int layer);

int bsarec_plan_is_fused(const bsarec_plan_t *plan);
int bsarec_config_is_fused(const bsarec_config_t *cfg);
void bsarec_plan_destroy(bsarec_plan_t *plan);

typedef void (*bsarec_hook_t)(void *user, void *stream);
int bsarec_plan_set_dense_grad_hook(bsarec_plan_t *plan, bsarec_hook_t hook, void *user, float *lookup_grad);

#define BSAREC_TRAIN_NEG_MAX 8192
#define BSAREC_TRAIN_NEG_SITE 0x4E454753u

int bsarec_plan_set_train_sampler(bsarec_plan_t *plan, const int64_t *pop_cum);

long bsarec_buffer_offset(const bsarec_plan_t *plan, int buffer, int layer);

int bsarec_step_begin(bsarec_plan_t *plan, void *stream);

int bsarec_forward(bsarec_plan_t *plan, const int64_t *ids, int train, void *stream);

int bsarec_loss(bsarec_plan_t *plan, const int64_t *answers, void *stream);

int bsarec_forward_last(bsarec_plan_t *plan, const int64_t *ids, int train, void *stream);

int bsarec_loss_bce(bsarec_plan_t *plan, const int64_t *pos_ids, const int64_t *neg_ids, void *stream);
int bsarec_loss_logsig(bsarec_plan_t *plan, const int64_t *pos_ids, const int64_t *neg_ids, void *stream);

int bsarec_logits(bsarec_plan_t *plan, void *stream);

int bsarec_backward(bsarec_plan_t *plan, void *stream);

int bsarec_backward_seq(bsarec_plan_t *plan, const float *d_out, void *stream);

int bsarec_backward_seq_multi(bsarec_plan_t *plan, const float *const *d_outs, void *stream);

typedef struct {
    float *params;
    const float *grads;
    float *exp_avg, *exp_avg_sq;
    long n;
    float lr, beta1, beta2, eps, weight_decay;
    float grad_scale;
    void *shadow_bf16;
    long shadow_from;
    float *grads2;
    long grads2_n;
// ... 152 lines not shown
```

Baseline: 1.727 million.

## Save dropout keep-masks as bits in forward and reuse them in backward

The forward fused layer and embedding kernels now pack each dropout keep/drop decision into a bitmask buffer in the workspace, one bitmask per layer. The backward kernels load these bits instead of regenerating the masks from the hash-based RNG. This trades RNG arithmetic in backward for a small amount of extra global memory traffic and workspace space. It is on by default and can be turned off with BSAREC_DROP_BITS=0.

```diff
diff --git a/bsarec_amd/_lib.py b/bsarec_amd/_lib.py
--- a/bsarec_amd/_lib.py
+++ b/bsarec_amd/_lib.py
@@ -12,7 +12,7 @@
 TRAIN_NEG_SITE = 0x4E454753
 
 (BUF_LAYER_OUT, BUF_LOGITS, BUF_LOSS, BUF_DSP, BUF_HMIX, BUF_PROBS, BUF_DLAYER_IN, BUF_LOSS_ROWS, BUF_CTX,
- BUF_DLOGITS, BUF_TRAIN_CAND, BUF_TRAIN_CORR, BUF_TRAIN_LOGITS, BUF_TRAIN_DLOGITS) = range(14)
+ BUF_DLOGITS, BUF_TRAIN_CAND, BUF_TRAIN_CORR, BUF_TRAIN_LOGITS, BUF_TRAIN_DLOGITS, BUF_DROP_BITS) = range(15)
 K_NONE, K_FFN1, K_FFN2, K_QKV, K_LOGITS, K_DU, K_DW1, K_FUSED_FWD, K_FUSED_BWD = range(9)
 
 LAYER_FIELDS = ["sqrt_beta", "filter_ln_w", "filter_ln_b", "query_w", "query_b", "key_w", "key_b", "value_w", "value_b",
@@ -53,10 +53,12 @@
 
 OPTION_FIELDS = ("storage", "no_fused", "no_prune_top", "dw_tiled", "splits", "top_slabs", "separate_embed", "separate_top", "chain_kernels", "x3_products",
                  "weight_image")
+PLAN_SETTERS = ("drop_bits",)
 HIDDEN_ACTS = {"gelu": 0, "relu": 1, "swish": 2, "tanh": 3, "sigmoid": 4}
 
-_defaults = {k: 0 for k in OPTION_FIELDS}
+_defaults = {k: 0 for k in OPTION_FIELDS + PLAN_SETTERS}
 _defaults["weight_image"] = 1
+_defaults["drop_bits"] = 1
 
 
 def _env_defaults():
@@ -83,6 +85,8 @@
         d["storage"] = 1
     if e.get("BSAREC_WEIGHT_IMAGE") == "0":
         d["weight_image"] = 0
+    if e.get("BSAREC_DROP_BITS") == "0":
+        d["drop_bits"] = 0
     return d
 
 
@@ -159,6 +163,10 @@
     "bsarec_wimage_offset": (C.c_long, [C.c_int] * 5),
     "bsarec_plan_set_dense_grad_hook": (C.c_int, [C.c_void_p, HOOK, C.c_void_p, C.c_void_p]),
     "bsarec_plan_set_train_sampler": (C.c_int, [C.c_void_p, C.c_void_p]),
+    "bsarec_plan_set_drop_bits": (C.c_int, [C.c_void_p, C.c_int]),
+    "bsarec_drop_bits_bytes": (C.c_long, [C.POINTER(Config)]),
+    "bsarec_drop_bits_hidden_bit": (C.c_long, [C.c_int, C.c_long, C.c_long, C.c_int]),
+    "bsarec_drop_bits_attn_bit": (C.c_long, [C.c_long, C.c_int, C.c_long, C.c_int, C.c_int, C.c_int]),
     "bsarec_buffer_is_bf16": (C.c_int, [C.c_void_p, C.c_int, C.c_int]),
     "bsarec_plan_is_fused": (C.c_int, [C.c_void_p]),
     "bsarec_config_is_fused": (C.c_int, [C.c_void_p]),
diff --git a/bsarec_amd/csrc/bsarec_hip.hip b/bsarec_amd/csrc/bsarec_hip.hip
--- a/bsarec_amd/csrc/bsarec_hip.hip
+++ b/bsarec_amd/csrc/bsarec_hip.hip
@@ -101,6 +101,8 @@
     LazyRows lazy = {};
     bool lazy_now = false;
     float* wimg = nullptr;
+    unsigned char* dbitsL[BSAREC_MAX_LAYERS] = {};
+    bool drop_bits = true;
 };
 struct PlanScope {
     bsarec_plan* prev;
@@ -215,6 +217,10 @@
 static bool fused_shape_ok(const bsarec_config_t& c);
 static bool wimage_wanted(const bsarec_config_t& c) {
     return c.weight_image && fused_shape_ok(c) && c.storage == 0 && !c.x3_products && !c.chain_kernels && c.filter_kind == 0;
+}
+
+static bool drop_bits_wanted(const bsarec_config_t& c) {
+    return fused_shape_ok(c) && c.filter_kind == 0 && (c.storage == 1 || (!c.x3_products && !c.chain_kernels && !c.separate_embed));
 }
 
 static bool fused_shape_ok(const bsarec_config_t& c) {
@@ -316,6 +322,8 @@
         p.lazy.d4 = (int)(d / 4);
         p.lazy.mark = cv.take<int>(c.item_size); p.lazy.rows = cv.take<int>(p.lazy.cap); p.lazy.count = cv.take<int>(1);
     }
+    if (drop_bits_wanted(c))
+        for (int l = 0; l < N; ++l) p.dbitsL[l] = cv.take<unsigned char>((size_t)drop_bits_layer_bytes(B, L, c.heads));
     *total = cv.off;
 }
 
@@ -484,7 +492,7 @@
     if (!p) return -1;
     const int N = p->cfg.layers;
     const void* ptr = nullptr;
-    if (buffer >= BSAREC_BUF_TRAIN_CAND && p->cfg.train_negatives == 0) return -1;
+    if (buffer >= BSAREC_BUF_TRAIN_CAND && buffer <= BSAREC_BUF_TRAIN_DLOGITS && p->cfg.train_negatives == 0) return -1;
     switch (buffer) {
         case BSAREC_BUF_LAYER_OUT: if (layer < 0 || layer > N) return -1; ptr = p->X[layer]; break;
         case BSAREC_BUF_LOGITS: ptr = p->logits; break;
@@ -500,6 +508,7 @@
         case BSAREC_BUF_TRAIN_CORR: ptr = p->ssm_corr; break;
         case BSAREC_BUF_TRAIN_LOGITS: ptr = p->ssm_logits; break;
         case BSAREC_BUF_TRAIN_DLOGITS: ptr = p->ssm_dlogits; break;
+        case BSAREC_BUF_DROP_BITS: if (layer < 0 || layer >= N || !p->dbitsL[layer]) return -1; ptr = p->dbitsL[layer]; break;
         default: return -1;
     }
     return (long)((const char*)ptr - p->ws);
@@ -510,6 +519,24 @@
     if (p->cfg.train_negatives > 0 && (hook || lookup_grad)) return -22;
     p->dense_hook = hook; p->dense_hook_user = user; p->lookup_grad = lookup_grad;
     return 0;
+}
+
+extern "C" int bsarec_plan_set_drop_bits(bsarec_plan_t* p, int on) {
+    if (!p || on < 0 || on > 1) return -10;
+    p->drop_bits = on != 0;
+    return 0;
+}
+extern "C" long bsarec_drop_bits_bytes(const bsarec_config_t* cfg) {
+    if (!cfg || check_cfg(*cfg) != 0) return -1;
+    return drop_bits_wanted(*cfg) ? drop_bits_layer_bytes(cfg->batch, cfg->seq_len, cfg->heads) : 0;
+}
+extern "C" long bsarec_drop_bits_hidden_bit(int slot, long tokens, long token, int column) {
+    if (slot < 0 || slot >= DB_SLOTS || tokens < 1 || token < 0 || token >= tokens || column < 0 || column >= 64) return -1;
+    return drop_bits_hidden_bit(slot, tokens, token, column);
+}
+extern "C" long bsarec_drop_bits_attn_bit(long tokens, int heads, long b, int head, int query, int key) {
+    if (tokens < 1 || heads < 1 || b < 0 || head < 0 || head >= heads || query < 0 || query >= 64 || key < 0 || key >= 64) return -1;
+    return drop_bits_attn_bit(tokens, heads, b, head, query, key);
 }
 
 extern "C" int bsarec_plan_set_train_sampler(bsarec_plan_t* p, const int64_t* pop_cum) {
@@ -677,6 +704,7 @@
     F.drop_f = make_drop(p, c.p_hidden, 1 + 4 * l, tr); F.drop_p = make_drop(p, c.p_attn, 2 + 4 * l, tr);
     F.drop_o = make_drop(p, c.p_hidden, 3 + 4 * l, tr); F.drop_ff = make_drop(p, c.p_hidden, 4 + 4 * l, tr);
     F.stamps = p.stamps ? p.stamps + 32 * (2 * l + (FWD ? 0 : 1)) : nullptr;
+    F.dbits = p.drop_bits ? p.dbitsL[l] : nullptr;
     if constexpr (FWD) {
         F.Xout = p.X[l + 1];
         F.f_b = w.filter_ln_b; F.bq = w.query_b; F.bk = w.key_b; F.bv = w.value_b; F.bo = w.dense_b; F.a_b = w.attn_ln_b;
@@ -766,6 +794,18 @@
         return launch_lds<fused_layer_bwd_kernel<32, false, NoTail, false, true>>(grid, block, smem, s, F, NoTail());
     }
     int rc = 0;
+    if (F.dbits) {
+        if (p.wimg)
+            DISPATCH_DH(p.dh, rc = head ? launch_lds<fused_layer_bwd_kernel<DH, false, TopBwdP, false, false, true, true>>(grid, block, smem, s, F, *head)
+                                        : launch_lds<fused_layer_bwd_kernel<DH, false, NoTail, false, false, true, true>>(grid, block, smem, s, F, NoTail()));
+        else if (p.bf)
+            DISPATCH_DH(p.dh, rc = head ? launch_lds<fused_layer_bwd_kernel<DH, true, TopBwdP, false, false, false, true>>(grid, block, smem, s, F, *head)
+                                        : launch_lds<fused_layer_bwd_kernel<DH, true, NoTail, false, false, false, true>>(grid, block, smem, s, F, NoTail()));
+        else
+            DISPATCH_DH(p.dh, rc = head ? launch_lds<fused_layer_bwd_kernel<DH, false, TopBwdP, false, false, false, true>>(grid, block, smem, s, F, *head)
+                                        : launch_lds<fused_layer_bwd_kernel<DH, false, NoTail, false, false, false, true>>(grid, block, smem, s, F, NoTail()));
+        return rc;
+    }
     if (p.wimg) {
         DISPATCH_DH(p.dh, rc = head ? launch_lds<fused_layer_bwd_kernel<DH, false, TopBwdP, false, false, true>>(grid, block, smem, s, F, *head)
                                     : launch_lds<fused_layer_bwd_kernel<DH, false, NoTail, false, false, true>>(grid, block, smem, s, F, NoTail()));
@@ -800,6 +840,11 @@
     TopBwdP F;
     fill_top_bwd(p, l, tr, dXout, F);
     int rc = 0;
+    if (F.dbits) {
+        if (p.bf) DISPATCH_DH(p.dh, rc = launch_lds<top_bwd_kernel<DH, true, true>>(dim3(p.cfg.batch), dim3(256), top_bwd_smem_bytes(), s, F));
+        else DISPATCH_DH(p.dh, rc = launch_lds<top_bwd_kernel<DH, false, true>>(dim3(p.cfg.batch), dim3(256), top_bwd_smem_bytes(), s, F));
+        return rc;
+    }
     DISPATCH_BLOCK(p, rc = launch_lds<top_bwd_kernel<DH, BF>>(dim3(p.cfg.batch), dim3(256), top_bwd_smem_bytes(), s, F));
     return rc;
 }
diff --git a/bsarec_amd/csrc/drop_bits.h b/bsarec_amd/csrc/drop_bits.h
--- /dev/null
+++ b/bsarec_amd/csrc/drop_bits.h
@@ -0,0 +1,52 @@
+#pragma once
+#include "common.h"
+
+enum { DB_EMBED = 0, DB_F = 1, DB_O = 2, DB_FF = 3, DB_SLOTS = 4 };
+
+__host__ __device__ inline long drop_bits_hidden_byte(int slot, long T, long token, int c4) {
+    return ((long)slot * T + token) * 16 + (c4 >> 2);
+}
+__host__ __device__ inline long drop_bits_attn_base(long T) { return (long)DB_SLOTS * T * 16; }
+__host__ __device__ inline long drop_bits_attn_word(int heads, long b, int head, int kt, int half, int query) {
+    return (((b * heads + head) * 2 + kt) * 2 + half) * 64 + query;
+}
+__host__ __device__ inline long drop_bits_layer_bytes(long B, long L, int heads) {
+    return drop_bits_attn_base(B * L) + B * heads * 256 * 2;
+}
+__host__ __device__ inline long drop_bits_hidden_bit(int slot, long T, long token, int c) {
+    return drop_bits_hidden_byte(slot, T, token, c & ~3) * 8 + (c & 3);
+}
+__host__ __device__ inline long drop_bits_attn_bit(long T, int heads, long b, int head, int query, int key) {
+    return (drop_bits_attn_base(T) + 2 * drop_bits_attn_word(heads, b, head, key >> 5, (key >> 2) & 1, query)) * 8 +
+           4 * ((key >> 3) & 3) + (key & 3);
+}
+
+#define DB_GLOBAL __attribute__((address_space(1)))
+__device__ __forceinline__ unsigned drop_keep4(const f32x4& m) {
+    float t = __builtin_amdgcn_fmed3f(m.w, 0.0f, 1.0f);
+    t = fmaf(t, 2.0f, __builtin_amdgcn_fmed3f(m.z, 0.0f, 1.0f));
+    t = fmaf(t, 2.0f, __builtin_amdgcn_fmed3f(m.y, 0.0f, 1.0f));
+    t = fmaf(t, 2.0f, __builtin_amdgcn_fmed3f(m.x, 0.0f, 1.0f));
+    return (unsigned)t;
+}
+__device__ __forceinline__ f32x4 drop_expand4(unsigned keep, float scale) {
+    return f32x4{(keep & 1u) ? scale : 0.f, (keep & 2u) ? scale : 0.f, (keep & 4u) ? scale : 0.f, (keep & 8u) ? scale : 0.f};
+}
+__device__ __forceinline__ unsigned drop_bits_ld8(const unsigned char* base, unsigned off) { return *((const DB_GLOBAL unsigned char*)base + off); }
+__device__ __forceinline__ unsigned drop_bits_ld16(const unsigned char* base, unsigned off) { return *(const DB_GLOBAL unsigned short*)((const DB_GLOBAL unsigned char*)base + off); }
+__device__ __forceinline__ void drop_bits_st8(unsigned char* base, unsigned off, unsigned v) { *((DB_GLOBAL unsigned char*)base + off) = (unsigned char)v; }
+__device__ __forceinline__ void drop_bits_st16(unsigned char* base, unsigned off, unsigned v) { *(DB_GLOBAL unsigned short*)((DB_GLOBAL unsigned char*)base + off) = (unsigned short)v; }
+__device__ __forceinline__ unsigned drop_bits_row_off(int row, int c4) { return (unsigned)(row * 16 + (c4 >> 2)); }
+__device__ __forceinline__ unsigned drop_bits_word_off(int kt, int half, int query) { return (unsigned)(2 * ((kt * 2 + half) * 64 + query)); }
+__device__ __forceinline__ bool drop_bits_live(const DropP& d, const unsigned char* bits) { return bits != nullptr && d.thresh != 0; }
+
+template <bool DB>
+__device__ __forceinline__ unsigned drop_bits_request(const DropP& d, const unsigned char* base, unsigned off) {
+    if constexpr (DB) return d.thresh != 0 ? drop_bits_ld8(base, off) : 0u;
+    else return 0u;
+}
+template <bool DB>
+__device__ __forceinline__ f32x4 drop_mult4_saved(const DropP& d, const DropSeed& sd, uint64_t grp, unsigned keep) {
+    if constexpr (!DB) return drop_mult4(d, sd, grp);
+    else return d.thresh == 0 ? f32x4{d.scale, d.scale, d.scale, d.scale} : drop_expand4(keep, d.scale);
+}
diff --git a/bsarec_amd/csrc/fused_layer.h b/bsarec_amd/csrc/fused_layer.h
--- a/bsarec_amd/csrc/fused_layer.h
+++ b/bsarec_amd/csrc/fused_layer.h
@@ -2,6 +2,7 @@
 #include "common.h"
 #include "kernels.h"
 #include "wimage.h"
+#include "drop_bits.h"
 #include <type_traits>
 
 #define FS 68
@@ -23,6 +24,7 @@
     float *e_X0, *e_xhat, *e_rstd; int* e_ids32;
     int xout_f32;
     const float* filter_cw;
+    unsigned char* dbits;
 };
 
 
@@ -291,7 +293,9 @@
                                            float alpha, float oma, long tok0, int L, float* __restrict__ outL,
                                            float* __restrict__ outG, float* __restrict__ xhatG, float* __restrict__ rstdG,
                                            bool out_f32 = false ,
-                                           bool round_outL = false ) {
+                                           bool round_outL = false ,
+                                           unsigned char* bits = nullptr ,
+                                           int slot = 0) {
     const int lr = threadIdx.x >> 4, lc = (threadIdx.x & 15) << 2;
 #pragma unroll
     for (int i = 0; i < 2; ++i) {
@@ -313,6 +317,7 @@
             ast4<BF>(xhatG, e, xh);
             if (BF && out_f32) gst4(outG + e, y); else ast4<BF>(outG, e, y);
             if (lc == 0) gst(rstdG + tok0 + r, rs);
+            if (bits) drop_bits_st8(bits + drop_bits_hidden_byte(slot, (long)gridDim.x * L, tok0, 0), drop_bits_row_off(r, lc), drop_keep4(P.dm[i]));
         }
         if (BF && round_outL) {
             const unsigned a = pk_bf16(y.x, y.y), c = pk_bf16(y.z, y.w);
@@ -340,12 +345,13 @@
     float xh_ff, g_ff, rs_ff, xa, xf, g_a, g_f, rs_a, rs_f, bt, low_l, x_l, q_l;
     f32x4 tq[16];
     float p_pre;
+    unsigned kb, kw;
 };
 struct TopBwdHelpRegs { f32x4 w2c[16], w1c[16], u4; };
-template <bool BF, unsigned KOFF> __device__ __forceinline__ void top_bwd_prefetch(TopBwdRegs& R);
-template <bool BF, unsigned KOFF> __device__ __forceinline__ void top_bwd_prefetch_tile(TopBwdRegs& R);
+template <bool BF, unsigned KOFF, bool DB> __device__ __forceinline__ void top_bwd_prefetch(TopBwdRegs& R);
+template <bool BF, unsigned KOFF, bool DB> __device__ __forceinline__ void top_bwd_prefetch_tile(TopBwdRegs& R);
 template <bool BF, unsigned KOFF> __device__ __forceinline__ void top_bwd_help_prefetch(TopBwdHelpRegs& H);
-template <int DH, bool BF, unsigned KOFF, bool HELPED>
+template <int DH, bool BF, unsigned KOFF, bool HELPED, bool DB>
 __device__ __forceinline__ void top_bwd_body(const TopBwdRegs& R, const DropSeed& dseed, float* sX, float* sK, float* sV, const float* sTab,
                                              float* sVec, float* sDX);
 template <bool BF, unsigned KOFF> __device__ __forceinline__ void top_bwd_help_a(const TopBwdHelpRegs& H, float* sVec);
@@ -362,6 +368,7 @@
     static_assert(!FM || (!BF && !X3 && !IsTail<TAILP>::value), "the FMLPRec block runs in fp32, without a top-block tail");
     constexpr int MAXCB = FM ? 36 : FUSED_MAX_CB;
     constexpr bool TAIL = IsTail<TAILP>::value;
+    constexpr bool DBITS = !X3 && !FM;
     constexpr unsigned KOFF = (unsigned)((sizeof(FusedFwdP) + 7) & ~(size_t)7);
     const auto R0_L = KARG(FusedFwdP, L);
     const auto R0_Lp = KARG(FusedFwdP, Lp);
@@ -391,6 +398,7 @@
     const int L = R0_L, Lp = R0_Lp, heads = R0_heads, cb = R0_cb;
     const int b = blockIdx.x;
     const long tok0 = (long)b * L;
+    const long Ttok = (long)gridDim.x * L;
     const int col = wn * 32 + l31;
     constexpr int KHM = MM ? 8 : 4;
     const int KH = KHM * half;
@@ -423,6 +431,7 @@
         const float* const e_g = KARG(FusedFwdP, e_g); const float* const e_b = KARG(FusedFwdP, e_b);
         int* const e_ids32 = KARG(FusedFwdP, e_ids32); const DropP e_drop = KARG(FusedFwdP, e_drop);
         float* const e_xhat = KARG(FusedFwdP, e_xhat); float* const e_X0 = KARG(FusedFwdP, e_X0); float* const e_rstd = KARG(FusedFwdP, e_rstd);
+        unsigned char* const e_bits = DBITS ? KARG(FusedFwdP, dbits) : nullptr;
         long src = 0;
         if (gp.table) {
             src = *(const AS_GLOBAL long long*)gp.cursor + b;
@@ -456,10 +465,12 @@
             f32x4 y = {0, 0, 0, 0};
             if (ok) {
                 const f32x4 xh = dl * rs;
-                y = (eg * xh + eb) * drop_mult4(e_drop, dseed, (uint64_t)e >> 2);
+                const f32x4 em = drop_mult4(e_drop, dseed, (uint64_t)e >> 2);
+                y = (eg * xh + eb) * em;
                 ast4<BF>(e_xhat, e, xh);
                 ast4<BF>(e_X0, e, y);
                 if (c4 == 0) gst(e_rstd + tok0 + r, rs);
+                if (drop_bits_live(e_drop, e_bits)) drop_bits_st8(e_bits + drop_bits_hidden_byte(DB_EMBED, Ttok, tok0, 0), drop_bits_row_off(r, c4), drop_keep4(em));
             }
             st4(sX + r * FS + c4, y);
         }
@@ -494,6 +505,7 @@
     const auto R2_wo = KARG(FusedFwdP, wo);
     const auto R2_wv = KARG(FusedFwdP, wv);
     const auto R2_xhat_f = KARG(FusedFwdP, xhat_f);
+    unsigned char* const R2_dbits = DBITS ? KARG(FusedFwdP, dbits) : nullptr;
     {
         float* part = sH;
         const int lr = (tid & 255) >> 4, lc = (tid & 15) << 2;
@@ -580,10 +592,13 @@
                 const bool ok = t < L;
                 const long e = (tok0 + t) * 64 + lc;
                 f32x4 v = {0, 0, 0, 0};
+                unsigned keep_f = 0;
                 if (ok) {
                     const f32x4 xv = ld4(sX + t * FS + lc);
                     const f32x4 low = lowpass_tab(sSpec, t, lc, L, cb, sTab);
-                    v = (low + b2 * (xv - low)) * drop_mult4(R2_drop_f, dseed, (uint64_t)e >> 2) + xv;
+                    const f32x4 fm = drop_mult4(R2_drop_f, dseed, (uint64_t)e >> 2);
+                    keep_f = drop_keep4(fm);
+                    v = (low + b2 * (xv - low)) * fm + xv;
                 }
                 const float mean = group_sum<16>(v.x + v.y + v.z + v.w) * (1.0f / 64.0f);
                 f32x4 dl = {0, 0, 0, 0};
@@ -598,6 +613,7 @@
                     if (R2_dsp) gst4(R2_dsp + e, y);
                     if constexpr (FM) gst4(R2_hmix + e, y);
                     if (lc == 0) gst(R2_rstd_f + (tok0 + t), rs);
+                    if (drop_bits_live(R2_drop_f, R2_dbits)) drop_bits_st8(R2_dbits + drop_bits_hidden_byte(DB_F, Ttok, tok0, 0), drop_bits_row_off(t, lc), keep_f);
                 }
                 st4((FM ? sH : sD) + t * FS + lc, y);
             }
@@ -625,6 +641,7 @@
     const auto R3_ctx = KARG(FusedFwdP, ctx);
     const auto R3_drop_p = KARG(FusedFwdP, drop_p);
     const auto R3_probs = KARG(FusedFwdP, probs);
+    unsigned char* const R3_dbits = DBITS ? KARG(FusedFwdP, dbits) : nullptr;
     {
         const int nt = (L + 31) >> 5;
         const float sqrt_dh = sqrtf((float)DH);
@@ -672,6 +689,7 @@
             if (act) {
                 if (nt == 2) sum += sRed[(pair * 2 + (kt ^ 1)) * 64 + lane];
                 const float inv = 1.0f / sum;
+                unsigned keep_p = 0;
 #pragma unroll
                 for (int g = 0; g < 4; ++g) {
                     const int key0 = 32 * kt + 8 * g + 4 * half;
@@ -681,10 +699,13 @@
                         const long e = (((long)b * heads + head) * L + query) * Lp + key0;
                         ast4<BF>(R3_probs, e, p);
                         m = drop_mult4(R3_drop_p, dseed, (uint64_t)e >> 2);
+                        keep_p |= drop_keep4(m) << (4 * g);
                     }
                     p = p * m;
                     st[4 * g] = p.x; st[4 * g + 1] = p.y; st[4 * g + 2] = p.z; st[4 * g + 3] = p.w;
                 }
+                if (drop_bits_live(R3_drop_p, R3_dbits) && query < L)
+                    drop_bits_st16(R3_dbits + drop_bits_attn_base(Ttok) + 2 * drop_bits_attn_word(heads, b, head, 0, 0, 0), drop_bits_word_off(kt, half, query), keep_p);
                 float* dstT = kt == 0 ? sC : sE;
 #pragma unroll
                 for (int ct = 0; ct < NCT; ++ct) {
@@ -772,7 +793,8 @@
     }
     if constexpr (!FM) {
     lds_barrier();
-    ln_rows_64<true, BF>(lnA, sQ, sK, sX, R4_eps, sD, R4_alpha, R4_oma, tok0, L, sH, R4_hmix, R4_xhat_a, R4_rstd_a);
+    ln_rows_64<true, BF>(lnA, sQ, sK, sX, R4_eps, sD, R4_alpha, R4_oma, tok0, L, sH, R4_hmix, R4_xhat_a, R4_rstd_a, false, false,
+                         DBITS && R4_drop_o.thresh != 0 ? KARG(FusedFwdP, dbits) : nullptr, DB_O);
     lds_barrier();
     }
 
@@ -846,7 +868,8 @@
     const auto R7_rstd_ff = KARG(FusedFwdP, rstd_ff);
     const auto R7_xhat_ff = KARG(FusedFwdP, xhat_ff);
     ln_rows_64<false, BF>(lnF, sX, sE, sH, R7_eps, nullptr, 0.f, 1.f, tok0, L,
-                          TAIL ? sD : nullptr, R7_Xout, R7_xhat_ff, R7_rstd_ff, KARG(FusedFwdP, xout_f32) != 0, TAIL);
+                          TAIL ? sD : nullptr, R7_Xout, R7_xhat_ff, R7_rstd_ff, KARG(FusedFwdP, xout_f32) != 0, TAIL,
+                          DBITS && R7_drop_ff.thresh != 0 ? KARG(FusedFwdP, dbits) : nullptr, DB_FF);
     STAMP(8);
     if constexpr (TAIL) {
         lds_barrier();
@@ -876,6 +899,7 @@
     float* e_dz; const float *e_xhat, *e_rstd, *e_g; float *e_pg, *e_pb; DropP e_drop;
     const float* filter_cw; float* pcw;
     const float* e_dx_extra;
+    const unsigned char* dbits;
 };
 
 
@@ -904,23 +928,22 @@
 #pragma unroll
     for (int i = 0; i < N; ++i) st4(red[i] + lr * 64 + lc, v[i]);
     lds_barrier();
-    const int i = threadIdx.x >> 6, c = threadIdx.x & 63;
-    if (i < N) {
-        const float* r = red[0];
-        float* d = dst[0];
-#pragma unroll
-        for (int k = 1; k < N; ++k) if (i == k) { r = red[k]; d = dst[k]; }
-        float s0 = 0.f, s1 = 0.f, s2 = 0.f, s3 = 0.f;
-        for (int g = 0; g < ng; g += 4) {
-            s0 += r[g * 64 + c]; s1 += r[(g + 1) * 64 + c]; s2 += r[(g + 2) * 64 + c]; s3 += r[(g + 3) * 64 + c];
-        }
-        float sum = (s0 + s1) + (s2 + s3);
-        if (i == 0) { if (mul0) sum *= gld(mul0 + c); sum *= scale0; }
-        gst(d + c, sum);
-    }
-}
-
-template <int DH, bool BF, class HEADP, bool X3 = false, bool FM = false, bool IMG = false>
+    const int i = __builtin_amdgcn_readfirstlane(threadIdx.x >> 6), c = threadIdx.x & 63;
+#pragma unroll
+    for (int k = 0; k < N; ++k)
+        if (i == k) {
+            const float* r = red[k];
+            float s0 = 0.f, s1 = 0.f, s2 = 0.f, s3 = 0.f;
+            for (int g = 0; g < ng; g += 4) {
+                s0 += r[g * 64 + c]; s1 += r[(g + 1) * 64 + c]; s2 += r[(g + 2) * 64 + c]; s3 += r[(g + 3) * 64 + c];
+            }
+            float sum = (s0 + s1) + (s2 + s3);
+            if (k == 0) { if (mul0) sum *= gld(mul0 + c); sum *= scale0; }
+            gst(dst[k] + c, sum);
+        }
+}
+
+template <int DH, bool BF, class HEADP, bool X3 = false, bool FM = false, bool IMG = false, bool DB = false>
 __global__ void __launch_bounds__(512) __attribute__((amdgpu_waves_per_eu(2, 2)))
 fused_layer_bwd_kernel(const FusedBwdP P_unused, const HEADP H_unused) {
 #define PTYPE FusedBwdP
@@ -929,6 +952,8 @@
     constexpr int MM = X3 ? 2 : (BF ? 1 : 0);
     static_assert(!FM || (!BF && !X3 && !IsTail<HEADP>::value), "the FMLPRec block runs in fp32, without a top-block head");
     constexpr bool HEAD = IsTail<HEADP>::value;
+    static_assert(!DB || (!X3 && !FM), "keep bits are left by the BSARec block's forward in fp32 / bf16 storage");
+    constexpr bool DBITS = DB;
     constexpr unsigned KOFF = (unsigned)((sizeof(FusedBwdP) + 7) & ~(size_t)7);
     const auto R0_L = KARG(FusedBwdP, L);
     const auto R0_Lp = KARG(FusedBwdP, Lp);
@@ -955,6 +980,7 @@
     const int L = R0_L, Lp = R0_Lp, heads = R0_heads, cb = R0_cb;
     const int b = blockIdx.x;
     const long tok0 = (long)b * L;
+    const long Ttok = (long)gridDim.x * L;
     const int col = wn * 32 + l31;
     constexpr int KHM = MM ? 8 : 4;
     const int KH = KHM * half;
@@ -966,10 +992,10 @@
     TopBwdRegs HR;
     TopBwdHelpRegs HH;
     if constexpr (HEAD) {
-        if (wave == 0) top_bwd_prefetch<BF, KOFF>(HR);
+        if (wave == 0) top_bwd_prefetch<BF, KOFF, DB>(HR);
         else if (wave < 4) {
             if (wave == 3) build_twiddle_table(KARG(FusedBwdP, tw), L, cb, sTab, 192, 64);
-            top_bwd_prefetch_tile<BF, KOFF>(HR);
+            top_bwd_prefetch_tile<BF, KOFF, DB>(HR);
         } else top_bwd_help_prefetch<BF, KOFF>(HH);
     }
     const DropSeed dseed = drop_seed(KARG(FusedBwdP, drop_f));
@@ -987,10 +1013,11 @@
     const auto R1_tw = KARG(FusedBwdP, tw);
     const auto R1_w2 = KARG(FusedBwdP, w2);
     const auto R1_xhat_ff = KARG(FusedBwdP, xhat_ff);
+    const unsigned char* const R1_dbits = DBITS ? KARG(FusedBwdP, dbits) : nullptr;
     if constexpr (!FM && !HEAD) build_twiddle_table(R1_tw, L, cb, sTab);
     if constexpr (HEAD) {
         if (wave < 4) {
-            top_bwd_body<DH, BF, KOFF, true>(HR, dseed, sG, sdF, sPm, sTab, sAcc, sT);
+            top_bwd_body<DH, BF, KOFF, true, DB>(HR, dseed, sG, sdF, sPm, sTab, sAcc, sT);
         } else {
             top_bwd_help_a<BF, KOFF>(HH, sAcc);
             f32x4 uw[16];
@@ -1009,11 +1036,13 @@
     const f32x4 g = gld4(R1_ff_g + lc);
     f32x4 dy[2], xh[2];
     float rs[2];
+    unsigned kb_ff[2];
 #pragma unroll
     for (int i = 0; i < 2; ++i) {
         const int r = 32 * i + lr;
         const long e = (tok0 + r) * 64 + lc;
         dy[i] = f32x4{0, 0, 0, 0}; xh[i] = dy[i]; rs[i] = 0.f;
+        kb_ff[i] = drop_bits_request<DBITS>(R1_drop_ff, R1_dbits + drop_bits_hidden_byte(DB_FF, Ttok, tok0, 0), drop_bits_row_off(min(r, L - 1), lc));
         if (R1_dh_slabs) {
             if (r < L) {
                 if (r == L - 1)
@@ -1055,7 +1084,7 @@
             const f32x4 dz = rs[i] * (gg - m1 - xh[i] * m2);
             sg += dy[i] * xh[i]; sb += dy[i];
             f32x4 dt = {0, 0, 0, 0};
-            if (ok) { dt = dz * drop_mult4(R1_drop_ff, dseed, (uint64_t)e >> 2); ast4<BF>(R1_dT, e, dt); }
+            if (ok) { dt = dz * drop_mult4_saved<DBITS>(R1_drop_ff, dseed, (uint64_t)e >> 2, kb_ff[i]); ast4<BF>(R1_dT, e, dt); }
             st4(sAcc + r * FS + lc, dz);
             st4(sT + r * FS + lc, dt);
         }
@@ -1135,9 +1164,12 @@
     STAMP(2);
     const auto R3_w1 = KARG(FusedBwdP, w1);
     const auto R3_wo = KARG(FusedBwdP, wo);
+    const unsigned char* const R3_dbits = DBITS ? KARG(FusedBwdP, dbits) : nullptr;
+    const DropP R3_drop_o = KARG(FusedBwdP, drop_o), R3_drop_f = KARG(FusedBwdP, drop_f);
     WFrag<MM, 32> wO;
     f32x4 pq[2], pk[2], pv[2], xa[2], xf[2];
     float ra[2], rf[2];
+    unsigned kb_o[2] = {0u, 0u}, kb_f[2] = {0u, 0u};
     {
         f32x16 acc;
 #pragma unroll
@@ -1155,6 +1187,8 @@
             }
             xf[i] = ald4<BF>(KARG(FusedBwdP, xhat_f), ec);
             rf[i] = gld(KARG(FusedBwdP, rstd_f) + tok0 + min(r, L - 1));
+            kb_o[i] = drop_bits_request<DBITS>(R3_drop_o, R3_dbits + drop_bits_hidden_byte(DB_O, Ttok, tok0, 0), drop_bits_row_off(min(r, L - 1), lc));
+            kb_f[i] = drop_bits_request<DBITS>(R3_drop_f, R3_dbits + drop_bits_hidden_byte(DB_F, Ttok, tok0, 0), drop_bits_row_off(min(r, L - 1), lc));
         }
         mma_w<MM, 64>(sa, wA, acc);
         mma_w<MM, 64>(sa + 64, wB, acc);
@@ -1355,8 +1389,8 @@
             sga += dya * xa[i]; sba += dya; sgf += dyf * xf[i]; sbf += dyf;
             f32x4 dO = {0, 0, 0, 0}, dF = dO;
             if (ok) {
-                dO = dza * drop_mult4(R4_drop_o, dseed, (uint64_t)e >> 2);
-                dF = dzf * drop_mult4(R4_drop_f, dseed, (uint64_t)e >> 2);
+                dO = dza * drop_mult4_saved<DBITS>(R4_drop_o, dseed, (uint64_t)e >> 2, kb_o[i]);
+                dF = dzf * drop_mult4_saved<DBITS>(R4_drop_f, dseed, (uint64_t)e >> 2, kb_f[i]);
                 ast4<BF>(R4_dO, e, dO);
             }
             st4(sAcc + r * FS + lc, dza + dzf);
@@ -1396,6 +1430,7 @@
     const auto R6_drop_p = KARG(FusedBwdP, drop_p);
     const auto R6_dv = KARG(FusedBwdP, dv);
     const auto R6_probs = KARG(FusedBwdP, probs);
+    const unsigned char* const R6_dbits = DBITS ? KARG(FusedBwdP, dbits) : nullptr;
     {
         const int nt = (L + 31) >> 5;
         const float inv_sqrt_dh = 1.0f / sqrtf((float)DH);
@@ -1406,18 +1441,28 @@
             const int qt = (wave >> 1) & 1, kt = wave & 1;
             const int query = 32 * qt + l31;
             const bool c1 = wave < 4;
-            f32x4 pp[4], mm[4];
+            f32x4 pp[4];
             f32x16 da;
             float delta = 0.f;
             if (c1) {
+                constexpr bool SAVED = DBITS;
+                f32x4 mm[SAVED ? 1 : 4];
+                unsigned kw = 0;
+                if constexpr (SAVED) {
+                    if (R6_drop_p.thresh != 0 && query < L)
+                        kw = drop_bits_ld16(R6_dbits + drop_bits_attn_base(Ttok) + 2 * drop_bits_attn_word(heads, b, head, 0, 0, 0),
+                                            drop_bits_word_off(kt, half, query));
+                }
 #pragma unroll
                 for (int g = 0; g < 4; ++g) {
                     const int key0 = 32 * kt + 8 * g + 4 * half;
-                    pp[g] = f32x4{0, 0, 0, 0}; mm[g] = pp[g];
+                    pp[g] = f32x4{0, 0, 0, 0};
+                    if constexpr (!SAVED) mm[g] = pp[g];
                     if (query < L && key0 < Lp) {
                         const long e = (((long)b * heads + head) * L + query) * Lp + key0;
                         pp[g] = ald4<BF>(R6_probs, e);
-                        mm[g] = drop_mult4(R6_drop_p, dseed, (uint64_t)e >> 2);
+                        if constexpr (!SAVED) mm[g] = drop_mult4(R6_drop_p, dseed, (uint64_t)e >> 2);
+                        else if (R6_drop_p.thresh == 0) kw |= 0xFu << (4 * g);
                     }
                 }
 #pragma unroll
@@ -1428,10 +1473,13 @@
                 for (int g = 0; g < 4; ++g)
 #pragma unroll
                     for (int j = 0; j < 4; ++j) {
-                        const float dA = da[4 * g + j] * mm[g][j];
+                        float m;
+                        if constexpr (SAVED) m = (kw >> (4 * g + j)) & 1u ? R6_drop_p.scale : 0.f;
+                        else m = mm[g][j];
+                        const float dA = da[4 * g + j] * m;
                         delta += dA * pp[g][j];
                         da[4 * g + j] = dA;
-                        sPm[(32 * kt + 8 * g + 4 * half + j) * FS + query] = pp[g][j] * mm[g][j];
+                        sPm[(32 * kt + 8 * g + 4 * half + j) * FS + query] = pp[g][j] * m;
                     }
                 delta = xor32_sum(delta);
                 sRed[(qt * 2 + kt) * 64 + lane] = delta;
@@ -1569,20 +1617,29 @@
         float* const e_dz = KARG(FusedBwdP, e_dz);
         const float* const e_dx_extra = KARG(FusedBwdP, e_dx_extra);
         f32x4 g0 = {0, 0, 0, 0}, e_xh[2], e_ex[2], e_dm[2];
-        float e_rs[2];
+        float e_rs[2], e_scale = 1.f;
+        unsigned kb_e[2] = {0u, 0u};
+        bool e_nodrop = true;
 #pragma unroll
         for (int i = 0; i < 2; ++i) { e_xh[i] = f32x4{0, 0, 0, 0}; e_ex[i] = e_xh[i]; e_dm[i] = e_xh[i]; e_rs[i] = 0.f; }
         if (e_dz || e_dx_extra) {
             const float* const e_xhat = KARG(FusedBwdP, e_xhat);
             const float* const e_rstd = KARG(FusedBwdP, e_rstd);
             const DropP e_drop = KARG(FusedBwdP, e_drop);
+            const unsigned char* const e_bits = DBITS ? KARG(FusedBwdP, dbits) : nullptr;
+            e_nodrop = e_drop.thresh == 0; e_scale = e_drop.scale;
             if (e_dz) g0 = gld4(KARG(FusedBwdP, e_g) + lc);
 #pragma unroll
             for (int i = 0; i < 2; ++i) {
                 const int t = 32 * i + lr;
                 const long e = (tok0 + min(t, L - 1)) * 64 + lc;
                 if (e_dx_extra) e_ex[i] = gld4(e_dx_extra + e);
-                if (e_dz) { e_xh[i] = ald4<BF>(e_xhat, e); e_rs[i] = gld(e_rstd + tok0 + min(t, L - 1)); e_dm[i] = drop_mult4(e_drop, dseed, (uint64_t)e >> 2); }
+                if (e_dz) {
+                    e_xh[i] = ald4<BF>(e_xhat, e); e_rs[i] = gld(e_rstd + tok0 + min(t, L - 1));
+                    if constexpr (DBITS)
+                        kb_e[i] = drop_bits_request<DBITS>(e_drop, e_bits + drop_bits_hidden_byte(DB_EMBED, Ttok, tok0, 0), drop_bits_row_off(min(t, L - 1), lc));
+                    else e_dm[i] = drop_mult4(e_drop, dseed, (uint64_t)e >> 2);
+                }
             }
         }
 #pragma unroll
@@ -1650,7 +1707,11 @@
                 dx = ld4(sG + t * FS + lc) + b2 * df + lowg;
                 if (e_dx_extra) dx += e_ex[i];
                 sb += df * (xv - lowx);
-                if (e_dz) { xh = e_xh[i]; rs = e_rs[i]; dx = dx * e_dm[i]; }
+                if (e_dz) {
+                    xh = e_xh[i]; rs = e_rs[i];
+                    if constexpr (DBITS) dx = dx * drop_expand4(e_nodrop ? 0xFu : kb_e[i], e_scale);
+                    else dx = dx * e_dm[i];
+                }
                 else ast4<BF>(R8_dX, e, dx);
             }
             if (e_dz) {
diff --git a/bsarec_amd/csrc/fused_top.h b/bsarec_amd/csrc/fused_top.h
--- a/bsarec_amd/csrc/fused_top.h
+++ b/bsarec_amd/csrc/fused_top.h
@@ -12,6 +12,7 @@
     DropP drop_f, drop_p, drop_o, drop_ff;
     long long* stamps;
     const float *wk_sh, *wv_sh;
+    unsigned char* dbits;
 };
 
 __device__ __forceinline__ float drop_mult1(const DropP& d, const DropSeed& sd, uint64_t e) {
@@ -21,6 +22,37 @@
     const int j = (int)(e & 3);
     const uint32_t r = j == 0 ? w.x : j == 1 ? w.y : j == 2 ? w.z : w.w;
     return r >= d.thresh ? d.scale : 0.f;
+}
+
+__device__ __forceinline__ void top_keep_row(const DropP& d, unsigned char* bits, int slot, long T, long tok, float mult) {
+    if (!drop_bits_live(d, bits)) return;
+    const unsigned long long k = __ballot(mult != 0.f);
+    const int lane = threadIdx.x & 63;
+    if (lane < 16) drop_bits_st8(bits + drop_bits_hidden_byte(slot, T, tok, 0), (unsigned)lane, (unsigned)(k >> (4 * lane)) & 0xFu);
+}
+__device__ __forceinline__ void top_keep_attn(const DropP& d, unsigned char* bits, long T, int heads, long b, int head, int query, int Lp,
+                                              float mult) {
+    if (!drop_bits_live(d, bits)) return;
+    const int lane = threadIdx.x & 63;
+    const unsigned long long k = __ballot(mult != 0.f && lane < Lp);
+    if (lane < 4) {
+        unsigned w = 0;
+#pragma unroll
+        for (int g = 0; g < 4; ++g) w |= ((unsigned)(k >> (4 * (8 * (lane >> 1) + 2 * g + (lane & 1)))) & 0xFu) << (4 * g);
+        drop_bits_st16(bits + drop_bits_attn_base(T) + 2 * drop_bits_attn_word(heads, b, head, 0, 0, 0),
+                       drop_bits_word_off(lane >> 1, lane & 1, query), w);
+    }
+}
+__device__ __forceinline__ unsigned top_row_request(const unsigned char* bits, int slot, long T, long tok, int c) {
+    return drop_bits_ld8(bits + drop_bits_hidden_byte(slot, T, tok, 0), (unsigned)(c >> 2));
+}
+__device__ __forceinline__ unsigned top_attn_request(const unsigned char* bits, long T, int heads, long b, int head, int query, int key) {
+    return drop_bits_ld16(bits + drop_bits_attn_base(T) + 2 * drop_bits_attn_word(heads, b, head, 0, 0, 0),
+                          drop_bits_word_off(key >> 5, (key >> 2) & 1, query));
+}
+__device__ __forceinline__ float top_row_mult(const DropP& d, unsigned keep, int c) { return (keep >> (c & 3)) & 1u ? d.scale : 0.f; }
+__device__ __forceinline__ float top_attn_mult(const DropP& d, unsigned word, int key) {
+    return (word >> (4 * ((key >> 3) & 3) + (key & 3))) & 1u ? d.scale : 0.f;
 }
 
 template <int K, int KS>
@@ -136,6 +168,8 @@
     float* const k_low = TP(low); const DropP d_f = TP(drop_f); const float k_eps = TP(eps);
     float* const k_xhat_f = TP(xhat_f); float* const k_rstd_f = TP(rstd_f);
     const float* const pW1 = TP(w1); const float* const pW2 = TP(w2);
+    unsigned char* const dbits = TP(dbits);
+    const long Ttok = (long)gridDim.x * L;
 
     if constexpr (!HELPED) {
         const int arow = (wm * 32 + l31) * FS + KH;
@@ -158,7 +192,11 @@
         auto xsrc = [&](int, int t, int lc) { return ld4(sX + t * FS + lc); };
         dft_spectrum_tab<1>(xsrc, L, cb, sTab, sSpec, sPart);
     } else {
-        if (wave == 1) sMul[lane] = drop_mult1(d_f, dseed, (uint64_t)(el + lane));
+        if (wave == 1) {
+            const float m = drop_mult1(d_f, dseed, (uint64_t)(el + lane));
+            sMul[lane] = m;
+            top_keep_row(d_f, dbits, DB_F, Ttok, tok0 + tl, m);
+        }
         const int t = 16 * wave + (lane & 15);
         float pl = 0.f;
         if (t < L)
@@ -204,7 +242,9 @@
         gst(k_low + el + c, low);
         const float bt = R.c_beta;
         const float f = low + bt * bt * (xv - low);
-        const float v = f * (HELPED ? sMul[c] : drop_mult1(d_f, dseed, (uint64_t)(el + c))) + xv;
+        const float m_f = HELPED ? sMul[c] : drop_mult1(d_f, dseed, (uint64_t)(el + c));
+        if constexpr (!HELPED) top_keep_row(d_f, dbits, DB_F, Ttok, tok0 + tl, m_f);
+        const float v = f * m_f + xv;
         float xh, rs;
         ln_row(v, k_eps, xh, rs);
         ast<BF>(k_xhat_f, el + c, xh);
@@ -214,11 +254,15 @@
     if constexpr (HELPED) {
         if (wave >= 2) {
             const DropP dd = wave == 2 ? TP(drop_o) : TP(drop_ff);
-            sMul[(wave - 1) * 64 + lane] = drop_mult1(dd, dseed, (uint64_t)(el + lane));
+            const float m = drop_mult1(dd, dseed, (uint64_t)(el + lane));
+            sMul[(wave - 1) * 64 + lane] = m;
+            top_keep_row(dd, dbits, wave == 2 ? DB_O : DB_FF, Ttok, tok0 + tl, m);
             const DropP dp = TP(drop_p);
             for (int h = wave - 2; h < heads; h += 2) {
                 const long pe = (((long)b * heads + h) * L + tl) * Lp;
-                sMp[h * 64 + lane] = drop_mult1(dp, dseed, (uint64_t)(pe + lane));
+                const float mp = drop_mult1(dp, dseed, (uint64_t)(pe + lane));
+                sMp[h * 64 + lane] = mp;
+                top_keep_attn(dp, dbits, Ttok, heads, b, h, tl, Lp, mp);
             }
         }
     }
@@ -247,7 +291,9 @@
         const float p = e / group_sum<64>(e);
         const long pe = (((long)b * heads + head) * L + tl) * Lp;
         if (key < Lp) ast<BF>(k_probs, pe + key, p);
-        sPd[head * 64 + key] = key < L ? p * (HELPED ? sMp[head * 64 + key] : drop_mult1(d_p, dseed, (uint64_t)(pe + key))) : 0.f;
+        const float m_p = HELPED ? sMp[head * 64 + key] : drop_mult1(d_p, dseed, (uint64_t)(pe + key));
+        if constexpr (!HELPED) top_keep_attn(d_p, dbits, Ttok, heads, b, head, tl, Lp, m_p);
+        sPd[head * 64 + key] = key < L ? p * m_p : 0.f;
     }
     const DropP d_o = TP(drop_o); float* const k_xhat_a = TP(xhat_a); float* const k_rstd_a = TP(rstd_a);
     const float k_alpha = TP(alpha), k_oma = TP(oma); float* const k_hmix = TP(hmix); float* const k_u = TP(u);
@@ -275,7 +321,9 @@
     if constexpr (!HELPED) { if (wave != 0) gemv_rows_load<256, 4>(pW2, 256, on, osl, w2r); }
     if (wave == 0) {
         const int c = lane;
-        const float v = sG[c] * (HELPED ? sMul[64 + c] : drop_mult1(d_o, dseed, (uint64_t)(el + c))) + sX[tl * FS + c];
+        const float m_o = HELPED ? sMul[64 + c] : drop_mult1(d_o, dseed, (uint64_t)(el + c));
+        if constexpr (!HELPED) top_keep_row(d_o, dbits, DB_O, Ttok, tok0 + tl, m_o);
+        const float v = sG[c] * m_o + sX[tl * FS + c];
         float xh, rs;
         ln_row(v, k_eps, xh, rs);
         ast<BF>(k_xhat_a, el + c, xh);
@@ -305,7 +353,9 @@
     TSTAMP(8);
     if (wave == 0) {
         const int c = lane;
-        const float v = sQ[c] * (HELPED ? sMul[128 + c] : drop_mult1(d_ff, dseed, (uint64_t)(el + c))) + sHm[c];
+        const float m_ff = HELPED ? sMul[128 + c] : drop_mult1(d_ff, dseed, (uint64_t)(el + c));
+        if constexpr (!HELPED) top_keep_row(d_ff, dbits, DB_FF, Ttok, tok0 + tl, m_ff);
+        const float v = sQ[c] * m_ff + sHm[c];
         float xh, rs;
         ln_row(v, k_eps, xh, rs);
         ast<BF>(k_xhat_ff, el + c, xh);
@@ -471,6 +521,7 @@
     float alpha, oma;
     DropP drop_f, drop_p, drop_o, drop_ff;
     long long* stamps;
+    const unsigned char* dbits;
 };
 
 __device__ __forceinline__ float ln_row_bwd(float dy, float gamma, float xhat, float rstd) {
@@ -484,7 +535,7 @@
 #define BSTAMP(i) do { long long* st_ = TB(stamps); if (st_ && blockIdx.x == 0 && threadIdx.x == 0) st_[i] = clock64(); } while (0)
 static_assert(TOP_BWD_BARRIERS == 11, "barriers of top_bwd_body (fused_layer.h holds the constant)");
 
-template <bool BF, unsigned KOFF>
+template <bool BF, unsigned KOFF, bool DB>
 __device__ __forceinline__ void top_bwd_prefetch(TopBwdRegs& R) {
     const int c = threadIdx.x & 63;
     const int L = TB(L), b = blockIdx.x, tl = L - 1;
@@ -509,14 +560,28 @@
     R.q_l = ald<BF>(k_q, el + c);
     const int heads = TB(heads), Lp = TB(Lp);
     R.p_pre = c < L ? ald<BF>(TB(probs), (((long)b * heads + 0) * L + tl) * Lp + c) : 0.f;
-}
-template <bool BF, unsigned KOFF>
+    R.kb = 0; R.kw = 0;
+    if constexpr (DB) {
+        const unsigned char* const bits = TB(dbits);
+        const long Ttok = (long)gridDim.x * L;
+        if (TB(drop_ff).thresh != 0) R.kb = top_row_request(bits, DB_FF, Ttok, tok0 + tl, c);
+        if (TB(drop_p).thresh != 0) R.kw = top_attn_request(bits, Ttok, heads, b, 0, tl, c);
+    }
+}
+template <bool BF, unsigned KOFF, bool DB>
 __device__ __forceinline__ void top_bwd_prefetch_tile(TopBwdRegs& R) {
     const int lane = threadIdx.x & 63, wave = threadIdx.x >> 6;
     const int L = TB(L), Lp = TB(Lp), heads = TB(heads), b = blockIdx.x, tl = L - 1;
     const long tok0 = (long)b * L;
     const float* const src = wave == 1 ? TB(X) : wave == 2 ? TB(k) : TB(v);
     R.p_pre = (wave < heads && lane < L) ? ald<BF>(TB(probs), (((long)b * heads + wave) * L + tl) * Lp + lane) : 0.f;
+    R.kb = 0; R.kw = 0;
+    if constexpr (DB) {
+        const unsigned char* const bits = TB(dbits);
+        const long Ttok = (long)gridDim.x * L;
+        if (wave < 3 && (wave == 1 ? TB(drop_o) : TB(drop_f)).thresh != 0) R.kb = top_row_request(bits, wave == 1 ? DB_O : DB_F, Ttok, tok0 + tl, lane);
+        if (wave < heads && TB(drop_p).thresh != 0) R.kw = top_attn_request(bits, Ttok, heads, b, wave, tl, lane);
+    }
 #pragma unroll
     for (int p = 0; p < 16; ++p) {
         const int idx = lane + p * 64, r = idx >> 4, c4 = (idx & 15) << 2;
@@ -608,7 +673,7 @@
     lds_barrier();
 }
 
-template <int DH, bool BF, unsigned KOFF, bool HELPED>
+template <int DH, bool BF, unsigned KOFF, bool HELPED, bool DB>
 __device__ __forceinline__ void top_bwd_body(const TopBwdRegs& R, const DropSeed& dseed, float* sX, float* sK, float* sV, const float* sTab,
                                              float* sVec, float* sDX) {
     float* sDT = sVec;
@@ -643,6 +708,15 @@
     const float* const pX = TB(X); const float* const pK = TB(k); const float* const pV = TB(v);
     const float* const pW1 = TB(w1); const float* const pW2 = TB(w2); const float* const pU = TB(u);
     const float* const pWo = TB(wo); const float* const pWq = TB(wq); const float* const pWk = TB(wk); const float* const pWv = TB(wv);
+    const unsigned char* const dbits = DB ? TB(dbits) : nullptr;
+    const long Ttok = (long)gridDim.x * L;
+    auto row_mult = [&](const DropP& d, int slot) {
+        if constexpr (!DB) return drop_mult1(d, dseed, (uint64_t)(el + c));
+        else {
+            if (d.thresh == 0) return d.scale;
+            return top_row_mult(d, (HELPED || wave == 0) ? R.kb : top_row_request(dbits, slot, Ttok, tok0 + tl, c), c);
+        }
+    };
     auto weight_loads = [&]() {
         if constexpr (!HELPED) {
             u_mine = ald<BF>(pU, (tok0 + tl) * 256 + tid);
@@ -661,15 +735,15 @@
     };
     if (wave != 0) {
         if constexpr (!HELPED) { weight_loads(); tile_loads(); }
-        if (wave == 1) { const DropP d_o = TB(drop_o); sDH[c] = drop_mult1(d_o, dseed, (uint64_t)(el + c)); }
-        if (wave == 2) { const DropP d_f = TB(drop_f); sDQ[c] = drop_mult1(d_f, dseed, (uint64_t)(el + c)); }
+        if (wave == 1) { const DropP d_o = TB(drop_o); sDH[c] = row_mult(d_o, DB_O); }
+        if (wave == 2) { const DropP d_f = TB(drop_f); sDQ[c] = row_mult(d_f, DB_F); }
     }
     if (wave == 0) {
         const int ns = TB(dh_nsplit);
         const DropP d_ff = TB(drop_ff);
         float* const k_pg_ff = TB(pg_ff); float* const k_pb_ff = TB(pb_ff); float* const k_dT = TB(dT);
         xa = R.xa; xf = R.xf; g_a = R.g_a; g_f = R.g_f; rs_a = R.rs_a; rs_f = R.rs_f; bt = R.bt; low_l = R.low_l; x_l = R.x_l;
-        const float m_ff = drop_mult1(d_ff, dseed, (uint64_t)(el + c));
+        const float m_ff = row_mult(d_ff, DB_FF);
         asm volatile("" :: "v"(m_ff));
         __builtin_amdgcn_sched_barrier(0);
         float part[4] = {0.f, 0.f, 0.f, 0.f};
@@ -781,7 +855,9 @@
             }
             const long pe = (((long)b * heads + head) * L + tl) * Lp + key;
             p = HELPED ? R.p_pre : ald<BF>(k_probs, pe);
-            mp = drop_mult1(d_p, dseed, (uint64_t)pe);
+            if constexpr (!DB) mp = drop_mult1(d_p, dseed, (uint64_t)pe);
+            else if (d_p.thresh == 0) mp = d_p.scale;
+            else mp = top_attn_mult(d_p, (HELPED || wave == 0) ? R.kw : top_attn_request(dbits, Ttok, heads, b, head, tl, key), key);
         }
         const float dp = dpd * mp;
         const float delta = group_sum<64>(p * dp);
@@ -839,7 +915,7 @@
     BSTAMP(15);
 }
 
-template <int DH, bool BF>
+template <int DH, bool BF, bool DB = false>
 __global__ void __launch_bounds__(256)
 top_bwd_kernel(const TopBwdP P_unused) {
     constexpr unsigned KOFF = 0;
@@ -852,11 +928,11 @@
     float* sVec = sTab + FUSED_MAX_CB * 128;
     BSTAMP(0);
     TopBwdRegs R;
-    if (threadIdx.x < 64) top_bwd_prefetch<BF, KOFF>(R);
+    if (threadIdx.x < 64) top_bwd_prefetch<BF, KOFF, DB>(R);
     const DropSeed dseed = drop_seed(TB(drop_f));
     build_twiddle_table(TB(tw), TB(L), TB(cb), sTab);
     lds_barrier();
-    top_bwd_body<DH, BF, KOFF, false>(R, dseed, sX, sK, sV, sTab, sVec, nullptr);
+    top_bwd_body<DH, BF, KOFF, false, DB>(R, dseed, sX, sK, sV, sTab, sVec, nullptr);
 }
 
 
diff --git a/bsarec_amd/model.py b/bsarec_amd/model.py
--- a/bsarec_amd/model.py
+++ b/bsarec_amd/model.py
@@ -65,6 +65,7 @@
         for k in L.OPTION_FIELDS:
             setattr(self.cfg, k, int(opts.get(k, 0)))
         self.options = {k: int(getattr(self.cfg, k)) for k in L.OPTION_FIELDS}
+        self.options.update({k: int(opts.get(k, 0)) for k in L.PLAN_SETTERS})
         for k in L.TRAIN_FIELDS:
             setattr(self.cfg, k, model.train_head[k])
         self.cfg.train_lazy_adam = int(model.lazy_adam)
@@ -94,6 +95,7 @@
                                        self.ws.data_ptr(), nbytes, self.state.data_ptr(),
                                        model._twiddle.data_ptr(), stream), "bsarec_plan_create")
         self.lib = lib
+        L.check(lib.bsarec_plan_set_drop_bits(self.handle, self.options["drop_bits"]), "bsarec_plan_set_drop_bits")
         if self.cfg.train_negatives > 0 and self.cfg.train_sampler == 1 and model._train_cum is not None:
             model._install_train_sampler(self)
 
diff --git a/include/bsarec_hip.h b/include/bsarec_hip.h
--- a/include/bsarec_hip.h
+++ b/include/bsarec_hip.h
@@ -71,7 +71,8 @@
     BSAREC_BUF_TRAIN_CAND = 10,
     BSAREC_BUF_TRAIN_CORR = 11,
     BSAREC_BUF_TRAIN_LOGITS = 12,
-    BSAREC_BUF_TRAIN_DLOGITS = 13
+    BSAREC_BUF_TRAIN_DLOGITS = 13,
+    BSAREC_BUF_DROP_BITS = 14
 };
 
 typedef struct bsarec_plan bsarec_plan_t;
@@ -102,6 +103,11 @@
 #define BSAREC_TRAIN_NEG_SITE 0x4E454753u
 
 int bsarec_plan_set_train_sampler(bsarec_plan_t *plan, const int64_t *pop_cum);
+
+int bsarec_plan_set_drop_bits(bsarec_plan_t *plan, int on);
+long bsarec_drop_bits_bytes(const bsarec_config_t *cfg);
+long bsarec_drop_bits_hidden_bit(int slot, long tokens, long token, int column);
+long bsarec_drop_bits_attn_bit(long tokens, int heads, long b, int head, int query, int key);
 
 long bsarec_buffer_offset(const bsarec_plan_t *plan, int buffer, int layer);
 
```

After: 1.746 million (median of 6 runs). 1.01x the previous value.
